# ratt-ru/tricolour

Measured on AMD Instinct MI355X. Metric: Mvis/s flagged (bl x time x chan x corr), higher is better.
Workload: dtype f32 data / f64 accumulators / u8 flags; 1 GPU; MeerKAT-64 slab: 252 of 2016 bl x 4 corr x 1024 time x 4096 chan per GPU (BASELINE configs[1] processed as HBM-resident baseline slabs), sum_threshold_flagger kwargs=stage1; params=stage1

## Files before the change

tricolour_amd/csrc/kernels_elementwise.hpp:

```cpp
#pragma once

template <int VD>
__global__ void k_prepare(const void* __restrict__ vis, const uint8_t* __restrict__ iflags,
                          float* __restrict__ data, uint8_t* __restrict__ flags,
                          int T, int F, int Fa, int factor) {
    size_t idx = (size_t)blockIdx.x * blockDim.x + threadIdx.x;
    size_t NA = (size_t)T * Fa;
    if (idx >= NA) return;
    int t = (int)(idx / Fa), fo = (int)(idx % Fa);
    size_t w = blockIdx.y;
    size_t base = w * (size_t)T * F + (size_t)t * F;
    int f0 = fo * factor;
    int f1 = min(F, f0 + factor);
    float sum = 0.0f;
    int cnt = 0;
    for (int f = f0; f < f1; f++) {
        if (VD == TRI_VIS_F64) {
            const double a = fabs(reinterpret_cast<const double*>(vis)[base + f]);
            if (!iflags[base + f] && !isnan(a)) { sum = (float)((double)sum + a); cnt++; }
            continue;
        }
        float a = load_amp<VD>(vis, base + f);
        if (!iflags[base + f] && !isnan(a)) { sum += a; cnt++; }
    }
    size_t o = w * NA + idx;
    if (cnt == 0) { data[o] = 0.0f; flags[o] = 1; }
    else { data[o] = sum / (float)cnt; flags[o] = 0; }
}

__global__ void k_abs_c64(const float2* __restrict__ z, float* __restrict__ out, size_t n) {
    size_t i = (size_t)blockIdx.x * blockDim.x + threadIdx.x;
    if (i < n) out[i] = tri_hypotf(z[i].x, z[i].y);
}

template <typename T, bool PANEL = false>
__global__ void k_transpose(const T* __restrict__ src, T* __restrict__ dst, int R, int C,
                            size_t src_ws, size_t dst_ws, float denom) {
    __shared__ T tile[64][65];
    const T* s = src + (size_t)blockIdx.z * src_ws;
    T* d = dst + (size_t)blockIdx.z * dst_ws;
    int c0 = blockIdx.x * 64, r0 = blockIdx.y * 64;
    int tx = threadIdx.x, ty = threadIdx.y;
    for (int j = ty; j < 64; j += 4) {
        int r = r0 + j, c = c0 + tx;
        if (r < R && c < C) tile[j][tx] = s[(size_t)r * C + c];
    }
    __syncthreads();
    for (int j = ty; j < 64; j += 4) {
        int c = c0 + j, r = r0 + tx;
        if (r < R && c < C) {
            T v = tile[tx][j];
            if (sizeof(T) == 4 && denom != 0.0f) v = (T)((float)v / denom);
            if (PANEL) d[((size_t)blockIdx.y * C + c) * 64 + tx] = v;
            else d[(size_t)c * R + r] = v;
        }
    }
}

template <typename T>
__global__ void k_panelize(const T* __restrict__ src, T* __restrict__ dst, int L, int C, size_t ws) {
    const size_t i = (size_t)blockIdx.x * blockDim.x + threadIdx.x;
    if (i >= (size_t)L * C) return;
    const int l = (int)(i / C), c = (int)(i % C);
    dst[blockIdx.y * ws + ((size_t)(c >> 6) * L + l) * 64 + (c & 63)] = src[blockIdx.y * ws + i];
}
template <typename T>
__global__ void k_unpanel_w(const T* __restrict__ src, T* __restrict__ dst, int L, int C, size_t ws) {
    const size_t i = (size_t)blockIdx.x * blockDim.x + threadIdx.x;
    if (i >= (size_t)L * C) return;
    const int l = (int)(i / C), c = (int)(i % C);
    dst[blockIdx.y * ws + i] = src[blockIdx.y * ws + ((size_t)(c >> 6) * L + l) * 64 + (c & 63)];
}
template <typename T>
__global__ void k_unpanel(const T* __restrict__ src, T* __restrict__ dst, int L, int C) {
    const size_t i = (size_t)blockIdx.x * blockDim.x + threadIdx.x;
    if (i >= (size_t)L * C) return;
    const int l = (int)(i / C), c = (int)(i % C);
    dst[i] = src[((size_t)(c >> 6) * L + l) * 64 + (c & 63)];
}

template <bool COPY, bool ZERO>
__global__ __launch_bounds__(256) void k_transpose_u8w(const uint8_t* __restrict__ src, uint8_t* __restrict__ dst,
                                                       uint8_t* __restrict__ copy, float* __restrict__ data, int R, int C,
                                                       size_t src_ws, size_t dst_ws, size_t copy_ws, size_t data_ws) {
    __shared__ unsigned tile[128][17];
    const uint8_t* s = src + (size_t)blockIdx.z * src_ws;
    uint8_t* d = dst + (size_t)blockIdx.z * dst_ws;
    const int c0 = blockIdx.x * 64, r0 = blockIdx.y * 128;
    const int tid = threadIdx.x;
    {
        const int tx = tid & 15, ty = tid >> 4;
        const int c = c0 + 4 * tx;
#pragma unroll
        for (int j = 0; j < 8; j++) {
            const int rr = ty + 16 * j, r = r0 + rr;
            unsigned v = 0;
            if (r < R && c < C) {
                v = *reinterpret_cast<const unsigned*>(s + (size_t)r * C + c);
                if (COPY) *reinterpret_cast<unsigned*>(copy + (size_t)blockIdx.z * copy_ws + (size_t)r * C + c) = v;
            }
            tile[rr][tx] = v;
        }
    }
    __syncthreads();
    const int bx = tid & 31, q0 = tid >> 5;
    const int r = r0 + 4 * bx;
    if (r >= R) return;
#pragma unroll
    for (int h = 0; h < 2; h++) {
        const int q = q0 + 8 * h;
        const unsigned a0 = tile[4 * bx][q], a1 = tile[4 * bx + 1][q], a2 = tile[4 * bx + 2][q], a3 = tile[4 * bx + 3][q];
        const unsigned t0 = __builtin_amdgcn_perm(a1, a0, 0x05010400u), t1 = __builtin_amdgcn_perm(a1, a0, 0x07030602u);
        const unsigned u0 = __builtin_amdgcn_perm(a3, a2, 0x05010400u), u1 = __builtin_amdgcn_perm(a3, a2, 0x07030602u);
        const unsigned o[4] = {__builtin_amdgcn_perm(u0, t0, 0x05040100u), __builtin_amdgcn_perm(u0, t0, 0x07060302u),
                               __builtin_amdgcn_perm(u1, t1, 0x05040100u), __builtin_amdgcn_perm(u1, t1, 0x07060302u)};
#pragma unroll
        for (int b = 0; b < 4; b++) {
            const int c = c0 + 4 * q + b;
            if (c >= C) break;
            *reinterpret_cast<unsigned*>(d + (size_t)c * R + r) = o[b];
            if (ZERO && o[b]) {
                const unsigned f = o[b];
                float4* pd = reinterpret_cast<float4*>(data + (size_t)blockIdx.z * data_ws + (size_t)c * R + r);
                float4 x = *pd;
                const bool dirty = ((f & 0xFFu) && __float_as_uint(x.x)) || ((f & 0xFF00u) && __float_as_uint(x.y)) ||
                                   ((f & 0xFF0000u) && __float_as_uint(x.z)) || ((f & 0xFF000000u) && __float_as_uint(x.w));
                if (dirty)
                    *pd = make_float4((f & 0xFFu) ? 0.0f : x.x, (f & 0xFF00u) ? 0.0f : x.y, (f & 0xFF0000u) ? 0.0f : x.z,
                                      (f & 0xFF000000u) ? 0.0f : x.w);
            }
        }
    }
}

__global__ void k_build_wo(const float* __restrict__ data, const uint8_t* __restrict__ flags,
                           float* __restrict__ w, float* __restrict__ o, size_t nper,
                           size_t sws, size_t dws) {
    size_t i = (size_t)blockIdx.x * blockDim.x + threadIdx.x;
    if (i >= nper) return;
    size_t win = blockIdx.y;
    bool fl = flags[win * sws + i] != 0;
    w[win * dws + i] = fl ? 0.0f : 1.0f;
    o[win * dws + i] = fl ? 0.0f : data[win * sws + i];
}

__global__ void k_build_wo4(const float* __restrict__ data, const uint8_t* __restrict__ flags,
                            float* __restrict__ w, float* __restrict__ o, size_t n4per,
                            size_t sws, size_t dws) {
    size_t i = (size_t)blockIdx.x * blockDim.x + threadIdx.x;
    if (i >= n4per) return;
    size_t win = blockIdx.y;
    uchar4 f = reinterpret_cast<const uchar4*>(flags + win * sws)[i];
    float4 d = reinterpret_cast<const float4*>(data + win * sws)[i];
    reinterpret_cast<float4*>(w + win * dws)[i] =
        make_float4(f.x ? 0.0f : 1.0f, f.y ? 0.0f : 1.0f, f.z ? 0.0f : 1.0f, f.w ? 0.0f : 1.0f);
    reinterpret_cast<float4*>(o + win * dws)[i] =
        make_float4(f.x ? 0.0f : d.x, f.y ? 0.0f : d.y, f.z ? 0.0f : d.z, f.w ? 0.0f : d.w);
}

template <int MODE>
__global__ void k_masked_div(const float* __restrict__ w, float* __restrict__ o,
                             const float* __restrict__ data, size_t nper, size_t ws_wo,
                             size_t ws_data, float denom, uint8_t* __restrict__ nanflag, int C) {
    size_t i = (size_t)blockIdx.x * blockDim.x + threadIdx.x;
    if (i >= nper) return;
    size_t win = blockIdx.y;
    float wv = w[win * ws_wo + i];
    float ov = o[win * ws_wo + i];
    if (denom != 0.0f) { wv = wv / denom; ov = ov / denom; }
    float bg = (wv == 0.0f) ? NAN : ov / wv;
    if (MODE != 1 && nanflag && isnan(bg)) nanflag[win * (size_t)C + (i % C)] = 1;
    if (MODE == 1) bg = fabsf(data[win * ws_data + i] - bg);
    o[win * ws_wo + i] = bg;
    if (MODE == 2) const_cast<float*>(w)[win * ws_wo + i] = data[win * ws_data + i] - bg;
}

template <bool TWOD>
__global__ void k_reject(const float* __restrict__ resid, uint8_t* __restrict__ flags,
                         const double* __restrict__ med, const int* __restrict__ chunk_of,
                         double scale, int L, int C, int G, size_t ws_resid, size_t ws_flags) {
    size_t i = (size_t)blockIdx.x * blockDim.x + threadIdx.x;
    if (i >= (size_t)L * C) return;
    size_t win = blockIdx.y;
    int l = (int)(i / C), c = (int)(i % C);
    int g = chunk_of[l];
    double m = TWOD ? med[win * G + g] : med[(size_t)c * G + g];
    double thr = m * scale;
    if ((double)resid[win * ws_resid + i] > thr) flags[win * ws_flags + i] = 1;
}

__global__ void k_colinterp(float* __restrict__ a, int L, int C, size_t ws,
                            const uint8_t* __restrict__ nanflag, const float* __restrict__ data,
                            size_t ws_data, float* __restrict__ resid, float* __restrict__ panel, size_t ws_panel) {
    int c = blockIdx.x * blockDim.x + threadIdx.x;
    if (c >= C) return;
    if (nanflag && !nanflag[(size_t)blockIdx.y * C + c]) return;
    float* x = a + (size_t)blockIdx.y * ws + c;
    const size_t Cs = (size_t)C;
    int last = -1;
    float lastv = 0.0f;
    int run = 0;
    constexpr int PFI = 64;
    for (int i0 = 0; i0 < L; i0 += PFI) {
        float vv[PFI];
#pragma unroll
        for (int u = 0; u < PFI; u++) vv[u] = (i0 + u < L) ? x[(size_t)(i0 + u) * Cs] : NAN;
#pragma unroll
        for (int u = 0; u < PFI; u++) {
            const int i = i0 + u;
            const float v = vv[u];
            if (i >= L || isnan(v)) continue;
            if (run < i) {
                if (last < 0) {
                    for (int j = run; j < i; j++) x[(size_t)j * Cs] = v;
                } else {
                    float diff = v - lastv;
                    double grad = (double)diff / (double)(i - last);
                    for (int j = run; j < i; j++)
                        x[(size_t)j * Cs] = (float)((double)lastv + (double)(j - last) * grad);
                }
            }
            last = i;
            lastv = v;
            run = i + 1;
        }
    }
    if (run < L) {
        float fill = last < 0 ? 0.0f : lastv;
        for (int j = run; j < L; j++) x[(size_t)j * Cs] = fill;
    }
    if (resid) {
        const float* d = data + (size_t)blockIdx.y * ws_data + c;
        float* rr = resid + (size_t)blockIdx.y * ws + c;
        int j = 0;
        for (; j + PFI <= L; j += PFI) {
            float dv[PFI], xv[PFI];
#pragma unroll
            for (int u = 0; u < PFI; u++) { dv[u] = d[(size_t)(j + u) * Cs]; xv[u] = x[(size_t)(j + u) * Cs]; }
#pragma unroll
            for (int u = 0; u < PFI; u++) rr[(size_t)(j + u) * Cs] = dv[u] - xv[u];
        }
        for (; j < L; j++) rr[(size_t)j * Cs] = d[(size_t)j * Cs] - x[(size_t)j * Cs];
        if (panel) {
            float* pp = panel + (size_t)blockIdx.y * ws_panel + (size_t)c * 64;
            for (j = 0; j < L; j++) pp[(size_t)(j >> 6) * Cs * 64 + (j & 63)] = rr[(size_t)j * Cs];
        }
    }
}

#define INTERP_SEG 512
__global__ void k_interp_scan(const float* __restrict__ a, int L, int C, size_t ws, const uint8_t* __restrict__ nanflag,
                              int* __restrict__ tab) {
    const int c = blockIdx.x * 64 + threadIdx.x;
    if (c >= C) return;
    const int seg = blockIdx.y, nseg = gridDim.y;
    const int s0 = seg * INTERP_SEG, s1 = min(L, s0 + INTERP_SEG);
    int* t = tab + (((size_t)blockIdx.z * nseg + seg) * 3) * C + c;
    if (nanflag && !nanflag[(size_t)blockIdx.z * C + c]) {
        t[0] = s0; t[C] = s1 - 1; t[2 * (size_t)C] = 0;
        return;
    }
    const float* x = a + (size_t)blockIdx.z * ws + c;
    const size_t Cs = (size_t)C;
    int first = -1, last = -1, nans = 0;
    constexpr int PFI = 64;
    for (int i0 = s0; i0 < s1; i0 += PFI) {
        float vv[PFI];
#pragma unroll
        for (int u = 0; u < PFI; u++) vv[u] = (i0 + u < s1) ? x[(size_t)(i0 + u) * Cs] : 0.0f;
#pragma unroll
        for (int u = 0; u < PFI; u++) {
            const bool nn = isnan(vv[u]);
            if (i0 + u < s1) {
                if (nn) nans = 1;
                else { if (first < 0) first = i0 + u; last = i0 + u; }
            }
        }
    }
    t[0] = first; t[C] = last; t[2 * (size_t)C] = nans;
}

__global__ void k_interp_fix(float* __restrict__ a, int L, int C, size_t ws, const int* __restrict__ tab,
                             const float* __restrict__ data, size_t ws_data, float* __restrict__ resid,
                             float* __restrict__ panel, size_t ws_panel) {
    const int c = blockIdx.x * 64 + threadIdx.x;
    if (c >= C) return;
    const int seg = blockIdx.y, nseg = gridDim.y;
    const int* tw = tab + (size_t)blockIdx.z * nseg * 3 * C + c;
    if (!tw[((size_t)seg * 3 + 2) * C]) return;
    const int s0 = seg * INTERP_SEG, s1 = min(L, s0 + INTERP_SEG);
    float* x = a + (size_t)blockIdx.z * ws + c;
    const float* d = resid ? data + (size_t)blockIdx.z * ws_data + c : nullptr;
    float* rr = resid ? resid + (size_t)blockIdx.z * ws + c : nullptr;
    float* pp = (resid && panel) ? panel + (size_t)blockIdx.z * ws_panel + (size_t)c * 64 : nullptr;
    const size_t Cs = (size_t)C;
    auto put = [&](int j, float v) {
        x[(size_t)j * Cs] = v;
        if (resid) {
            const float dr = d[(size_t)j * Cs] - v;
            rr[(size_t)j * Cs] = dr;
            if (pp) pp[(size_t)(j >> 6) * Cs * 64 + (j & 63)] = dr;
        }
    };
    auto fill = [&](int lo, int hi, int last, float lastv, int i, float v) {
        if (last < 0) {
            for (int j = lo; j < hi; j++) put(j, v);
        } else {
            float diff = v - lastv;
            double grad = (double)diff / (double)(i - last);
            for (int j = lo; j < hi; j++) put(j, (float)((double)lastv + (double)(j - last) * grad));
        }
    };
    int last = -1;
    for (int sg = seg - 1; sg >= 0 && last < 0; sg--) last = tw[((size_t)sg * 3 + 1) * C];
    float lastv = last >= 0 ? x[(size_t)last * Cs] : 0.0f;
    int run = s0;
    constexpr int PFI = 64;
    for (int i0 = s0; i0 < s1; i0 += PFI) {
        float vv[PFI];
#pragma unroll
        for (int u = 0; u < PFI; u++) vv[u] = (i0 + u < s1) ? x[(size_t)(i0 + u) * Cs] : NAN;
#pragma unroll
        for (int u = 0; u < PFI; u++) {
            const int i = i0 + u;
            const float v = vv[u];
            if (i >= s1 || isnan(v)) continue;
            if (run < i) fill(run, i, last, lastv, i, v);
            last = i;
            lastv = v;
            run = i + 1;
        }
    }
    if (run < s1) {
        int nxt = -1;
        for (int sg = seg + 1; sg < nseg && nxt < 0; sg++) nxt = tw[((size_t)sg * 3) * C];
        if (nxt >= 0) {
            fill(run, s1, last, lastv, nxt, x[(size_t)nxt * Cs]);
        } else {
            const float f = last < 0 ? 0.0f : lastv;
            for (int j = run; j < s1; j++) put(j, f);
        }
    }
}

__global__ void k_sub(const float* __restrict__ a, const float* __restrict__ b,
                      float* __restrict__ out, size_t nper, size_t ws_a, size_t ws_b,
                      size_t ws_o) {
    size_t i = (size_t)blockIdx.x * blockDim.x + threadIdx.x;
    if (i >= nper) return;
    size_t win = blockIdx.y;
    out[win * ws_o + i] = a[win * ws_a + i] - b[win * ws_b + i];
}

__global__ void k_or(uint8_t* __restrict__ a, const uint8_t* __restrict__ b, size_t nper,
                     size_t ws_a, size_t ws_b) {
    size_t i = (size_t)blockIdx.x * blockDim.x + threadIdx.x;
    if (i >= nper) return;
    size_t win = blockIdx.y;
    if (b[win * ws_b + i]) a[win * ws_a + i] = 1;
}

__global__ void k_copy_u8(const uint8_t* __restrict__ a, uint8_t* __restrict__ b, size_t n) {
    size_t i = (size_t)blockIdx.x * blockDim.x + threadIdx.x;
    if (i < n) b[i] = a[i];
}

__global__ void k_or_spec(uint8_t* __restrict__ flags, const uint8_t* __restrict__ spec, int T,
                          int Fa, int Wn) {
    size_t i = (size_t)blockIdx.x * blockDim.x + threadIdx.x;
    if (i >= (size_t)T * Fa) return;
    size_t win = blockIdx.y;
    int f = (int)(i % Fa);
    if (spec[(size_t)f * Wn + win]) flags[win * (size_t)T * Fa + i] = 1;
}

__global__ void k_combine(const uint8_t* __restrict__ spec, const uint8_t* __restrict__ tflags,
                          const uint8_t* __restrict__ fflags, uint8_t* __restrict__ comb, int T,
                          int Fa, int Wn, int lo, int hi) {
    size_t i = (size_t)blockIdx.x * blockDim.x + threadIdx.x;
    if (i >= (size_t)T * Fa) return;
    size_t win = blockIdx.y;
    int t = (int)(i / Fa), f = (int)(i % Fa);
    size_t base = win * (size_t)T * Fa;
    int t0 = max(t + lo, 0), t1 = min(t + hi, T);
    uint8_t v = 0;
    if (t1 > t0) {
        if (spec[(size_t)f * Wn + win]) v = 1;
        for (int tt = t0; tt < t1 && !v; tt++) {
            size_t a = base + (size_t)tt * Fa + f;
            v = (tflags[a] | fflags[a]) ? 1 : 0;
        }
    }
    comb[base + i] = v;
}

__global__ void k_unaverage(const uint8_t* __restrict__ comb, uint8_t* __restrict__ dil,
                            int* __restrict__ rowcnt, int* __restrict__ colcnt, int T, int Fa,
                            int F, int avg, int lo, int hi) {
    int f = blockIdx.x * blockDim.x + threadIdx.x;
    int t = blockIdx.y;
    size_t win = blockIdx.z;
    int v = 0;
    if (f < F) {
        int f0 = max(f + lo, 0), f1 = min(f + hi, F);
        const uint8_t* row = comb + win * (size_t)T * Fa + (size_t)t * Fa;
        for (int ff = f0; ff < f1 && !v; ff++) v = row[ff / avg] ? 1 : 0;
        dil[win * (size_t)T * F + (size_t)t * F + f] = (uint8_t)v;
        if (v) atomicAdd(&colcnt[win * (size_t)F + f], 1);
    }
    unsigned long long b = __ballot(v);
    if ((threadIdx.x & 63) == 0 && b) atomicAdd(&rowcnt[win * (size_t)T + t], __popcll(b));
}

template <int VD>
__global__ void k_final(const uint8_t* __restrict__ dil, const int* __restrict__ rowcnt,
                        const int* __restrict__ colcnt, const void* __restrict__ vis,
                        uint8_t* __restrict__ out, uint8_t* __restrict__ iter, int T, int F,
                        double row_limit, double col_limit, int update_iter) {
    size_t i = (size_t)blockIdx.x * blockDim.x + threadIdx.x;
    if (i >= (size_t)T * F) return;
    size_t win = blockIdx.y;
    int t = (int)(i / F), f = (int)(i % F);
    size_t a = win * (size_t)T * F + i;
    bool v = dil[a] != 0;
    v = v || ((double)rowcnt[win * (size_t)T + t] > row_limit);
    v = v || ((double)colcnt[win * (size_t)F + f] > col_limit);
    v = v || load_isnan<VD>(vis, a);
    out[a] = v ? 1 : 0;
    if (update_iter && v) iter[a] = 1;
}

__device__ __forceinline__ uint4 or4(uint4 a, uint4 b) { return make_uint4(a.x | b.x, a.y | b.y, a.z | b.z, a.w | b.w); }
__device__ __forceinline__ unsigned nz_bytes(unsigned x) {
    unsigned t = (x & 0x7F7F7F7Fu) + 0x7F7F7F7Fu;
    return ((t | x) & 0x80808080u) >> 7;
}

template <int VD>
__global__ void k_prepare4(const void* __restrict__ vis, const uint8_t* __restrict__ iflags,
                           float* __restrict__ data, uint8_t* __restrict__ flags, size_t n4) {
    size_t i = (size_t)blockIdx.x * blockDim.x + threadIdx.x;
    if (i >= n4) return;
    uchar4 f = reinterpret_cast<const uchar4*>(iflags)[i];
    float a[4];
    if (VD == TRI_VIS_C64) {
        float4 z0 = reinterpret_cast<const float4*>(vis)[2 * i];
        float4 z1 = reinterpret_cast<const float4*>(vis)[2 * i + 1];
        a[0] = tri_hypotf(z0.x, z0.y); a[1] = tri_hypotf(z0.z, z0.w);
        a[2] = tri_hypotf(z1.x, z1.y); a[3] = tri_hypotf(z1.z, z1.w);
    } else {
        float4 z = reinterpret_cast<const float4*>(vis)[i];
        a[0] = fabsf(z.x); a[1] = fabsf(z.y); a[2] = fabsf(z.z); a[3] = fabsf(z.w);
    }
    unsigned char fl[4] = {f.x, f.y, f.z, f.w};
    float o[4];
    unsigned char of[4];
#pragma unroll
    for (int k = 0; k < 4; k++) {
        bool bad = fl[k] != 0 || isnan(a[k]);
        o[k] = bad ? 0.0f : (0.0f + a[k]) / 1.0f;
        of[k] = bad ? 1 : 0;
    }
    reinterpret_cast<float4*>(data)[i] = make_float4(o[0], o[1], o[2], o[3]);
    reinterpret_cast<uchar4*>(flags)[i] = make_uchar4(of[0], of[1], of[2], of[3]);
}

template <int VD>
__global__ void k_amplitude4(const void* __restrict__ vis, float* __restrict__ ampl,
                             uint8_t* __restrict__ iter, uint16_t* __restrict__ nanmask, size_t n4) {
    size_t i = (size_t)blockIdx.x * blockDim.x + threadIdx.x;
    if (i >= n4) return;
    float a[4];
    bool vn[4];
    if (VD == TRI_VIS_C64) {
        float4 z0 = reinterpret_cast<const float4*>(vis)[2 * i];
        float4 z1 = reinterpret_cast<const float4*>(vis)[2 * i + 1];
        a[0] = tri_hypotf(z0.x, z0.y); a[1] = tri_hypotf(z0.z, z0.w);
        a[2] = tri_hypotf(z1.x, z1.y); a[3] = tri_hypotf(z1.z, z1.w);
        vn[0] = isnan(z0.x) || isnan(z0.y); vn[1] = isnan(z0.z) || isnan(z0.w);
        vn[2] = isnan(z1.x) || isnan(z1.y); vn[3] = isnan(z1.z) || isnan(z1.w);
    } else {
        float4 z = reinterpret_cast<const float4*>(vis)[i];
        a[0] = fabsf(z.x); a[1] = fabsf(z.y); a[2] = fabsf(z.z); a[3] = fabsf(z.w);
        vn[0] = isnan(z.x); vn[1] = isnan(z.y); vn[2] = isnan(z.z); vn[3] = isnan(z.w);
    }
#pragma unroll
    for (int k = 0; k < 4; k++) a[k] = (0.0f + a[k]) / 1.0f;
    reinterpret_cast<float4*>(ampl)[i] = make_float4(a[0], a[1], a[2], a[3]);
    const unsigned nanb = (isnan(a[0]) ? 1u : 0u) | (isnan(a[1]) ? 0x100u : 0u) | (isnan(a[2]) ? 0x10000u : 0u) |
                          (isnan(a[3]) ? 0x1000000u : 0u);
    if (nanb) reinterpret_cast<unsigned*>(iter)[i] |= nanb;
    unsigned m = ((vn[0] ? 1u : 0u) | (vn[1] ? 2u : 0u) | (vn[2] ? 4u : 0u) | (vn[3] ? 8u : 0u)) << (4 * (threadIdx.x & 3));
    m |= __shfl_xor(m, 1, 64);
    m |= __shfl_xor(m, 2, 64);
    if ((threadIdx.x & 3) == 0) nanmask[i >> 2] = (uint16_t)m;
}

__global__ void k_zero_flagged4(const uint8_t* __restrict__ flags, float* __restrict__ data, size_t n4per,
                                size_t ws_flags, size_t ws_data) {
    size_t i = (size_t)blockIdx.x * blockDim.x + threadIdx.x;
    if (i >= n4per) return;
    size_t win = blockIdx.y;
    const unsigned f = reinterpret_cast<const unsigned*>(flags + win * ws_flags)[i];
    if (f == 0) return;
    float4* pd = reinterpret_cast<float4*>(data + win * ws_data) + i;
    float4 d = *pd;
    *pd = make_float4((f & 0xFFu) ? 0.0f : d.x, (f & 0xFF00u) ? 0.0f : d.y, (f & 0xFF0000u) ? 0.0f : d.z,
                      (f & 0xFF000000u) ? 0.0f : d.w);
}

template <int OP>
__global__ void k_u8_op16(const uint8_t* __restrict__ a, uint8_t* __restrict__ b, size_t n16per,
                          size_t ws_a, size_t ws_b) {
    size_t i = (size_t)blockIdx.x * blockDim.x + threadIdx.x;
    if (i >= n16per) return;
    size_t win = blockIdx.y;
    uint4 va = reinterpret_cast<const uint4*>(a + win * ws_a)[i];
    uint4* pb = reinterpret_cast<uint4*>(b + win * ws_b) + i;
    if (OP == 0) *pb = va;
    else if (OP == 1) *pb = or4(*pb, va);
    else *pb = make_uint4(nz_bytes(va.x), nz_bytes(va.y), nz_bytes(va.z), nz_bytes(va.w));
}

__global__ void k_spec_rows(const uint8_t* __restrict__ spec, uint8_t* __restrict__ rows, int Fa, int Wn) {
    size_t i = (size_t)blockIdx.x * blockDim.x + threadIdx.x;
    if (i >= (size_t)Fa * Wn) return;
    int w = (int)(i / Fa), f = (int)(i % Fa);
    rows[i] = spec[(size_t)f * Wn + w];
}

__global__ void k_or_spec16(uint8_t* __restrict__ flags, const uint8_t* __restrict__ spec_rows, int T, int Fa16) {
    size_t i = (size_t)blockIdx.x * blockDim.x + threadIdx.x;
    if (i >= (size_t)T * Fa16) return;
    size_t win = blockIdx.y;
    int f16 = (int)(i % Fa16);
    uint4 sp = reinterpret_cast<const uint4*>(spec_rows + win * (size_t)Fa16 * 16)[f16];
    uint4* pf = reinterpret_cast<uint4*>(flags + win * (size_t)T * Fa16 * 16) + i;
    *pf = or4(*pf, sp);
}

__global__ void k_or_spec_more16(uint8_t* __restrict__ flags, const uint8_t* __restrict__ spec_rows,
                                 const uint8_t* __restrict__ more, int T, int Fa16) {
    size_t i = (size_t)blockIdx.x * blockDim.x + threadIdx.x;
    if (i >= (size_t)T * Fa16) return;
    size_t win = blockIdx.y;
    int f16 = (int)(i % Fa16);
    uint4 sp = reinterpret_cast<const uint4*>(spec_rows + win * (size_t)Fa16 * 16)[f16];
    size_t a = win * (size_t)T * Fa16 + i;
    uint4* pf = reinterpret_cast<uint4*>(flags) + a;
    *pf = or4(or4(*pf, sp), reinterpret_cast<const uint4*>(more)[a]);
}

__global__ void k_or_spec_ft16(uint8_t* __restrict__ flagsFT, const uint8_t* __restrict__ spec_rows, int T16, int Fa) {
    size_t i = (size_t)blockIdx.x * blockDim.x + threadIdx.x;
    if (i >= (size_t)T16 * Fa) return;
    size_t win = blockIdx.y;
    int f = (int)(i / T16);
    if (!spec_rows[win * (size_t)Fa + f]) return;
    reinterpret_cast<uint4*>(flagsFT + win * (size_t)T16 * 16 * Fa)[i] = make_uint4(0x01010101u, 0x01010101u, 0x01010101u, 0x01010101u);
}

__global__ void k_combine16(const uint8_t* __restrict__ spec_rows, const uint8_t* __restrict__ tflags,
                            const uint8_t* __restrict__ fflags, uint8_t* __restrict__ comb, int T,
                            int Fa16, int lo, int hi) {
    size_t i = (size_t)blockIdx.x * blockDim.x + threadIdx.x;
    if (i >= (size_t)T * Fa16) return;
    size_t win = blockIdx.y;
    int t = (int)(i / Fa16), f16 = (int)(i % Fa16);
    size_t base = win * (size_t)T * Fa16;
    int t0 = max(t + lo, 0), t1 = min(t + hi, T);
    uint4 v = make_uint4(0, 0, 0, 0);
    if (t1 > t0) {
        v = reinterpret_cast<const uint4*>(spec_rows + win * (size_t)Fa16 * 16)[f16];
        const uint4* tp = reinterpret_cast<const uint4*>(tflags) + base;
        const uint4* fp = reinterpret_cast<const uint4*>(fflags) + base;
        for (int tt = t0; tt < t1; tt++) {
            size_t a = (size_t)tt * Fa16 + f16;
            v = or4(v, or4(tp[a], fp[a]));
        }
    }
    reinterpret_cast<uint4*>(comb)[base + i] = v;
}

template <bool TPANEL>
__global__ __launch_bounds__(64) void k_combine_dilate16(const uint8_t* __restrict__ spec_rows, const uint8_t* __restrict__ tflags,
                                                        const uint8_t* __restrict__ fflags, uint8_t* __restrict__ dil,
                                                        int* __restrict__ rowcnt, int T, int F16, int lo, int hi) {
    const int lane = threadIdx.x;
    const int f16 = blockIdx.x * 64 + lane;
    const int t = blockIdx.y;
    const size_t win = blockIdx.z;
    const size_t base = win * (size_t)T * F16;
    const int t0 = max(t + lo, 0), t1 = min(t + hi, T);
    const bool in = f16 < F16;
    uint4 c = make_uint4(0, 0, 0, 0);
    if (in && t1 > t0) {
        c = reinterpret_cast<const uint4*>(spec_rows + win * (size_t)F16 * 16)[f16];
        const uint4* tp = reinterpret_cast<const uint4*>(tflags) + base;
        const uint4* fp = reinterpret_cast<const uint4*>(fflags) + base;
        for (int tt = t0; tt < t1; tt++) {
            size_t a = (size_t)tt * F16 + f16;
            size_t at = TPANEL ? ((size_t)(f16 >> 2) * T + tt) * 4 + (f16 & 3) : a;
            c = or4(c, or4(tp[at], fp[a]));
        }
    }
    auto edge = [&](int g, int b) -> unsigned {
        if (g < 0 || g >= F16 || t1 <= t0) return 0u;
        unsigned v = spec_rows[(win * (size_t)F16 + g) * 16 + b];
        for (int tt = t0; tt < t1; tt++) {
            size_t a = (base + (size_t)tt * F16 + g) * 16 + b;
            size_t at = TPANEL ? (base + ((size_t)(g >> 2) * T + tt) * 4 + (g & 3)) * 16 + b : a;
            v |= (unsigned)tflags[at] | (unsigned)fflags[a];
        }
        return v;
    };
    unsigned prev = __shfl_up(c.w >> 24, 1, 64), next = __shfl_down(c.x & 0xFFu, 1, 64);
    if (lane == 0) prev = edge(f16 - 1, 15);
    if (lane == 63) next = edge(f16 + 1, 0);
    int cnt = 0;
    if (in) {
        const unsigned w[4] = {c.x, c.y, c.z, c.w};
        unsigned o[4];
#pragma unroll
        for (int j = 0; j < 4; j++) {
            const unsigned left = (w[j] << 8) | (j > 0 ? w[j - 1] >> 24 : prev & 0xFFu);
            const unsigned right = (w[j] >> 8) | ((j < 3 ? w[j + 1] & 0xFFu : next & 0xFFu) << 24);
            o[j] = (w[j] | left | right) & 0x01010101u;
            cnt += __popc(o[j]);
        }
        reinterpret_cast<uint4*>(dil)[base + (size_t)t * F16 + f16] = make_uint4(o[0], o[1], o[2], o[3]);
    }
    for (int off = 32; off > 0; off >>= 1) cnt += __shfl_down(cnt, off, 64);
    if (lane == 0 && cnt) atomicAdd(&rowcnt[win * (size_t)T + t], cnt);
}

template <int LO, int E>
__global__ void k_unaverage16(const uint8_t* __restrict__ comb, uint8_t* __restrict__ dil,
                              int* __restrict__ rowcnt, int T, int F16) {
    int f16 = blockIdx.x * blockDim.x + threadIdx.x;
    int t = blockIdx.y;
    size_t win = blockIdx.z;
    int cnt = 0;
    if (f16 < F16) {
        const uint4* row = reinterpret_cast<const uint4*>(comb) + (win * (size_t)T + t) * F16;
        uint4 z = make_uint4(0, 0, 0, 0);
        uint4 p = f16 > 0 ? row[f16 - 1] : z;
        uint4 c = row[f16];
        uint4 n = f16 + 1 < F16 ? row[f16 + 1] : z;
        unsigned w[12] = {p.x, p.y, p.z, p.w, c.x, c.y, c.z, c.w, n.x, n.y, n.z, n.w};
        unsigned o[4] = {0, 0, 0, 0};
#pragma unroll
        for (int k = 0; k < 16; k++) {
            unsigned v = 0;
#pragma unroll
            for (int sft = LO; sft < LO + E; sft++) {
                const int idx = 16 + k + sft;
                v |= (w[idx >> 2] >> (8 * (idx & 3))) & 0xFFu;
            }
            o[k >> 2] |= (v & 1u) << (8 * (k & 3));
        }
        reinterpret_cast<uint4*>(dil)[(win * (size_t)T + t) * F16 + f16] = make_uint4(o[0], o[1], o[2], o[3]);
        cnt = __popc(o[0]) + __popc(o[1]) + __popc(o[2]) + __popc(o[3]);
    }
    for (int off = 32; off > 0; off >>= 1) cnt += __shfl_down(cnt, off, 64);
    if ((threadIdx.x & 63) == 0 && cnt) atomicAdd(&rowcnt[win * (size_t)T + t], cnt);
}

__global__ void k_colcount(const uint8_t* __restrict__ dil, int* __restrict__ colcnt, int T, int F4) {
    int f4 = blockIdx.x * blockDim.x + threadIdx.x;
    if (f4 >= F4) return;
    size_t win = blockIdx.y;
    const unsigned* p = reinterpret_cast<const unsigned*>(dil) + win * (size_t)T * F4 + f4;
    unsigned c0 = 0, c1 = 0, c2 = 0, c3 = 0;
    int t = 0;
    for (; t + 8 <= T; t += 8) {
        unsigned v[8];
#pragma unroll
        for (int u = 0; u < 8; u++) v[u] = p[(size_t)(t + u) * F4];
#pragma unroll
        for (int u = 0; u < 8; u++) {
            c0 += v[u] & 0xFFu; c1 += (v[u] >> 8) & 0xFFu; c2 += (v[u] >> 16) & 0xFFu; c3 += v[u] >> 24;
        }
    }
    for (; t < T; t++) {
        unsigned v = p[(size_t)t * F4];
        c0 += v & 0xFFu; c1 += (v >> 8) & 0xFFu; c2 += (v >> 16) & 0xFFu; c3 += v >> 24;
    }
    reinterpret_cast<int4*>(colcnt)[win * (size_t)F4 + f4] = make_int4((int)c0, (int)c1, (int)c2, (int)c3);
}

#define TRI_VIS_NANMASK (-1000)
template <int VD>
__global__ void k_final16(const uint8_t* __restrict__ dil, const int* __restrict__ rowcnt,
                          const int* __restrict__ colcnt, const void* __restrict__ vis,
                          uint8_t* __restrict__ out, uint8_t* __restrict__ iter, int T, int F16,
                          double row_limit, double col_limit, int update_iter) {
    size_t i = (size_t)blockIdx.x * blockDim.x + threadIdx.x;
    if (i >= (size_t)T * F16) return;
    size_t win = blockIdx.y;
    int t = (int)(i / F16), f16 = (int)(i % F16);
    size_t a16 = win * (size_t)T * F16 + i;
    uint4 d = reinterpret_cast<const uint4*>(dil)[a16];
    unsigned dw[4] = {d.x, d.y, d.z, d.w};
    bool rowall = (double)rowcnt[win * (size_t)T + t] > row_limit;
    const int4* cc = reinterpret_cast<const int4*>(colcnt + win * (size_t)F16 * 16) + (size_t)f16 * 4;
    unsigned o[4];
    unsigned nm = 0;
    if (VD == TRI_VIS_NANMASK) nm = reinterpret_cast<const uint16_t*>(vis)[a16];
#pragma unroll
    for (int q = 0; q < 4; q++) {
        int4 c4 = cc[q];
        int cv[4] = {c4.x, c4.y, c4.z, c4.w};
        unsigned nanb = 0;
        if (VD == TRI_VIS_NANMASK) {
            const unsigned b = nm >> (4 * q);
            nanb = (b & 1u) | ((b & 2u) << 7) | ((b & 4u) << 14) | ((b & 8u) << 21);
        } else if (VD == TRI_VIS_C64) {
            const float4* vp = reinterpret_cast<const float4*>(vis) + (a16 * 16 + q * 4) / 2;
            float4 z0 = vp[0], z1 = vp[1];
            nanb = ((isnan(z0.x) || isnan(z0.y)) ? 1u : 0u) | ((isnan(z0.z) || isnan(z0.w)) ? 0x100u : 0u) |
                   ((isnan(z1.x) || isnan(z1.y)) ? 0x10000u : 0u) | ((isnan(z1.z) || isnan(z1.w)) ? 0x1000000u : 0u);
        } else {
            float4 z = reinterpret_cast<const float4*>(vis)[(a16 * 16 + q * 4) / 4];
            nanb = (isnan(z.x) ? 1u : 0u) | (isnan(z.y) ? 0x100u : 0u) | (isnan(z.z) ? 0x10000u : 0u) |
                   (isnan(z.w) ? 0x1000000u : 0u);
        }
        unsigned colb = 0;
#pragma unroll
        for (int k = 0; k < 4; k++) colb |= ((double)cv[k] > col_limit ? 1u : 0u) << (8 * k);
        o[q] = rowall ? 0x01010101u : (dw[q] | colb | nanb);
    }
    uint4 ov = make_uint4(o[0], o[1], o[2], o[3]);
    reinterpret_cast<uint4*>(out)[a16] = ov;
    if (update_iter) {
        uint4* ip = reinterpret_cast<uint4*>(iter) + a16;
        *ip = or4(*ip, ov);
    }
}

template <int MODE>
__global__ void k_masked_div4(const float* __restrict__ w, float* __restrict__ o,
                              const float* __restrict__ data, size_t n4per, size_t ws_wo, size_t ws_data,
                              float denom, uint8_t* __restrict__ nanflag, int C) {
    size_t i = (size_t)blockIdx.x * blockDim.x + threadIdx.x;
    if (i >= n4per) return;
    size_t win = blockIdx.y;
    float4 wv = reinterpret_cast<const float4*>(w + win * ws_wo)[i];
    float4* po = reinterpret_cast<float4*>(o + win * ws_wo) + i;
    float4 ov = *po;
    if (denom != 0.0f) {
        wv = make_float4(wv.x / denom, wv.y / denom, wv.z / denom, wv.w / denom);
        ov = make_float4(ov.x / denom, ov.y / denom, ov.z / denom, ov.w / denom);
    }
    float bg[4] = {(wv.x == 0.0f) ? NAN : ov.x / wv.x, (wv.y == 0.0f) ? NAN : ov.y / wv.y,
                   (wv.z == 0.0f) ? NAN : ov.z / wv.z, (wv.w == 0.0f) ? NAN : ov.w / wv.w};
    if (MODE != 1 && nanflag) {
        int cb = (int)((i * 4) % C);
#pragma unroll
        for (int k = 0; k < 4; k++)
            if (isnan(bg[k])) nanflag[win * (size_t)C + cb + k] = 1;
    }
    if (MODE == 1) {
        float4 dv = reinterpret_cast<const float4*>(data + win * ws_data)[i];
        bg[0] = fabsf(dv.x - bg[0]); bg[1] = fabsf(dv.y - bg[1]);
        bg[2] = fabsf(dv.z - bg[2]); bg[3] = fabsf(dv.w - bg[3]);
    }
    *po = make_float4(bg[0], bg[1], bg[2], bg[3]);
    if (MODE == 2) {
        float4 dv = reinterpret_cast<const float4*>(data + win * ws_data)[i];
        reinterpret_cast<float4*>(const_cast<float*>(w) + win * ws_wo)[i] =
            make_float4(dv.x - bg[0], dv.y - bg[1], dv.z - bg[2], dv.w - bg[3]);
    }
}

__global__ void k_sub4(const float* __restrict__ a, const float* __restrict__ b, float* __restrict__ out,
                       size_t n4per, size_t ws_a, size_t ws_b, size_t ws_o) {
    size_t i = (size_t)blockIdx.x * blockDim.x + threadIdx.x;
    if (i >= n4per) return;
    size_t win = blockIdx.y;
    float4 x = reinterpret_cast<const float4*>(a + win * ws_a)[i];
    float4 y = reinterpret_cast<const float4*>(b + win * ws_b)[i];
    reinterpret_cast<float4*>(out + win * ws_o)[i] = make_float4(x.x - y.x, x.y - y.y, x.z - y.z, x.w - y.w);
}

__global__ void __launch_bounds__(256)
k_reject4_t(const float* __restrict__ resid, uint8_t* __restrict__ flags, uint8_t* __restrict__ flags_t4,
            const double* __restrict__ med, const int* __restrict__ chunk_of, double scale, int L, int C4, int G,
            size_t ws_resid, size_t ws_flags) {
    __shared__ unsigned tile[64][65];
    const size_t win = blockIdx.z;
    const int w0 = blockIdx.x * 64, l0 = blockIdx.y * 64;
    const int tx = threadIdx.x, ty = threadIdx.y;
    const float4* r4 = reinterpret_cast<const float4*>(resid + win * ws_resid);
    unsigned* fw = reinterpret_cast<unsigned*>(flags + win * ws_flags);
    unsigned* ft = reinterpret_cast<unsigned*>(flags_t4 + win * ws_flags);
    for (int j = ty; j < 64; j += 4) {
        const int l = l0 + j, w = w0 + tx;
        if (l < L && w < C4) {
            const double thr = med[win * G + chunk_of[l]] * scale;
            const size_t i = (size_t)l * C4 + w;
            const float4 rv = r4[i];
            unsigned f = fw[i];
            if ((double)rv.x > thr) f = (f & 0xFFFFFF00u) | 0x00000001u;
            if ((double)rv.y > thr) f = (f & 0xFFFF00FFu) | 0x00000100u;
            if ((double)rv.z > thr) f = (f & 0xFF00FFFFu) | 0x00010000u;
            if ((double)rv.w > thr) f = (f & 0x00FFFFFFu) | 0x01000000u;
            fw[i] = f;
            tile[j][tx] = f;
        }
    }
    __syncthreads();
    for (int j = ty; j < 64; j += 4) {
        const int w = w0 + j, l = l0 + tx;
        if (l < L && w < C4) ft[(size_t)w * L + l] = tile[tx][j];
    }
}

__global__ void __launch_bounds__(256)
k_reject_tf(const float* __restrict__ resid, unsigned* __restrict__ flags_t4, const double* __restrict__ med,
            const int* __restrict__ chunk_of, double scale, int T4, int C, int ld, int G, size_t ws_resid, size_t ws_words) {
    const int c = blockIdx.x * 256 + threadIdx.x;
    if (c >= C) return;
    const int q = blockIdx.y;
    const size_t win = blockIdx.z;
    const double thr = med[win * G + chunk_of[c]] * scale;
    const float* rr = resid + win * ws_resid + (size_t)(4 * q) * ld + c;
    unsigned* pw = flags_t4 + win * ws_words + (size_t)q * C + c;
    unsigned f = *pw;
    if ((double)rr[0] > thr) f = (f & 0xFFFFFF00u) | 0x00000001u;
    if ((double)rr[(size_t)ld] > thr) f = (f & 0xFFFF00FFu) | 0x00000100u;
    if ((double)rr[(size_t)2 * ld] > thr) f = (f & 0xFF00FFFFu) | 0x00010000u;
    if ((double)rr[(size_t)3 * ld] > thr) f = (f & 0x00FFFFFFu) | 0x01000000u;
    *pw = f;
}

__global__ void k_reject4(const float* __restrict__ resid, uint8_t* __restrict__ flags,
                          const double* __restrict__ med, const int* __restrict__ chunk_of,
                          double scale, int C4, int G, size_t n4per, size_t ws_resid, size_t ws_flags) {
    size_t i = (size_t)blockIdx.x * blockDim.x + threadIdx.x;
    if (i >= n4per) return;
    size_t win = blockIdx.y;
    int l = (int)(i / C4);
    double thr = med[win * G + chunk_of[l]] * scale;
    float4 rv = reinterpret_cast<const float4*>(resid + win * ws_resid)[i];
    uchar4* pf = reinterpret_cast<uchar4*>(flags + win * ws_flags) + i;
    uchar4 f = *pf;
    if ((double)rv.x > thr) f.x = 1;
    if ((double)rv.y > thr) f.y = 1;
    if ((double)rv.z > thr) f.z = 1;
    if ((double)rv.w > thr) f.w = 1;
    *pf = f;
}

__global__ void k_fill_windows(float2* __restrict__ vis, uint8_t* __restrict__ flags, size_t n) {
    size_t i = (size_t)blockIdx.x * blockDim.x + threadIdx.x;
    if (i >= n) return;
    vis[i] = make_float2(NAN, NAN);
    flags[i] = 1;
}

__global__ void k_pack(const float2* __restrict__ data, const uint8_t* __restrict__ flag,
                       const int32_t* __restrict__ row_bl, const int32_t* __restrict__ row_time,
                       int nchan, int ncorr, int nbl, int ntime, float2* __restrict__ vw,
                       uint8_t* __restrict__ fw) {
    int f = blockIdx.x * blockDim.x + threadIdx.x;
    size_t r = blockIdx.y;
    if (f >= nchan) return;
    int bl = row_bl[r], t = row_time[r];
    if (bl < 0 || bl >= nbl || t < 0 || t >= ntime) return;
    for (int c = 0; c < ncorr; c++) {
        size_t i = (r * nchan + f) * (size_t)ncorr + c;
        size_t o = (((size_t)bl * ncorr + c) * ntime + t) * (size_t)nchan + f;
        vw[o] = data[i];
        fw[o] = flag[i];
    }
}

template <int NC>
__global__ void k_pack_v(const float2* __restrict__ data, const uint8_t* __restrict__ flag,
                         const int32_t* __restrict__ row_bl, const int32_t* __restrict__ row_time,
                         int nchan, int nbl, int ntime, float2* __restrict__ vw, uint8_t* __restrict__ fw) {
    const int f = blockIdx.x * blockDim.x + threadIdx.x;
    const size_t r = blockIdx.y;
    if (f >= nchan) return;
    const int bl = row_bl[r], t = row_time[r];
    if (bl < 0 || bl >= nbl || t < 0 || t >= ntime) return;
    const size_t i = (r * nchan + f) * (size_t)NC;
    float2 v[NC];
    uint8_t fl[NC];
    if (NC == 4) {
        const float4 a = reinterpret_cast<const float4*>(data + i)[0], b = reinterpret_cast<const float4*>(data + i)[1];
        v[0] = make_float2(a.x, a.y); v[1 % NC] = make_float2(a.z, a.w);
        v[2 % NC] = make_float2(b.x, b.y); v[3 % NC] = make_float2(b.z, b.w);
        const uchar4 q = *reinterpret_cast<const uchar4*>(flag + i);
        fl[0] = q.x; fl[1 % NC] = q.y; fl[2 % NC] = q.z; fl[3 % NC] = q.w;
    } else if (NC == 2) {
        const float4 a = *reinterpret_cast<const float4*>(data + i);
        v[0] = make_float2(a.x, a.y); v[1 % NC] = make_float2(a.z, a.w);
        const uchar2 q = *reinterpret_cast<const uchar2*>(flag + i);
        fl[0] = q.x; fl[1 % NC] = q.y;
    } else {
        v[0] = data[i];
        fl[0] = flag[i];
    }
#pragma unroll
    for (int c = 0; c < NC; c++) {
        const size_t o = (((size_t)bl * NC + c) * ntime + t) * (size_t)nchan + f;
        vw[o] = v[c];
        fw[o] = fl[c];
    }
}

template <int NC>
__global__ void k_unpack_v(const uint8_t* __restrict__ fw, const int32_t* __restrict__ row_bl,
                           const int32_t* __restrict__ row_time, int nchan, int nbl, int ntime,
                           uint8_t* __restrict__ out, int any_corr) {
    const int f = blockIdx.x * blockDim.x + threadIdx.x;
    const size_t r = blockIdx.y;
    if (f >= nchan) return;
    const int bl = row_bl[r], t = row_time[r];
    const bool ok = !(bl < 0 || bl >= nbl || t < 0 || t >= ntime);
    uint8_t v[NC];
    uint8_t any = 0;
#pragma unroll
    for (int c = 0; c < NC; c++) {
        v[c] = ok ? fw[(((size_t)bl * NC + c) * ntime + t) * (size_t)nchan + f] : 0;
        any |= v[c] ? 1 : 0;
    }
    const size_t i = (r * nchan + f) * (size_t)NC;
    if (NC == 4) *reinterpret_cast<uchar4*>(out + i) = any_corr ? make_uchar4(any, any, any, any) : make_uchar4(v[0], v[1 % NC], v[2 % NC], v[3 % NC]);
    else if (NC == 2) *reinterpret_cast<uchar2*>(out + i) = any_corr ? make_uchar2(any, any) : make_uchar2(v[0], v[1 % NC]);
    else out[i] = any_corr ? any : v[0];
}

__global__ void k_unpack(const uint8_t* __restrict__ fw, const int32_t* __restrict__ row_bl,
                         const int32_t* __restrict__ row_time, int nchan, int ncorr, int nbl,
                         int ntime, uint8_t* __restrict__ out, int any_corr) {
    int f = blockIdx.x * blockDim.x + threadIdx.x;
    size_t r = blockIdx.y;
    if (f >= nchan) return;
    int bl = row_bl[r], t = row_time[r];
    bool ok = !(bl < 0 || bl >= nbl || t < 0 || t >= ntime);
    uint8_t any = 0;
    if (any_corr && ok)
        for (int c = 0; c < ncorr; c++)
            any |= fw[(((size_t)bl * ncorr + c) * ntime + t) * (size_t)nchan + f] ? 1 : 0;
    for (int c = 0; c < ncorr; c++) {
        size_t i = (r * nchan + f) * (size_t)ncorr + c;
        uint8_t v = ok ? fw[(((size_t)bl * ncorr + c) * ntime + t) * (size_t)nchan + f] : 0;
        out[i] = any_corr ? any : v;
    }
}

template <int VD>
__global__ void k_flag_nans_zeros(const void* __restrict__ vis, const uint8_t* __restrict__ flags,
                                  uint8_t* __restrict__ out, size_t n) {
    size_t i = (size_t)blockIdx.x * blockDim.x + threadIdx.x;
    if (i >= n) return;
    bool f;
    if (VD == TRI_VIS_C64) {
        float2 z = reinterpret_cast<const float2*>(vis)[i];
        f = (z.x == 0.0f && z.y == 0.0f) || isnan(z.x) || isnan(z.y);
    } else {
        float x = reinterpret_cast<const float*>(vis)[i];
        f = x == 0.0f || isnan(x);
    }
    out[i] = (f || flags[i] != 0) ? 1 : 0;
}

__global__ void k_apply_bl_chan_mask(const uint8_t* __restrict__ flags, uint8_t* __restrict__ out,
                                     const uint8_t* __restrict__ bl_sel,
                                     const uint8_t* __restrict__ chan_mask, int mode, int nchan,
                                     size_t rows_per_bl, size_t row0, size_t bl0) {
    int f = blockIdx.x * blockDim.x + threadIdx.x;
    if (f >= nchan) return;
    size_t bl = bl0 + blockIdx.z;
    size_t a = (bl * rows_per_bl + row0 + blockIdx.y) * (size_t)nchan + f;
    uint8_t v = flags[a];
    if (bl_sel[bl]) v = mode == 0 ? (uint8_t)((v | chan_mask[f]) ? 1 : 0) : (uint8_t)(chan_mask[f] ? 1 : 0);
    out[a] = v;
}


__global__ void k_uv_count(const uint8_t* __restrict__ rflags, unsigned* __restrict__ cnt, size_t N) {
    size_t cp = blockIdx.y;
    size_t i0 = (size_t)blockIdx.x * 4096;
    unsigned c = 0;
    for (size_t i = i0 + threadIdx.x; i < min(N, i0 + 4096); i += 256) c += rflags[cp * N + i] ? 1u : 0u;
    for (int o = 32; o > 0; o >>= 1) c += __shfl_down(c, o, 64);
    if ((threadIdx.x & 63) == 0 && c) atomicAdd(&cnt[cp], c);
}

__global__ void k_uv_mean(const float2* __restrict__ vis, const uint8_t* __restrict__ rflags,
                          float2* __restrict__ avg, int T, int F) {
    int f = blockIdx.x * blockDim.x + threadIdx.x;
    if (f >= F) return;
    size_t cp = blockIdx.y;
    size_t base = cp * (size_t)T * F + f;
    float sr = 0.0f, si = 0.0f;
    long long n = 0;
    for (int t = 0; t < T; t++) {
        size_t a = base + (size_t)t * F;
        float2 z = vis[a];
        if (!rflags[a] && !isnan(z.x) && !isnan(z.y)) { sr += z.x; si += z.y; n++; }
    }
    float2 m = make_float2(0.0f, 0.0f);
    if (n > 0 && isfinite(sr) && isfinite(si)) m = make_float2((float)((double)sr / (double)n), (float)((double)si / (double)n));
    avg[cp * (size_t)F + f] = m;
}

__global__ void __launch_bounds__(256)
k_uv_lowpass(const float2* __restrict__ avg, float2* __restrict__ smooth, int F, int K) {
    __shared__ double xr[64], xi[64];
    __shared__ double red[2][4];
    size_t cp = blockIdx.x;
    const float2* a = avg + cp * (size_t)F;
    const int tid = threadIdx.x, lane = tid & 63, wave = tid >> 6;
    for (int k = 0; k < K; k++) {
        double pr = 0.0, pi_ = 0.0;
        for (int f = tid; f < F; f += 256) {
            double s, c;
            long long kf = ((long long)k * f) % F;
            sincospi(2.0 * (double)kf / (double)F, &s, &c);
            double re = a[f].x, im = a[f].y;
            pr += re * c + im * s;
            pi_ += im * c - re * s;
        }
        for (int o = 32; o > 0; o >>= 1) { pr += __shfl_down(pr, o, 64); pi_ += __shfl_down(pi_, o, 64); }
        if (lane == 0) { red[0][wave] = pr; red[1][wave] = pi_; }
        __syncthreads();
        if (tid == 0) {
            xr[k] = red[0][0] + red[0][1] + red[0][2] + red[0][3];
            xi[k] = red[1][0] + red[1][1] + red[1][2] + red[1][3];
        }
        __syncthreads();
    }
// ... 221 lines not shown
```

tricolour_amd/csrc/tricolour_amd.hip:

```cpp
#include <unordered_set>
#include "tri_common.hpp"
#include "kernels_elementwise.hpp"
#include "kernels_median.hpp"
#include "kernels_reject.hpp"
#include "kernels_reject_tile.hpp"
#include "kernels_boxfilter.hpp"
#include "kernels_boxline.hpp"
#include "kernels_boxpipe.hpp"
#include "kernels_boxweight.hpp"
#include "kernels_boxexact.hpp"
#include "kernels_sumthreshold.hpp"
#include "kernels_scan.hpp"
#include "kernels_sir.hpp"
#include "kernels_linerms.hpp"
#include "steps/kernels_blint.hpp"
#include "steps/ldev/kernels_ldev.hpp"

namespace {

static hipError_t lds_optin(const void* fn, hipFuncAttribute attr, int value) {
    thread_local std::unordered_set<uint64_t> done;
    int dev = 0;
    hipError_t e = hipGetDevice(&dev);
    if (e != hipSuccess) return e;
// ... 530 lines not shown
    LAUNCHCHK();
    return TRI_OK;
}

template <int KS>
int launch_boxt_spec_ks(const Run& r, const float* srcData, const uint8_t* srcFlags, float* dstW, float* dstO,
                        int n, int C, int rad, float denom) {
    const int d = 2 * rad - KS;
    const size_t lds = (size_t)4 * d * 64 * sizeof(float);
    dim3 grid((unsigned)cdiv(C, 64), 2);
    HIPCHK(lds_optin_all(160 * 1024, &k_boxt_spec<KS, true>));
    if (d > 0) hipLaunchKernelGGL((k_boxt_spec<KS, true>), grid, dim3(64), lds, r.st, srcData, srcFlags, dstW, dstO, n, C, rad, denom);
    else hipLaunchKernelGGL((k_boxt_spec<KS, false>), grid, dim3(64), 0, r.st, srcData, srcFlags, dstW, dstO, n, C, rad, denom);
    LAUNCHCHK();
    return TRI_OK;
}

int launch_boxt_spec(const Run& r, int ks, const float* srcData, const uint8_t* srcFlags, float* dstW, float* dstO,
                     int n, int C, int rad, float denom) {
    switch (ks) {
        case 8: return launch_boxt_spec_ks<8>(r, srcData, srcFlags, dstW, dstO, n, C, rad, denom);
        case 16: return launch_boxt_spec_ks<16>(r, srcData, srcFlags, dstW, dstO, n, C, rad, denom);
        case 32: return launch_boxt_spec_ks<32>(r, srcData, srcFlags, dstW, dstO, n, C, rad, denom);
        case 64: return launch_boxt_spec_ks<64>(r, srcData, srcFlags, dstW, dstO, n, C, rad, denom);
        case 80: return launch_boxt_spec_ks<80>(r, srcData, srcFlags, dstW, dstO, n, C, rad, denom);
    }
    return set_err(TRI_EINVAL, "no register-ring kernel for %d slots", ks);
}

static thread_local int g_boxp_override = -1;
static int boxp_pick_block(int rad, int C) {
    static const bool off = is1(getenv("TRI_SPEC_NO_PIPE"));
    if (g_boxp_override == 0 || (off && g_boxp_override < 0)) return 0;
    if (g_boxp_override != 8 && 2 * rad >= 16 && C % 4 == 0 && boxp_lds_bytes(rad, 16) <= 160 * 1024) return 16;
    if (g_boxp_override == 16) return 0;
    if (2 * rad >= 8 && C % 2 == 0 && boxp_lds_bytes(rad, 8) <= 160 * 1024) return 8;
    return 0;
}

template <int B, int P>
int launch_boxp_spec_b(const Run& r, const float* srcData, const uint8_t* srcFlags, float* dstW, float* dstO,
                       int n, int C, int rad, float denom) {
    HIPCHK(lds_optin_all(160 * 1024, &k_boxp_spec<B, P>));
    dim3 grid((unsigned)cdiv(C, 64), 2);
    hipLaunchKernelGGL((k_boxp_spec<B, P>), grid, dim3(256), boxp_lds_bytes(rad, B), r.st, srcData, srcFlags, dstW, dstO, n, C, rad, denom);
    LAUNCHCHK();
    return TRI_OK;
}

#ifndef BOXQ_MIN_2R
#define BOXQ_MIN_2R 56
#endif
thread_local int g_boxq_override = -1;
static int boxq_pick_ks(int rad) {
    static const bool off = is1(getenv("TRI_FILTER_NO_PIPE_T"));
    if (g_boxq_override == 0 || (off && g_boxq_override < 0)) return 0;
    const int ks = 2 * rad / 16 * 16;
    return (ks >= 16 && ks <= 96) ? ks : 0;
}

template <int KS, int B = 16>
int launch_boxq_ks(const Run& r, const float* srcData, const uint8_t* srcFlags, float* dstW, float* dstO,
                   int n, int C, int rad, float denom, size_t sws, size_t dws, int64_t W) {
    HIPCHK(lds_optin_all(160 * 1024, &k_boxq<KS, 0, B>, &k_boxq<KS, 1, B>));
    dim3 grid((unsigned)cdiv(C, 64), (unsigned)W);
    const BoxDenom dn = box_reciprocal(denom);
    if (boxw_usable(rad, n, C)) { const int rc = launch_boxw(r, srcFlags, dstW, n, C, rad, denom, sws, dws, W); if (rc) return rc; }
    else hipLaunchKernelGGL((k_boxq<KS, 0, B>), grid, dim3(256), boxq_lds_bytes(B), r.st, srcData, srcFlags, dstW, n, C, rad, dn, sws, dws);
    hipLaunchKernelGGL((k_boxq<KS, 1, B>), grid, dim3(256), boxq_lds_bytes(B), r.st, srcData, srcFlags, dstO, n, C, rad, dn, sws, dws);
    LAUNCHCHK();
    return TRI_OK;
}

#ifndef BOXQ_B8_MIN_2R
#define BOXQ_B8_MIN_2R 32
#endif
#ifndef BOXQ_B8_MAX2R
#define BOXQ_B8_MAX2R 88
#endif
thread_local int g_boxq_b8_override = -1;
static int boxq_pick_ks8(int rad) {
    static const int b8 = [] { const char* e = getenv("TRI_FILTER_PIPE_T_B8"); return e ? atoi(e) : 1; }();
    if (!b8 || g_boxq_b8_override == 0 || 2 * rad < BOXQ_B8_MIN_2R || 2 * rad >= BOXQ_B8_MAX2R) return 0;
    return 2 * rad / 8 * 8;
}

template <int KS>
int launch_boxq_deep(const Run& r, const float* srcData, const uint8_t* srcFlags, float* dstW, float* dstO,
                     int n, int C, int rad, float denom, size_t sws, size_t dws, int64_t W) {
    HIPCHK(lds_optin_all(160 * 1024, &k_boxq_deep<KS, 0>, &k_boxq_deep<KS, 1>));
    dim3 grid((unsigned)cdiv(C, 64), (unsigned)W);
    const BoxDenom dn = box_reciprocal(denom);
    if (boxw_usable(rad, n, C)) { const int rc = launch_boxw(r, srcFlags, dstW, n, C, rad, denom, sws, dws, W); if (rc) return rc; }
    else hipLaunchKernelGGL((k_boxq_deep<KS, 0>), grid, dim3(256), boxq_lds_bytes(8, 4), r.st, srcData, srcFlags, dstW, n, C, rad, dn, sws, dws);
    hipLaunchKernelGGL((k_boxq_deep<KS, 1>), grid, dim3(256), boxq_lds_bytes(8, 4), r.st, srcData, srcFlags, dstO, n, C, rad, dn, sws, dws);
    LAUNCHCHK();
    return TRI_OK;
}
#ifndef BOXQ_DEEP
#define BOXQ_DEEP 1
#endif

int launch_boxq(const Run& r, int ks, const float* srcData, const uint8_t* srcFlags, float* dstW, float* dstO,
                int n, int C, int rad, float denom, size_t sws, size_t dws, int64_t W) {
    if (BOXQ_DEEP && boxq_pick_ks8(40) > 0) {
        if (2 * rad >= 88 && 2 * rad < 96) return launch_boxq_deep<80>(r, srcData, srcFlags, dstW, dstO, n, C, rad, denom, sws, dws, W);
        if (2 * rad >= 104 && 2 * rad < 112) return launch_boxq_deep<96>(r, srcData, srcFlags, dstW, dstO, n, C, rad, denom, sws, dws, W);
    }
    switch (boxq_pick_ks8(rad)) {
        case 32: return launch_boxq_ks<32, 8>(r, srcData, srcFlags, dstW, dstO, n, C, rad, denom, sws, dws, W);
        case 40: return launch_boxq_ks<40, 8>(r, srcData, srcFlags, dstW, dstO, n, C, rad, denom, sws, dws, W);
        case 48: return launch_boxq_ks<48, 8>(r, srcData, srcFlags, dstW, dstO, n, C, rad, denom, sws, dws, W);
        case 56: return launch_boxq_ks<56, 8>(r, srcData, srcFlags, dstW, dstO, n, C, rad, denom, sws, dws, W);
        case 64: return launch_boxq_ks<64, 8>(r, srcData, srcFlags, dstW, dstO, n, C, rad, denom, sws, dws, W);
        case 80: return launch_boxq_ks<80, 8>(r, srcData, srcFlags, dstW, dstO, n, C, rad, denom, sws, dws, W);
    }
    switch (ks) {
        case 16: return launch_boxq_ks<16>(r, srcData, srcFlags, dstW, dstO, n, C, rad, denom, sws, dws, W);
        case 32: return launch_boxq_ks<32>(r, srcData, srcFlags, dstW, dstO, n, C, rad, denom, sws, dws, W);
        case 48: return launch_boxq_ks<48>(r, srcData, srcFlags, dstW, dstO, n, C, rad, denom, sws, dws, W);
        case 64: return launch_boxq_ks<64>(r, srcData, srcFlags, dstW, dstO, n, C, rad, denom, sws, dws, W);
        case 80: return launch_boxq_ks<80>(r, srcData, srcFlags, dstW, dstO, n, C, rad, denom, sws, dws, W);
        case 96: return launch_boxq_ks<96>(r, srcData, srcFlags, dstW, dstO, n, C, rad, denom, sws, dws, W);
    }
    return set_err(TRI_EINVAL, "no stage-pipeline kernel for %d slots", ks);
}

int launch_boxt(const Run& r, int ks, const float* srcData, const uint8_t* srcFlags, float* dstW, float* dstO,
                int n, int C, int rad, float denom, size_t sws, size_t dws, int64_t W) {
    switch (ks) {
        case 16: return launch_boxt_ks<16>(r, srcData, srcFlags, dstW, dstO, n, C, rad, denom, sws, dws, W);
        case 20: return launch_boxt_ks<20>(r, srcData, srcFlags, dstW, dstO, n, C, rad, denom, sws, dws, W);
        case 32: return launch_boxt_ks<32>(r, srcData, srcFlags, dstW, dstO, n, C, rad, denom, sws, dws, W);
        case 64: return launch_boxt_ks<64>(r, srcData, srcFlags, dstW, dstO, n, C, rad, denom, sws, dws, W);
        case 80: return launch_boxt_ks<80>(r, srcData, srcFlags, dstW, dstO, n, C, rad, denom, sws, dws, W);
    }
    return set_err(TRI_EINVAL, "no register-ring kernel for %d slots", ks);
}

enum class ColSrc {
    ByteFlags,
    Images,
    PackedFlags
};
enum ColFlag : unsigned {
    COL_TRANSPOSED_OUT = 1,
    COL_WEIGHTS_01 = 2
};
enum class ColFamily { SpecPipe, SpecRing, StagePipe, RegRing, Lane4, LdsRing, MultiPass };
thread_local bool g_colfilter_unpadded = false;

int launch_colfilter(const Run& r, ColSrc src, float* bufW, float* bufO, const float* srcData,
                     const uint8_t* srcFlags, float* dstW, float* dstO, int n, int C, int rad,
                     size_t bws, size_t sws, size_t dws, int64_t W, unsigned flags = 0, float* deferred_denom = nullptr) {
    const bool transposed_out = flags & COL_TRANSPOSED_OUT, weights_are_01 = flags & COL_WEIGHTS_01;
    const float denom = box_denominator(rad);
    const int intw = (weights_are_01 && rad <= 31) ? 1 : 0;
    int bt = colfilter_lds_block(rad, C);
    if (deferred_denom) *deferred_denom = 0.0f;
    const bool regs_ok = !deferred_denom && !transposed_out && weights_are_01 && (uint64_t)n * (uint64_t)C * 4u < (1ull << 31);
    const bool spectrum = regs_ok && src == ColSrc::ByteFlags && W == 1;
    const bool packed = regs_ok && src == ColSrc::PackedFlags && n % 4 == 0;
    ColFamily fam;
    if (spectrum && boxp_pick_block(rad, C) > 0 && rad <= 107 && ((uintptr_t)srcData % 16 == 0) && ((uintptr_t)srcFlags % 4 == 0) &&
        ((uintptr_t)dstW % 16 == 0) && ((uintptr_t)dstO % 16 == 0))
        fam = ColFamily::SpecPipe;
    else if (spectrum && boxr_pick_ks(rad) > 0) fam = ColFamily::SpecRing;
    else if (packed && boxq_pick_ks(rad) > 0 && rad <= 107 && (g_boxq_override == 1 || 2 * rad >= BOXQ_MIN_2R)) fam = ColFamily::StagePipe;
    else if (packed && boxr_pick_ks_t(rad) > 0) fam = ColFamily::RegRing;
    else if (bt > 0 && colfilter_use_lane4(rad) && !transposed_out && src != ColSrc::ByteFlags) fam = ColFamily::Lane4;
    else {
        if (bt > 0 && colfilter_use_lane4(rad) && src == ColSrc::ByteFlags) {
            bt = rad <= 20 ? 128 : (rad <= 40 ? 64 : 0);
            while (bt > 64 && bt / 2 >= C) bt /= 2;
        }
        fam = bt > 0 ? ColFamily::LdsRing : ColFamily::MultiPass;
    }
    if (fam == ColFamily::MultiPass && g_colfilter_unpadded)
        return set_err(TRI_EUNSUPPORTED, "radius %d takes the in-place multi-pass filter, which needs images padded to n + 4r rows", rad);
    const bool built = src != ColSrc::Images, divide = !deferred_denom;
    const float *const inW = built ? nullptr : bufW, *const inO = built ? nullptr : bufO;
    const size_t in_ws = built ? 0 : bws;
    switch (fam) {
        case ColFamily::SpecPipe:
            if (boxp_pick_block(rad, C) == 16) return launch_boxp_spec_b<16, 16>(r, srcData, srcFlags, dstW, dstO, n, C, rad, denom);
            return launch_boxp_spec_b<8, 16>(r, srcData, srcFlags, dstW, dstO, n, C, rad, denom);
        case ColFamily::SpecRing:
            return launch_boxt_spec(r, boxr_pick_ks(rad), srcData, srcFlags, dstW, dstO, n, C, rad, denom);
        case ColFamily::StagePipe:
            return launch_boxq(r, boxq_pick_ks(rad), srcData, srcFlags, dstW, dstO, n, C, rad, denom, sws, dws, W);
        case ColFamily::RegRing:
            return launch_boxt(r, boxr_pick_ks_t(rad), srcData, srcFlags, dstW, dstO, n, C, rad, denom, sws, dws, W);
        case ColFamily::Lane4: {
            HIPCHK(lds_optin_all(160 * 1024, &k_colfilter_lane4<0, true>, &k_colfilter_lane4<1, true>, &k_colfilter_lane4<1, false>,
                                 &k_colfilter_lane4<2, false>, &k_colfilter_lane4<2, true>));
            const auto k = src == ColSrc::PackedFlags ? (divide ? &k_colfilter_lane4<2, true> : &k_colfilter_lane4<2, false>)
                                                      : (divide ? &k_colfilter_lane4<1, true> : &k_colfilter_lane4<1, false>);
            if (!divide) *deferred_denom = denom;
            hipLaunchKernelGGL(k, dim3((unsigned)cdiv(C, 16), (unsigned)W, 2), dim3(64), (size_t)lane4_ring_capacity(rad) * 64 * sizeof(float), r.st,
                               inW, inO, srcData, srcFlags, dstW, dstO, n, C, rad, denom, in_ws, sws, dws);
            break;
        }
        case ColFamily::LdsRing: {
            HIPCHK(lds_optin_all(160 * 1024, &k_colfilter_lds<0, true, false>, &k_colfilter_lds<1, true, false>, &k_colfilter_lds<1, false, false>,
                                 &k_colfilter_lds<1, true, true>, &k_colfilter_lds<2, false, false>, &k_colfilter_lds<2, true, false>));
            auto k = &k_colfilter_lds<0, true, false>;
            bool div = true;
            if (src == ColSrc::PackedFlags) { div = divide; k = div ? &k_colfilter_lds<2, true, false> : &k_colfilter_lds<2, false, false>; }
            else if (transposed_out) k = &k_colfilter_lds<1, true, true>;
            else if (src == ColSrc::Images) { div = divide; k = div ? &k_colfilter_lds<1, true, false> : &k_colfilter_lds<1, false, false>; }
            if (!div) *deferred_denom = denom;
            hipLaunchKernelGGL(k, dim3((unsigned)cdiv(C, bt), (unsigned)W, 2), dim3(bt), (size_t)4 * 2 * rad * bt * sizeof(float), r.st,
                               inW, inO, srcData, srcFlags, dstW, dstO, n, C, rad, denom, in_ws, sws, dws, intw);
            break;
        }
        case ColFamily::MultiPass: {
            const int blk = C >= 256 ? 256 : (C >= 128 ? 128 : 64);
            const auto k = src == ColSrc::ByteFlags ? &k_colfilter<0> : &k_colfilter<1>;
            hipLaunchKernelGGL(k, dim3((unsigned)cdiv(C, blk), (unsigned)W, 2), dim3(blk), 0, r.st, bufW, bufO, srcData, srcFlags,
                               dstW, dstO, n, C, rad, denom, bws, sws, dws);
            break;
        }
    }
    LAUNCHCHK();
    return TRI_OK;
}

bool st_use_pipe(const StWin& sw) {
    static const bool off = is1(getenv("TRI_ST_NO_PIPE"));
    return !off && sw.nw >= 1 && sw.nw <= 8 && stp_lds_bytes(sw) <= 160 * 1024;
}

enum class StKernel { Dyn, Fused, Mask, MaskPanel, Pipe };

int st_launch(hipStream_t st, StKernel k, const StWin& sw, const float* data, const double* med, uint8_t* out,
              const int64_t* d_chunk_ends, double thr_scale, int L, int C, int G, size_t ws_data, size_t ws_out, int64_t W,
              double* ring, uint8_t* acc) {
    int blk = C >= 256 ? 256 : (C >= 128 ? 128 : 64);
    if (const char* e = getenv("TRI_ST_BLK")) { int b = atoi(e); if (b >= 64 && b <= ST_MAXBLK && C >= b) blk = b; }
    const dim3 grid((unsigned)cdiv(C, blk), (unsigned)G, (unsigned)W);
    StFusedArgs fa;
    for (int j = 0; j < 4; j++) fa.tf[j] = sw.tf[j < sw.nw ? j : 0];
    if (k == StKernel::MaskPanel)
        hipLaunchKernelGGL((k_colst_mask<1, 2, 4, 8, true>), grid, dim3(blk), 0, st, data, med, out, d_chunk_ends, fa, thr_scale, L, C, G, ws_data, ws_out);
    else if (k == StKernel::Mask)
        hipLaunchKernelGGL((k_colst_mask<1, 2, 4, 8>), grid, dim3(blk), 0, st, data, med, out, d_chunk_ends, fa, thr_scale, L, C, G, ws_data, ws_out);
    else if (k == StKernel::Fused)
        hipLaunchKernelGGL((k_colst_fused<1, 2, 4, 8>), grid, dim3(blk), 0, st, data, med, out, d_chunk_ends, fa, thr_scale, L, C, G, ws_data, ws_out);
    else if (k == StKernel::Pipe) {
        HIPCHK(lds_optin_all(160 * 1024, &k_colst_pipe));
        hipLaunchKernelGGL(k_colst_pipe, dim3((unsigned)cdiv(C, 64), (unsigned)G, (unsigned)W), dim3(64 * sw.nw), stp_lds_bytes(sw), st,
                           data, med, out, d_chunk_ends, sw, stp_plan(sw), thr_scale, L, C, G, ws_data, ws_out);
    } else
        hipLaunchKernelGGL(k_colst_dyn, grid, dim3(blk), 0, st, data, med, out, ring, acc, d_chunk_ends, sw, thr_scale, L, C, G, ws_data, ws_out);
    LAUNCHCHK();
    return TRI_OK;
}

int launch_colst(const Run& r, const StWin& sw, const float* data, const double* med,
                 uint8_t* out, const int64_t* d_chunk_ends, int L, int C, int G, size_t ws_data,
                 size_t ws_out, int64_t W, bool panel = false) {
    StKernel k;
    if (st_use_fused(sw)) {
        if (panel && !(st_use_mask(L, C) && C % 64 == 0)) return set_err(TRI_EUNSUPPORTED, "panel images: lane-mask SumThreshold kernel on 64-column panels only");
        k = panel ? StKernel::MaskPanel : (st_use_mask(L, C) ? StKernel::Mask : StKernel::Fused);
    } else if (panel) {
        return set_err(TRI_EUNSUPPORTED, "panel images: windows (1, 2, 4, 8) only");
    } else {
        k = st_use_pipe(sw) ? StKernel::Pipe : StKernel::Dyn;
    }
    const double thr_scale = r.p->outlier_nsigma * TRI_MAD_NORMAL;
    return st_launch(r.st, k, sw, data, med, out, d_chunk_ends, thr_scale, L, C, G, ws_data, ws_out, W, r.ws.ring, r.ws.acc);
}

int launch_interp(const Run& r, float* a, int L, int C, size_t ws, int64_t W, const uint8_t* nanflag,
                  const float* data, size_t ws_data, float* resid, float* panel = nullptr, size_t ws_panel = 0) {
    static const bool one_pass = is1(getenv("TRI_INTERP_ONE_PASS"));
    const int nseg = (int)cdiv(L, INTERP_SEG);
    if (one_pass || nseg < 2 || nseg > 65535) {
        hipLaunchKernelGGL(k_colinterp, dim3((unsigned)cdiv(C, 256), (unsigned)W), dim3(256), 0, r.st, a, L, C, ws, nanflag, data, ws_data, resid, panel, ws_panel);
    } else {
        dim3 grid((unsigned)cdiv(C, 64), (unsigned)nseg, (unsigned)W);
        hipLaunchKernelGGL(k_interp_scan, grid, dim3(64), 0, r.st, (const float*)a, L, C, ws, nanflag, r.ws.itab);
        hipLaunchKernelGGL(k_interp_fix, grid, dim3(64), 0, r.st, a, L, C, ws, (const int*)r.ws.itab, data, ws_data, resid, panel, ws_panel);
    }
    LAUNCHCHK();
    return TRI_OK;
}

template <typename T>
int launch_transpose(const Run& r, const T* src, T* dst, int R, int C, size_t sws, size_t dws,
                     int64_t W, float denom = 0.0f, bool panel = false) {
    dim3 grid((unsigned)cdiv(C, 64), (unsigned)cdiv(R, 64), (unsigned)W);
    if (panel) {
        if (R % 64 != 0) return set_err(TRI_EUNSUPPORTED, "panel output needs a multiple of 64 columns");
        hipLaunchKernelGGL((k_transpose<T, true>), grid, dim3(64, 4), 0, r.st, src, dst, R, C, sws, dws, denom);
        LAUNCHCHK();
        return TRI_OK;
    }
    if (sizeof(T) == 1 && R % 4 == 0 && C % 4 == 0 && sws % 4 == 0 && dws % 4 == 0 &&
        ((uintptr_t)src % 4 == 0) && ((uintptr_t)dst % 4 == 0)) {
        dim3 gridw((unsigned)cdiv(C, 64), (unsigned)cdiv(R, 128), (unsigned)W);
        hipLaunchKernelGGL((k_transpose_u8w<false, false>), gridw, dim3(256), 0, r.st, (const uint8_t*)src, (uint8_t*)dst,
                           (uint8_t*)nullptr, (float*)nullptr, R, C, sws, dws, (size_t)0, (size_t)0);
        LAUNCHCHK();
        return TRI_OK;
    }
    hipLaunchKernelGGL(k_transpose<T>, grid, dim3(64, 4), 0, r.st, src, dst, R, C, sws, dws, denom);
    LAUNCHCHK();
    return TRI_OK;
}


template <int OP>
int launch_u8(const Run& r, const uint8_t* a, uint8_t* b, size_t nper, size_t ws_a, size_t ws_b, int64_t W) {
    if (r.pl.vec && nper % 16 == 0 && ws_a % 16 == 0 && ws_b % 16 == 0) {
        hipLaunchKernelGGL(k_u8_op16<OP>, grid1(nper / 16, W), dim3(256), 0, r.st, a, b, nper / 16, ws_a, ws_b);
    } else if (OP == 0) {
        for (int64_t w = 0; w < W; w++)
            hipLaunchKernelGGL(k_copy_u8, dim3((unsigned)cdiv(nper, 256)), dim3(256), 0, r.st, a + w * ws_a, b + w * ws_b, nper);
    } else if (OP == 1) {
        hipLaunchKernelGGL(k_or, grid1(nper, W), dim3(256), 0, r.st, b, a, nper, ws_b, ws_a);
    } else {
        for (int64_t w = 0; w < W; w++)
            hipLaunchKernelGGL(k_normalise_flags, dim3((unsigned)cdiv(nper, 256)), dim3(256), 0, r.st, a + w * ws_a, b + w * ws_b, nper);
    }
    LAUNCHCHK();
    return TRI_OK;
}

template <int MODE>
int launch_masked_div(const Run& r, const float* w, float* o, const float* data, size_t nper, size_t ws_wo, size_t ws_data, int64_t W, float denom = 0.0f,
                      uint8_t* nanflag = nullptr, int C = 1) {
    if (nper % 4 == 0 && ws_wo % 4 == 0 && ws_data % 4 == 0 && (nanflag == nullptr || C % 4 == 0) && ((uintptr_t)w % 16 == 0) && ((uintptr_t)o % 16 == 0))
        hipLaunchKernelGGL(k_masked_div4<MODE>, grid1(nper / 4, W), dim3(256), 0, r.st, w, o, data, nper / 4, ws_wo, ws_data, denom, nanflag, C);
    else
        hipLaunchKernelGGL(k_masked_div<MODE>, grid1(nper, W), dim3(256), 0, r.st, w, o, data, nper, ws_wo, ws_data, denom, nanflag, C);
    LAUNCHCHK();
    return TRI_OK;
}

int launch_sub(const Run& r, const float* a, const float* b, float* out, size_t nper, size_t ws_a, size_t ws_b, size_t ws_o, int64_t W) {
    if (nper % 4 == 0 && ws_a % 4 == 0 && ws_b % 4 == 0 && ws_o % 4 == 0 && ((uintptr_t)a % 16 == 0) && ((uintptr_t)b % 16 == 0) && ((uintptr_t)out % 16 == 0))
        hipLaunchKernelGGL(k_sub4, grid1(nper / 4, W), dim3(256), 0, r.st, a, b, out, nper / 4, ws_a, ws_b, ws_o);
    else
        hipLaunchKernelGGL(k_sub, grid1(nper, W), dim3(256), 0, r.st, a, b, out, nper, ws_a, ws_b, ws_o);
    LAUNCHCHK();
    return TRI_OK;
}

static bool filter_no_tin() { static const bool v = is1(getenv("TRI_FILTER_NO_TIN")); return v; }
bool colfilter_t_usable(int rad) { return !filter_no_tin() && rad > 0 && rad <= 16; }

int launch_colfilter_t(const Run& r, const float* srcW, const float* srcO, float* dstW, float* dstO,
                       int n, int C, int ld, int rad, size_t sws_img, size_t dws, int64_t W, float* deferred_denom) {
    float denom = box_denominator(rad);
    size_t lds = ((size_t)4 * 2 * rad * CFT_BT + (size_t)CFT_PF * (CFT_BT + 1)) * sizeof(float);
    HIPCHK(lds_optin_all(160 * 1024, &k_colfilter_lds_t<false>, &k_colfilter_lds_t<true>));
    dim3 grid((unsigned)cdiv(C, CFT_BT), (unsigned)W, 2);
    if (deferred_denom) *deferred_denom = denom;
    const auto k = deferred_denom ? &k_colfilter_lds_t<false> : &k_colfilter_lds_t<true>;
    hipLaunchKernelGGL(k, grid, dim3(CFT_BT), lds, r.st, srcW, srcO, dstW, dstO, n, C, ld, rad, denom, sws_img, dws);
    LAUNCHCHK();
    return TRI_OK;
}

bool colfilter_tf_usable(int rad) {
    static const bool off = is1(getenv("TRI_FILTER_NO_FUSED_DIV"));
    return !off && colfilter_t_usable(rad);
}

template <int MODE>
int launch_colfilter_tf(const Run& r, const float* srcW, const float* srcO, float* dstW, float* dstO, const float* data,
                        int n, int C, int ld, int rad, size_t sws_img, size_t dws, size_t ws_data, int64_t W, uint8_t* nanflag) {
    float denom = box_denominator(rad);
    size_t lds = (size_t)2 * ((size_t)4 * 2 * rad * CFF_BT + (size_t)CFT_PF * (CFF_BT + 1)) * sizeof(float);
    HIPCHK(lds_optin_all(160 * 1024, &k_colfilter_lds_tf<MODE>));
    dim3 grid((unsigned)cdiv(C, CFF_BT), (unsigned)W);
    hipLaunchKernelGGL(k_colfilter_lds_tf<MODE>, grid, dim3(2 * CFF_BT), lds, r.st, srcW, srcO, dstW, dstO, data, n, C, ld, rad,
                       denom, sws_img, dws, ws_data, nanflag);
    LAUNCHCHK();
    return TRI_OK;
}

template <int KS, int MODE>
int launch_boxf_ks(const Run& r, const float* srcW, const float* srcO, float* dstW, float* dstO, const float* data,
                   int n, int C, int ld, int rad, size_t sws_img, size_t dws, size_t ws_data, int64_t W, uint8_t* nanflag,
                   float* dstP, size_t pws, bool* wroteP) {
    const BoxDenom denom = box_reciprocal(box_denominator(rad));
    const int d = 2 * rad - KS;
    if (!(MODE == 2 && boxf_panel_ok(KS, d > 0))) dstP = nullptr;
    if (dstP && wroteP) *wroteP = true;
    const size_t lds = ((size_t)4 * d * 64 + (size_t)2 * boxr_pf_f(KS) * boxf_nsub(KS) * boxf_ts(boxr_pf_f(KS) * boxf_nsub(KS))) * sizeof(float);
    if (srcO <= srcW || ((uint64_t)(srcO - srcW) + (uint64_t)C * ld) * 4u >= (1ull << 31))
        return set_err(TRI_EUNSUPPORTED, "fused frequency stage: the data image must follow the weight image within 2^31 bytes");
    const unsigned gap = (unsigned)(srcO - srcW);
    HIPCHK(lds_optin_all(160 * 1024, &k_boxf<KS, true, MODE>));
    dim3 grid((unsigned)cdiv(C, 32), (unsigned)W);
    auto k = d > 0 ? &k_boxf<KS, true, MODE> : &k_boxf<KS, false, MODE>;
    if constexpr (KS == 32) {
        if (d > 14) { k = &k_boxf<KS, true, MODE, 1>; HIPCHK(lds_optin_all(160 * 1024, k)); }
    }
    hipLaunchKernelGGL(k, grid, dim3(64), lds, r.st, srcW, gap, dstW, dstO, data, n, C, ld, rad, denom, sws_img, dws, ws_data, nanflag, dstP, pws);
    LAUNCHCHK();
    return TRI_OK;
}

#ifndef BOXQF_MIN_2R
#define BOXQF_MIN_2R 34
#endif
#ifndef BOXQF_FEW_WAVES
#define BOXQF_FEW_WAVES 2048
#endif
#ifndef BOXQF_B8_DEFAULT
#define BOXQF_B8_DEFAULT 1
#endif
#ifndef BOXQF_B8_MAX2R
#define BOXQF_B8_MAX2R 88
#endif
template <int KS, int MODE, int B = 16>
int launch_boxqf_ks(const Run& r, const float* srcW, unsigned gap, float* dstW, float* dstO, const float* data,
                    int n, int C, int ld, int rad, size_t sws_img, size_t dws, size_t ws_data, int64_t W, uint8_t* nanflag) {
    HIPCHK(lds_optin_all(160 * 1024, &k_boxqf<KS, MODE, B>));
    const BoxDenom denom = box_reciprocal(box_denominator(rad));
    dim3 grid((unsigned)cdiv(C, 64), (unsigned)W);
    hipLaunchKernelGGL((k_boxqf<KS, MODE, B>), grid, dim3(512), boxqf_lds_bytes(B, boxqf_dbl(KS, B)), r.st, srcW, gap, dstW, dstO, data, n, C, ld, rad,
                       denom, sws_img, dws, ws_data, nanflag);
    LAUNCHCHK();
    return TRI_OK;
}

template <int MODE>
int launch_boxf(const Run& r, int ks, const float* srcW, const float* srcO, float* dstW, float* dstO, const float* data,
                int n, int C, int ld, int rad, size_t sws_img, size_t dws, size_t ws_data, int64_t W, uint8_t* nanflag,
                float* dstP = nullptr, size_t pws = 0, bool* wroteP = nullptr) {
    if (MODE != 2 || n % 64 != 0) dstP = nullptr;
    {
        static const bool off = is1(getenv("TRI_FILTER_NO_PIPE_F"));
        const int kq = boxq_pick_ks(rad);
        const bool few = (int64_t)W * cdiv(C, 32) < BOXQF_FEW_WAVES;
        const bool want = g_boxq_override == 1 || (g_boxq_override < 0 && !off && (2 * rad >= BOXQF_MIN_2R || (few && 2 * rad >= 16)));
        if (want && kq > 0 && srcO > srcW && n % 4 == 0 && ld % 4 == 0 && sws_img % 4 == 0 && (uint64_t)(srcO - srcW) % 4 == 0 &&
            ((uintptr_t)srcW % 16 == 0) && ((uint64_t)(srcO - srcW) + (uint64_t)C * ld) * 4u < (1ull << 31) &&
            (uint64_t)n * (uint64_t)C * 4u < (1ull << 31)) {
            const unsigned gap = (unsigned)(srcO - srcW);
            static const int b8 = [] { const char* e = getenv("TRI_FILTER_PIPE_F_B8"); return e ? atoi(e) : BOXQF_B8_DEFAULT; }();
            if (b8 && g_boxq_b8_override != 0 && 2 * rad >= 16 && 2 * rad < BOXQF_B8_MAX2R) {
                switch (2 * rad / 8 * 8) {
                    case 16: return launch_boxqf_ks<16, MODE, 8>(r, srcW, gap, dstW, dstO, data, n, C, ld, rad, sws_img, dws, ws_data, W, nanflag);
                    case 24: return launch_boxqf_ks<24, MODE, 8>(r, srcW, gap, dstW, dstO, data, n, C, ld, rad, sws_img, dws, ws_data, W, nanflag);
                    case 32: return launch_boxqf_ks<32, MODE, 8>(r, srcW, gap, dstW, dstO, data, n, C, ld, rad, sws_img, dws, ws_data, W, nanflag);
                    case 40: return launch_boxqf_ks<40, MODE, 8>(r, srcW, gap, dstW, dstO, data, n, C, ld, rad, sws_img, dws, ws_data, W, nanflag);
                    case 48: return launch_boxqf_ks<48, MODE, 8>(r, srcW, gap, dstW, dstO, data, n, C, ld, rad, sws_img, dws, ws_data, W, nanflag);
#if BOXQF_B8_MAX2R > 56
                    case 56: return launch_boxqf_ks<56, MODE, 8>(r, srcW, gap, dstW, dstO, data, n, C, ld, rad, sws_img, dws, ws_data, W, nanflag);
                    case 64: return launch_boxqf_ks<64, MODE, 8>(r, srcW, gap, dstW, dstO, data, n, C, ld, rad, sws_img, dws, ws_data, W, nanflag);
#endif
#if BOXQF_B8_MAX2R > 72
                    case 72: return launch_boxqf_ks<72, MODE, 8>(r, srcW, gap, dstW, dstO, data, n, C, ld, rad, sws_img, dws, ws_data, W, nanflag);
                    case 80:
                        if (MODE == 1) return launch_boxqf_ks<80, 1, 8>(r, srcW, gap, dstW, dstO, data, n, C, ld, rad, sws_img, dws, ws_data, W, nanflag);
                        break;
#endif
#if BOXQF_B8_MAX2R > 88
                    case 96: return launch_boxqf_ks<96, MODE, 8>(r, srcW, gap, dstW, dstO, data, n, C, ld, rad, sws_img, dws, ws_data, W, nanflag);
#endif
                }
            }
            switch (kq) {
                case 16: return launch_boxqf_ks<16, MODE>(r, srcW, gap, dstW, dstO, data, n, C, ld, rad, sws_img, dws, ws_data, W, nanflag);
                case 32: return launch_boxqf_ks<32, MODE>(r, srcW, gap, dstW, dstO, data, n, C, ld, rad, sws_img, dws, ws_data, W, nanflag);
                case 48: return launch_boxqf_ks<48, MODE>(r, srcW, gap, dstW, dstO, data, n, C, ld, rad, sws_img, dws, ws_data, W, nanflag);
                case 64: return launch_boxqf_ks<64, MODE>(r, srcW, gap, dstW, dstO, data, n, C, ld, rad, sws_img, dws, ws_data, W, nanflag);
                case 80: return launch_boxqf_ks<80, MODE>(r, srcW, gap, dstW, dstO, data, n, C, ld, rad, sws_img, dws, ws_data, W, nanflag);
                case 96: return launch_boxqf_ks<96, MODE>(r, srcW, gap, dstW, dstO, data, n, C, ld, rad, sws_img, dws, ws_data, W, nanflag);
            }
        }
    }
    switch (ks) {
        case 8: return launch_boxf_ks<8, MODE>(r, srcW, srcO, dstW, dstO, data, n, C, ld, rad, sws_img, dws, ws_data, W, nanflag, dstP, pws, wroteP);
        case 16: return launch_boxf_ks<16, MODE>(r, srcW, srcO, dstW, dstO, data, n, C, ld, rad, sws_img, dws, ws_data, W, nanflag, dstP, pws, wroteP);
        case 32: return launch_boxf_ks<32, MODE>(r, srcW, srcO, dstW, dstO, data, n, C, ld, rad, sws_img, dws, ws_data, W, nanflag, dstP, pws, wroteP);
        case 64: return launch_boxf_ks<64, MODE>(r, srcW, srcO, dstW, dstO, data, n, C, ld, rad, sws_img, dws, ws_data, W, nanflag, dstP, pws, wroteP);
        case 80: return launch_boxf_ks<80, MODE>(r, srcW, srcO, dstW, dstO, data, n, C, ld, rad, sws_img, dws, ws_data, W, nanflag, dstP, pws, wroteP);
    }
    return set_err(TRI_EINVAL, "no register-ring kernel for %d slots", ks);
}

thread_local int g_boxx_override = -1;
thread_local unsigned long long g_boxx_last_stats[2] = {0, 0};
#ifndef BOXX_MIN_R
#define BOXX_MIN_R 56
#endif
int boxx_pick_l(int rad, int n) {
    static const bool env_off = is1(getenv("TRI_FILTER_NO_EXACT"));
    static const int force_nti = [] { const char* e = getenv("TRI_BOXX_NTI"); return e ? atoi(e) : 0; }();
    if (g_boxx_override == 0 || (g_boxx_override < 0 && (env_off || rad < BOXX_MIN_R))) return 0;
    if (rad < 1 || n % 4 != 0) return 0;
    const int64_t P = (int64_t)n + 4 * (int64_t)rad;
    struct Cand { int nti, l; };
    static const Cand cands[] = {{128, 37}, {128, 41}, {256, 17}, {256, 19}, {256, 21}, {256, 25}};
    for (const Cand& c : cands) {
        if (force_nti && c.nti != force_nti) continue;
        if (c.nti == 128 && (P <= 128 * 17 || rad < 64)) continue;
        if ((int64_t)c.nti * c.l < P || c.l > 2 * rad + 1 || (2 * rad + 1) / c.l > BOXX_AMAX) continue;
        if (boxx_lds_bytes(c.nti, c.l, rad) > 159 * 1024) continue;
        return c.l | (c.nti << 8);
    }
    return 0;
}
static bool boxx_recip_ok(int rad) { return rad <= 128 || rad == 166 || rad == 221 || rad == 277 || rad == 397 || rad == 795; }

template <int NTI, int L, int MODE>
int launch_boxx_l(const Run& r, const float* srcW, unsigned gap, const float* data, const uint8_t* mask, float* outA, float* outB,
                  int n, int C, int ld, int rad, size_t sws_img, size_t ws_data, size_t ws_mask, size_t ws_outA, size_t ws_outB,
                  int64_t W, uint8_t* nanflag, unsigned long long* stats) {
    const BoxDenom denom = box_reciprocal(box_denominator(rad));
    const size_t lds = boxx_lds_bytes(NTI, L, rad);
    dim3 grid((unsigned)C, (unsigned)W);
    const auto k = boxx_recip_ok(rad) ? &k_boxx<NTI, L, MODE, true> : &k_boxx<NTI, L, MODE, false>;
    HIPCHK(lds_optin_all(159 * 1024, k));
    hipLaunchKernelGGL(k, grid, dim3(2 * NTI), lds, r.st, srcW, gap, data, mask, outA, outB, n, ld, rad, denom, sws_img,
                       ws_data, ws_mask, ws_outA, ws_outB, nanflag, stats);
    LAUNCHCHK();
    return TRI_OK;
}
template <int MODE>
int launch_boxx(const Run& r, int L, const float* srcW, const float* srcO, const float* data, const uint8_t* mask, float* outA, float* outB,
                int n, int C, int ld, int rad, size_t sws_img, size_t ws_data, size_t ws_mask, size_t ws_outA, size_t ws_outB,
                int64_t W, uint8_t* nanflag, unsigned long long* stats = nullptr) {
    if (srcO <= srcW || ld % 4 != 0 || sws_img % 4 != 0 || (uint64_t)(srcO - srcW) % 4 != 0 || ((uintptr_t)srcW % 16 != 0) ||
        ((uintptr_t)data % 16 != 0) || ws_data % 4 != 0 || ((uintptr_t)outA % 16 != 0) || ws_outA % 4 != 0 ||
        (mask && (((uintptr_t)mask % 4 != 0) || ws_mask % 4 != 0)) || (uint64_t)(srcO - srcW) > 0xffffffffull ||
        (MODE == 2 && (((uintptr_t)outB % 16 != 0) || ws_outB % 4 != 0)) || C > 65535 * 1024)
        return set_err(TRI_EUNSUPPORTED, "exact row filter: unaligned images");
    const unsigned gap = (unsigned)(srcO - srcW);
#define BOXX_CASE(NTI, LL) case ((NTI) << 8 | (LL)): return launch_boxx_l<NTI, LL, MODE>(r, srcW, gap, data, mask, outA, outB, n, C, ld, rad, sws_img, ws_data, ws_mask, ws_outA, ws_outB, W, nanflag, stats);
    switch (L) {
        BOXX_CASE(128, 37) BOXX_CASE(128, 41)
        BOXX_CASE(256, 17) BOXX_CASE(256, 19) BOXX_CASE(256, 21) BOXX_CASE(256, 25)
    }
#undef BOXX_CASE
    return set_err(TRI_EINVAL, "no exact row filter for code %d", L);
}

bool colfilter_t4_usable(int rad) { return !filter_no_tin() && colfilter_use_lane4(rad); }

int launch_colfilter_t4(const Run& r, const float* srcW, const float* srcO, float* dstW, float* dstO,
                        int n, int C, int ld, int rad, size_t sws_img, size_t dws, int64_t W, float* deferred_denom) {
    float denom = box_denominator(rad);
    size_t lds = ((size_t)lane4_ring_capacity(rad) * 64 + 32 * 17) * sizeof(float);
    HIPCHK(lds_optin_all(160 * 1024, &k_colfilter_lane4<3, false>, &k_colfilter_lane4<3, true>));
    dim3 grid((unsigned)cdiv(C, 16), (unsigned)W, 2);
    if (deferred_denom) *deferred_denom = denom;
    const auto k = deferred_denom ? &k_colfilter_lane4<3, false> : &k_colfilter_lane4<3, true>;
    hipLaunchKernelGGL(k, grid, dim3(64), lds, r.st, srcW, srcO, (const float*)nullptr, (const uint8_t*)nullptr,
                       dstW, dstO, n, C, rad, denom, sws_img, (size_t)ld, dws);
    LAUNCHCHK();
    return TRI_OK;
}

int spectrum_medians(const Run& r, const float* img, const uint8_t* flg) {
    const Plan& pl = r.pl;
    const Ws& ws = r.ws;
    const int Fa = (int)pl.Fa, Wn = (int)r.Wb, G = (int)pl.G;
    int rc = launch_transpose<float>(r, img, ws.srowsf, Fa, Wn, 0, 0, 1);
    if (rc) return rc;
    rc = launch_transpose<uint8_t>(r, flg, ws.srowsu, Fa, Wn, 0, 0, 1);
    if (rc) return rc;
    bool seg4 = Fa % 4 == 0;
    for (int64_t g = 0; g < pl.G + 1 && seg4; g++) seg4 = r.p->chunk_ends[g] % 4 == 0;
    MedianJob j;
    j.data = ws.srowsf; j.flags = ws.srowsu; j.med = ws.smed; j.RS = (size_t)Fa;
    j.seg_start = ws.segC_start; j.seg_len = ws.segC_len; j.R = Wn; j.G = G; j.W = 1; j.max_len = pl.maxchunk;
    j.vec_ok = j.segs_aligned = seg4; j.rows_aligned = Fa % 4 == 0;
    return launch_median(r, j);
}

int spectrum_background(const Run& r) {
    const Plan& pl = r.pl;
    const Ws& ws = r.ws;
    int Fa = (int)pl.Fa, Wn = (int)r.Wb, G = (int)pl.G;
    size_t nS = (size_t)Fa * Wn;
    hipLaunchKernelGGL(k_copy_u8, dim3((unsigned)cdiv(nS, 256)), dim3(256), 0, r.st, ws.sflags, ws.sbgf, nS);
    LAUNCHCHK();
    double rej = TRI_MAD_NORMAL * r.p->background_reject;
    bool rowD_valid = false;
    for (int ext = pl.nit; ext >= 0; ext--) {
        bool final_pass = ext == 0;
        double sigma = (double)(final_pass ? 1 : ext) * r.p->spike_width_freq;
        int rad = (int)box_radius(sigma);
        const int xl = (rad > 0 && 2 * (size_t)pl.PT >= 4) ? boxx_pick_l(rad, Fa) : 0;
        if (xl > 0) {
            float* rowW = ws.Aw;
            float* rowO = ws.Aw + nS;
            float* rowD = ws.Aw + 2 * nS;
            float* rowR = ws.Aw + 3 * nS;
            hipLaunchKernelGGL(k_build_wo, grid1(nS, 1), dim3(256), 0, r.st, ws.sdata, ws.sbgf, ws.sw, ws.so, nS, (size_t)0, (size_t)0);
            LAUNCHCHK();
            int rc = launch_transpose<float>(r, ws.sw, rowW, Fa, Wn, 0, 0, 1);
            if (!rc) rc = launch_transpose<float>(r, ws.so, rowO, Fa, Wn, 0, 0, 1);
            if (!rc && !rowD_valid) rc = launch_transpose<float>(r, ws.sdata, rowD, Fa, Wn, 0, 0, 1);
            if (rc) return rc;
            rowD_valid = true;
            if (final_pass)
                rc = launch_boxx<2>(r, xl, rowW, rowO, rowD, nullptr, rowR, rowW, Fa, Wn, Fa, rad, 0, 0, 0, 0, 0, 1, reinterpret_cast<uint8_t*>(ws.rowcnt));
            else
                rc = launch_boxx<1>(r, xl, rowW, rowO, rowD, nullptr, rowR, nullptr, Fa, Wn, Fa, rad, 0, 0, 0, 0, 0, 1, nullptr);
            if (!rc) rc = launch_transpose<float>(r, rowR, ws.so, Wn, Fa, 0, 0, 1);
            if (rc) return rc;
            if (!final_pass) {
                rc = spectrum_medians(r, ws.so, ws.sbgf);
                if (rc) return rc;
                hipLaunchKernelGGL(k_reject<false>, grid1(nS, 1), dim3(256), 0, r.st, ws.so, ws.sbgf, ws.smed, ws.d_chunk_of, rej, Fa, Wn, G, (size_t)0, (size_t)0);
                LAUNCHCHK();
            }
            continue;
        }
        if (rad > 0) {
            int rc = launch_colfilter(r, ColSrc::ByteFlags, ws.sw, ws.so, ws.sdata, ws.sbgf, ws.sw, ws.so, Fa, Wn, rad, 0, 0, 0, 1, COL_WEIGHTS_01);
            if (rc) return rc;
        } else {
            hipLaunchKernelGGL(k_build_wo, grid1(nS, 1), dim3(256), 0, r.st, ws.sdata, ws.sbgf, ws.sw, ws.so, nS, (size_t)0, (size_t)0);
            LAUNCHCHK();
        }
        if (final_pass) {
            { int rc2 = launch_masked_div<0>(r, ws.sw, ws.so, ws.sdata, nS, 0, 0, 1); if (rc2) return rc2; }
        } else {
            { int rc2 = launch_masked_div<1>(r, ws.sw, ws.so, ws.sdata, nS, 0, 0, 1); if (rc2) return rc2; }
            int rc = spectrum_medians(r, ws.so, ws.sbgf);
            if (rc) return rc;
            hipLaunchKernelGGL(k_reject<false>, grid1(nS, 1), dim3(256), 0, r.st, ws.so, ws.sbgf, ws.smed, ws.d_chunk_of, rej, Fa, Wn, G, (size_t)0, (size_t)0);
            LAUNCHCHK();
        }
    }
    return launch_interp(r, ws.so, Fa, Wn, (size_t)0, 1, (const uint8_t*)nullptr, (const float*)nullptr, (size_t)0, (float*)nullptr);
}

static bool bg_flags_packed(int T, size_t N) {
    static const bool no_pack = is1(getenv("TRI_NO_PACKED_FLAGS"));
    return !no_pack && (T % 4 == 0) && (N % 4 == 0);
}


enum class TimeStage {
    BuildOnly,
    PackedSweep,
    Prebuilt,
    PrebuiltDirectFT,
    ByteFlags
};
enum class FreqStage {
    ExactRows,
    FusedRing,
    FusedLds,
    LdsDiv,
    Lane4Div,
    Transposed
};
enum class Reject {
    None,
    InRows,
    Tile,
    OnePass,
    MedianReject4T,
    MedianReject4,
    MedianReject
};

struct FreqPick {
    FreqStage route;
    int ks;
    int xl;
    size_t off;
};
static FreqPick pick_freq_unfused(int rad, int C) {
    return {FreqStage::Transposed, 0, 0, colfilter_lds_block(rad, C) > 0 ? 0 : (size_t)4 * rad * C};
}
static FreqPick pick_freq_stage(int rad, int n, int C, size_t gap, bool exact_rows) {
    const int ks = ((uint64_t)gap + (uint64_t)n * C) * 4u < (1ull << 31) ? boxr_pick_ks_f(rad) : 0;
    const int xl = (rad > 0 && (!ks || rad >= BOXX_MIN_R) && exact_rows) ? boxx_pick_l(rad, n) : 0;
    if (xl > 0) return {FreqStage::ExactRows, 0, xl, 0};
    if (ks > 0) return {FreqStage::FusedRing, ks, 0, 0};
    if (colfilter_tf_usable(rad)) return {FreqStage::FusedLds, 0, 0, 0};
    if (colfilter_t_usable(rad)) return {FreqStage::LdsDiv, 0, 0, 0};
    if (colfilter_t4_usable(rad)) return {FreqStage::Lane4Div, 0, 0, 0};
    return pick_freq_unfused(rad, C);
}

struct TileRoute { bool use; size_t ccap, ucap; int ytiles; };
static int medrej_force_fallback() { static const int v = [] { const char* e = getenv("TRI_MEDREJ_FORCE_FALLBACK"); return e ? atoi(e) : 0; }(); return v; }
static bool no_fused_reject() { static const bool v = is1(getenv("TRI_NO_FUSED_REJECT")); return v; }
static bool fused_medrej() { static const bool v = is1(getenv("TRI_FUSED_MEDREJ")); return v; }
static TileRoute pick_tile_route(const Run& r, bool packed) {
    const Plan& pl = r.pl;
    static const bool no_tile = is1(getenv("TRI_NO_TILE_MEDREJ"));
    const int T = (int)pl.T, G = (int)pl.G;
    const size_t wsA = 2 * (size_t)pl.PT * pl.Fa, wsB = (size_t)pl.PF * T;
    const size_t mr_nb = (size_t)pl.maxchunk * T;
    TileRoute t = {false, (mr_nb / 4) & ~(size_t)3, (mr_nb / 8) & ~(size_t)3, 0};
    for (int g = 0; g < G; g++) t.ytiles += (int)cdiv(r.p->chunk_ends[g + 1] - r.p->chunk_ends[g], 64);
    t.use = pl.vec && wsB % 4 == 0 && wsA % 4 == 0 && packed && !no_fused_reject() && !no_tile && !fused_medrej() && G <= 65535 &&
            mrt_scratch_words(G, t.ccap, t.ucap) <= wsA && (medrej_force_fallback() || (pl.maxchunk - 1) * (int64_t)T >= 65536) &&
            t.ytiles > 0 && t.ytiles <= 65535;
    return t;
}
static unsigned medrej_capq(size_t wsA, int G) {
    const size_t per_block = (wsA / (size_t)G) & ~(size_t)7;
    return (unsigned)std::min<size_t>(per_block / 2, 0x3ffffffcu);
}

struct BgStep {
    int r0, r1;
    bool final_pass;
    TimeStage time;
    bool time_needs_bytes;
    bool time_defers;
    FreqPick freq;
    bool freq_transposes;
    Reject reject;
    bool reads_ft_flags;
};

static BgStep pick_bg_step(const Run& r, bool packed, bool tile_route, int ext) {
    const Plan& pl = r.pl;
    const int T = (int)pl.T, Fa = (int)pl.Fa, G = (int)pl.G;
    const size_t wsA = 2 * (size_t)pl.PT * Fa, wsB = (size_t)pl.PF * T;
    BgStep s;
    s.final_pass = ext == 0;
    const double e = (double)(s.final_pass ? 1 : ext);
    s.r0 = (int)box_radius(e * r.p->spike_width_time);
    s.r1 = (int)box_radius(e * r.p->spike_width_freq);

    static const bool prebuild = [] { const char* e = getenv("TRI_TIME_PREBUILD"); return !(e && e[0] == '0'); }();
    const bool sweep = s.r0 > 0 && colfilter_lds_block(s.r0, Fa) > 0;
    if (s.r0 == 0) s.time = TimeStage::BuildOnly;
    else if (sweep && packed) s.time = TimeStage::PackedSweep;
    else if (sweep && prebuild) {
        static const bool want_direct = is1(getenv("TRI_FILTER_DIRECT_FT"));
        s.time = (want_direct && T % 4 == 0 && wsB % 4 == 0) ? TimeStage::PrebuiltDirectFT : TimeStage::Prebuilt;
    } else s.time = TimeStage::ByteFlags;
    s.time_needs_bytes = packed && (s.time == TimeStage::BuildOnly || s.time == TimeStage::ByteFlags);

    s.freq = s.time == TimeStage::PrebuiltDirectFT ? pick_freq_unfused(s.r1, T)
                                                   : pick_freq_stage(s.r1, Fa, T, (size_t)(r.ws.Ao - r.ws.Aw), !r.ampl_cached || r.data_mask);
    s.freq_transposes = s.time != TimeStage::PrebuiltDirectFT;
    s.time_defers = s.freq.route == FreqStage::Transposed;

    static const bool no_tfr = is1(getenv("TRI_FILTER_NO_TF_REJECT"));
    const bool vec4 = pl.vec && wsB % 4 == 0;
    if (s.final_pass) s.reject = Reject::None;
    else if (s.freq.route == FreqStage::ExactRows && packed && !no_tfr && G <= 65535 && (uint64_t)T * Fa * 4u < (1ull << 31))
        s.reject = Reject::InRows;
    else if (tile_route) s.reject = Reject::Tile;
    else if (vec4 && wsA % 4 == 0 && packed && !no_fused_reject() && fused_medrej() && medrej_capq(wsA, G) >= 1024 && G <= 65535 &&
             (uint64_t)T * Fa * 4u < (1ull << 32))
        s.reject = Reject::OnePass;
    else if (vec4 && packed && !no_fused_reject()) s.reject = Reject::MedianReject4T;
    else s.reject = vec4 ? Reject::MedianReject4 : Reject::MedianReject;
    s.reads_ft_flags = s.time_needs_bytes || (!s.final_pass && s.reject != Reject::InRows);
    return s;
}

struct BgImages {
    int T, Fa;
    int64_t W;
    const float *dataTF, *dataFT;
    const uint8_t* flagsTF;
    uint8_t* comb;
    float *Aw, *Ao; size_t wsA;
    float *Bw, *Bo; size_t wsB;
    float* rows; size_t ws_rows;
    const uint8_t* mask; size_t ws_mask;
    uint8_t* nanflag;
    float* residP;
    unsigned long long* xstats;
};

struct BgState {
    uint8_t *cur_ft, *alt_ft;
    bool bgf_ft_stale;
    bool wrote_panel;
};

static int bg_time_stage(const Run& r, const BgStep& s, const BgImages& im, const BgState& st, float* den_t) {
    const int T = im.T, Fa = im.Fa;
    const size_t N = (size_t)T * Fa;
    const int64_t W = im.W;
    int rc = TRI_OK;
    *den_t = 0.0f;
    float* const defer = s.time_defers ? den_t : nullptr;
    const uint8_t* fl = im.flagsTF;
    if (s.time_needs_bytes) {
        rc = launch_transpose<uint8_t>(r, st.cur_ft, im.comb, Fa, T, N, N, W);
        if (rc) return rc;
        fl = im.comb;
    }
    switch (s.time) {
        case TimeStage::BuildOnly:
            hipLaunchKernelGGL(k_build_wo, grid1(N, W), dim3(256), 0, r.st, im.dataTF, fl, im.Aw, im.Ao, N, N, im.wsA);
            LAUNCHCHK();
            return TRI_OK;
        case TimeStage::PackedSweep:
            return launch_colfilter(r, ColSrc::PackedFlags, im.Aw, im.Ao, im.dataTF, fl, im.Aw, im.Ao, T, Fa, s.r0, im.wsA, N, im.wsA, W, COL_WEIGHTS_01, defer);
        case TimeStage::Prebuilt:
        case TimeStage::PrebuiltDirectFT:
            if (N % 4 == 0 && im.wsA % 4 == 0)
                hipLaunchKernelGGL(k_build_wo4, grid1(N / 4, W), dim3(256), 0, r.st, im.dataTF, fl, im.Aw, im.Ao, N / 4, N, im.wsA);
            else
                hipLaunchKernelGGL(k_build_wo, grid1(N, W), dim3(256), 0, r.st, im.dataTF, fl, im.Aw, im.Ao, N, N, im.wsA);
            LAUNCHCHK();
            if (s.time == TimeStage::Prebuilt)
                return launch_colfilter(r, ColSrc::Images, im.Aw, im.Ao, nullptr, nullptr, im.Aw, im.Ao, T, Fa, s.r0, im.wsA, 0, im.wsA, W, COL_WEIGHTS_01, defer);
            return launch_colfilter(r, ColSrc::Images, im.Aw, im.Ao, nullptr, nullptr, im.Bw + s.freq.off, im.Bo + s.freq.off, T, Fa, s.r0, im.wsA, 0, im.wsB, W, COL_TRANSPOSED_OUT);
        case TimeStage::ByteFlags:
            return launch_colfilter(r, ColSrc::ByteFlags, im.Aw, im.Ao, im.dataTF, fl, im.Aw, im.Ao, T, Fa, s.r0, im.wsA, N, im.wsA, W);
    }
    return set_err(TRI_EINVAL, "internal: no such time stage");
}

template <int MODE>
static int bg_freq_stage_mode(const Run& r, const BgStep& s, const BgImages& im, BgState& st, float den_t) {
    const int T = im.T, Fa = im.Fa, r1 = s.r1;
    const size_t N = (size_t)T * Fa, wsA = im.wsA, wsB = im.wsB;
    const int64_t W = im.W;
    uint8_t* const nan = MODE == 2 ? im.nanflag : nullptr;
    float den_f = 0.0f;
    int rc = TRI_OK;
    if (MODE == 2) HIPCHK(hipMemsetAsync(im.nanflag, 0, (size_t)W * T, r.st));
    switch (s.freq.route) {
        case FreqStage::ExactRows:
            rc = launch_boxx<MODE>(r, s.freq.xl, im.Aw, im.Ao, im.dataTF, im.mask, im.rows, MODE == 2 ? im.Aw : nullptr, Fa, T, Fa, r1, wsA, N,
                                   im.ws_mask, im.ws_rows, MODE == 2 ? wsA : 0, W, nan, im.xstats);
            if (!rc && MODE == 2) rc = launch_transpose<float>(r, im.Aw, im.Bw, T, Fa, wsA, wsB, W);
            if (rc || s.reject == Reject::InRows) return rc;
            return launch_transpose<float>(r, im.rows, im.Bo, T, Fa, im.ws_rows, wsB, W);
        case FreqStage::FusedRing:
            return launch_boxf<MODE>(r, s.freq.ks, im.Aw, im.Ao, im.Bw, im.Bo, im.dataFT, Fa, T, Fa, r1, wsA, wsB, N, W, nan,
                                     MODE == 2 ? im.residP : nullptr, MODE == 2 ? N : 0, &st.wrote_panel);
        case FreqStage::FusedLds:
            return launch_colfilter_tf<MODE>(r, im.Aw, im.Ao, im.Bw, im.Bo, im.dataFT, Fa, T, Fa, r1, wsA, wsB, N, W, nan);
        case FreqStage::LdsDiv:
            rc = launch_colfilter_t(r, im.Aw, im.Ao, im.Bw, im.Bo, Fa, T, Fa, r1, wsA, wsB, W, &den_f);
            break;
        case FreqStage::Lane4Div:
            rc = launch_colfilter_t4(r, im.Aw, im.Ao, im.Bw, im.Bo, Fa, T, Fa, r1, wsA, wsB, W, &den_f);
            break;
        case FreqStage::Transposed:
            if (s.freq_transposes) {
                rc = launch_transpose<float>(r, im.Aw, im.Bw + s.freq.off, T, Fa, wsA, wsB, W, den_t);
                if (!rc) rc = launch_transpose<float>(r, im.Ao, im.Bo + s.freq.off, T, Fa, wsA, wsB, W, den_t);
            }
            if (!rc && r1 > 0) rc = launch_colfilter(r, ColSrc::Images, im.Bw, im.Bo, nullptr, nullptr, im.Bw, im.Bo, Fa, T, r1, wsB, 0, wsB, W, 0, &den_f);
            break;
    }
    if (rc) return rc;
    return launch_masked_div<MODE>(r, im.Bw, im.Bo, im.dataFT, N, wsB, N, W, den_f, nan, MODE == 2 ? T : 1);
}
static int bg_freq_stage(const Run& r, const BgStep& s, const BgImages& im, BgState& st, float den_t) {
    return s.final_pass ? bg_freq_stage_mode<2>(r, s, im, st, den_t) : bg_freq_stage_mode<1>(r, s, im, st, den_t);
}

static int bg_reject_stage(const Run& r, const BgStep& s, const TileRoute& tile, bool packed, BgState& st) {
    const Plan& pl = r.pl;
    const Ws& ws = r.ws;
    const int T = (int)pl.T, Fa = (int)pl.Fa, G = (int)pl.G;
    const int64_t W = r.Wb;
    const size_t N = (size_t)T * Fa, wsA = 2 * (size_t)pl.PT * Fa, wsB = (size_t)pl.PF * T;
    const double rej = TRI_MAD_NORMAL * r.p->background_reject;
    if (s.reject == Reject::None) return TRI_OK;
    if (s.reject != Reject::Tile && st.cur_ft == ws.flagsFT)
        return set_err(TRI_EUNSUPPORTED, "internal: background flags read in place on a route that rewrites them");
    switch (s.reject) {
        case Reject::InRows: {
            unsigned* gc = reinterpret_cast<unsigned*>(ws.Aw);
            unsigned cap = (unsigned)(std::min<size_t>((wsA / 2) / (size_t)G, 0x7fffffffu) & ~(size_t)3);
            if (median_no_predict() || (int64_t)cap < pl.maxchunk * pl.T || wsA % 4 != 0) { gc = nullptr; cap = 0; }
            hipLaunchKernelGGL((k_median2<false, true>), dim3((unsigned)G, (unsigned)W), dim3(256), 0, r.st, (const float*)ws.Ao,
                               (const uint8_t*)ws.bgfTF, ws.med, wsA, N, (size_t)0, (size_t)1, ws.segC_start, ws.segC_len, 1, G,
                               gc, gc ? wsA : (size_t)0, cap, T / 4, Fa);
            hipLaunchKernelGGL(k_reject_tf, dim3((unsigned)cdiv(Fa, 256), (unsigned)(T / 4), (unsigned)W), dim3(256), 0, r.st,
                               (const float*)ws.Ao, reinterpret_cast<unsigned*>(ws.bgfTF), ws.med, ws.d_chunk_of, rej, T / 4, Fa, Fa, G,
                               wsA, N / 4);
            LAUNCHCHK();
            st.bgf_ft_stale = true;
            return TRI_OK;
        }
        case Reject::Tile: {
            unsigned* sc = reinterpret_cast<unsigned*>(ws.Aw);
            hipLaunchKernelGGL(k_mr_predict, dim3((unsigned)G, (unsigned)W), dim3(256), 0, r.st, (const float*)ws.Bo, (const uint8_t*)st.cur_ft,
                               ws.d_chunk_ends, rej, T / 4, G, wsB, N, sc, wsA, tile.ccap, tile.ucap, medrej_force_fallback());
            for (unsigned round = 1; round <= 2; round++) {
                hipLaunchKernelGGL(k_mr_pass, dim3((unsigned)cdiv(T / 4, 64), (unsigned)tile.ytiles, (unsigned)W), dim3(256), 0, r.st, (const float*)ws.Bo,
                                   (const uint8_t*)st.cur_ft, st.alt_ft, ws.bgfTF, ws.d_chunk_ends, Fa, T / 4, G, wsB, N, sc, wsA, tile.ccap, tile.ucap, round);
                hipLaunchKernelGGL(k_mr_finish, dim3((unsigned)G, (unsigned)W), dim3(256), 0, r.st, (const float*)ws.Bo, (const uint8_t*)st.cur_ft, st.alt_ft,
                                   ws.bgfTF, ws.med, ws.d_chunk_ends, rej, Fa, T / 4, G, wsB, N, sc, wsA, tile.ccap, tile.ucap, round);
            }
            hipLaunchKernelGGL(k_median_reject, dim3((unsigned)G, (unsigned)W), dim3(256), 0, r.st, (const float*)ws.Bo, (const uint8_t*)st.cur_ft,
                               st.alt_ft, ws.bgfTF, ws.med, ws.d_chunk_ends, rej, Fa, T / 4, G, wsB, N, sc, wsA, 0u, 0u, 1,
                               (const unsigned*)sc, wsA, (int)MRT_PARW, 11);
            LAUNCHCHK();
            std::swap(st.cur_ft, st.alt_ft);
            if (st.alt_ft == ws.flagsFT) st.alt_ft = ws.fflFT;
            return TRI_OK;
        }
        case Reject::OnePass: {
            const unsigned capq = medrej_capq(wsA, G);
            hipLaunchKernelGGL(k_median_reject, dim3((unsigned)G, (unsigned)W), dim3(256), 0, r.st, (const float*)ws.Bo, (const uint8_t*)st.cur_ft,
                               st.alt_ft, ws.bgfTF, ws.med, ws.d_chunk_ends, rej, Fa, T / 4, G, wsB, N,
                               reinterpret_cast<unsigned*>(ws.Aw), wsA, capq, capq, medrej_force_fallback());
            LAUNCHCHK();
            std::swap(st.cur_ft, st.alt_ft);
            return TRI_OK;
        }
        default:
            break;
    }
    MedianJob j;
    j.data = ws.Bo; j.flags = st.cur_ft; j.med = ws.med; j.WSd = wsB; j.WSf = N;
    j.seg_start = ws.segB_start; j.seg_len = ws.segB_len; j.R = 1; j.G = G; j.W = W; j.max_len = pl.maxchunk * pl.T;
    j.vec_ok = T % 4 == 0 && wsB % 4 == 0 && N % 4 == 0;
    j.gcand = reinterpret_cast<unsigned*>(ws.Aw); j.cand_ws = wsA;
    j.cand_cap = (unsigned)(std::min<size_t>(wsA / (size_t)G, 0x7fffffffu) & ~(size_t)3);
    const int rc = launch_median(r, j);
    if (rc) return rc;
    if (s.reject == Reject::MedianReject4T) {
        hipLaunchKernelGGL(k_reject4_t, dim3((unsigned)cdiv(T / 4, 64), (unsigned)cdiv(Fa, 64), (unsigned)W), dim3(64, 4), 0, r.st,
                           ws.Bo, st.cur_ft, ws.bgfTF, ws.med, ws.d_chunk_of, rej, Fa, T / 4, G, wsB, N);
        LAUNCHCHK();
        return TRI_OK;
    }
    if (s.reject == Reject::MedianReject4)
        hipLaunchKernelGGL(k_reject4, grid1(N / 4, W), dim3(256), 0, r.st, ws.Bo, st.cur_ft, ws.med, ws.d_chunk_of, rej, T / 4, G, N / 4, wsB, N);
    else
        hipLaunchKernelGGL(k_reject<true>, grid1(N, W), dim3(256), 0, r.st, ws.Bo, st.cur_ft, ws.med, ws.d_chunk_of, rej, Fa, T, G, wsB, N);
    LAUNCHCHK();
    if (packed) return launch_transpose<float>(r, reinterpret_cast<const float*>(st.cur_ft), reinterpret_cast<float*>(ws.bgfTF), Fa, T / 4, N / 4, N / 4, W);
    return launch_transpose<uint8_t>(r, st.cur_ft, ws.bgfTF, Fa, T, N, N, W);
}

int background2d(const Run& r, bool flagsFT_current, float* residP = nullptr, bool* wroteP = nullptr) {
    const Plan& pl = r.pl;
    const Ws& ws = r.ws;
    const int T = (int)pl.T, Fa = (int)pl.Fa;
    const int64_t W = r.Wb;
    const size_t N = (size_t)T * Fa;
    const bool packed = bg_flags_packed(T, N);
    const TileRoute tile = pick_tile_route(r, packed);
    static const bool copy_flags = is1(getenv("TRI_BG_COPY_FLAGS"));
    bool flags_in_place = flagsFT_current && !copy_flags && packed && tile.use;
    for (int ext = pl.nit; ext >= 1 && flags_in_place; ext--)
        if (pick_bg_step(r, packed, tile.use, ext).freq.route == FreqStage::ExactRows) flags_in_place = false;
    int rc = TRI_OK;
    if (!flags_in_place)
        rc = flagsFT_current ? launch_u8<0>(r, ws.flagsFT, ws.bgfFT, N, N, N, W)
                             : launch_transpose<uint8_t>(r, ws.flagsTF, ws.bgfFT, T, Fa, N, N, W);
    if (rc) return rc;
    if (packed)
        rc = launch_transpose<float>(r, reinterpret_cast<const float*>(flags_in_place ? ws.flagsFT : ws.bgfFT), reinterpret_cast<float*>(ws.bgfTF), Fa, T / 4, N / 4, N / 4, W);
    else
        rc = launch_u8<0>(r, ws.flagsTF, ws.bgfTF, N, N, N, W);
    if (rc) return rc;

    BgImages im;
    im.T = T; im.Fa = Fa; im.W = W;
    im.dataTF = ws.dataTF; im.dataFT = ws.dataFT;
    im.flagsTF = ws.bgfTF; im.comb = ws.comb;
    im.Aw = ws.Aw; im.Ao = ws.Ao; im.wsA = 2 * (size_t)pl.PT * Fa;
    im.Bw = ws.Bw; im.Bo = ws.Bo; im.wsB = (size_t)pl.PF * T;
    im.rows = ws.Ao; im.ws_rows = im.wsA;
    im.mask = r.ampl_cached ? r.data_mask : nullptr; im.ws_mask = r.data_mask_ws;
    im.nanflag = reinterpret_cast<uint8_t*>(ws.rowcnt);
    im.residP = residP; im.xstats = nullptr;
    BgState st = {flags_in_place ? ws.flagsFT : ws.bgfFT, flags_in_place ? ws.bgfFT : ws.fflFT, false, false};
    for (int ext = pl.nit; ext >= 0; ext--) {
        const BgStep s = pick_bg_step(r, packed, tile.use, ext);
        if (st.bgf_ft_stale && s.reads_ft_flags) {
            rc = launch_transpose<float>(r, reinterpret_cast<const float*>(ws.bgfTF), reinterpret_cast<float*>(st.cur_ft), T / 4, Fa, N / 4, N / 4, W);
            if (rc) return rc;
            st.bgf_ft_stale = false;
        }
        float den_t = 0.0f;
        rc = bg_time_stage(r, s, im, st, &den_t);
        if (!rc) rc = bg_freq_stage(r, s, im, st, den_t);
        if (!rc) rc = bg_reject_stage(r, s, tile, packed, st);
        if (rc) return rc;
    }
    if (wroteP) *wroteP = st.wrote_panel;
    return launch_interp(r, ws.Bo, Fa, T, im.wsB, W, reinterpret_cast<const uint8_t*>(ws.rowcnt), (const float*)ws.dataFT, N, ws.Bw,
                         st.wrote_panel ? residP : nullptr, N);
}


enum class Begin {
    FusedCached,
    Cached,
    Prepare4,
    Prepare
};
enum class SpecOr {
    Scalar,
    Rows16,
    FtInPlace,
    FtInPlaceDeferTf
};
enum class ChunkFlags {
    ExtraSources,
    OrMore16,
    OrBytes
};
enum class Finish {
    FusedDilate,
    Combine16Dilate,
    Combine16,
    Combine
};
enum class FinalKernel {
    NanMask16,
    Vis16,
    Scalar
};
struct IterStep {
    Begin begin; SpecOr spec_or; ChunkFlags chunk_flags; Finish finish; FinalKernel final_kernel;
    bool panel;
    bool fused_resid;
    int lo, hi, flo, fhi;
    bool ft_current() const { return spec_or == SpecOr::FtInPlace || spec_or == SpecOr::FtInPlaceDeferTf; }
};

static void smear_extents(int64_t e, int* lo, int* hi) {
    const int64_t half = e >= 0 ? e / 2 : -((-e + 1) / 2);
    *lo = (int)-half; *hi = (int)(-half + e);
}
static bool st_no_panel() { static const bool off = is1(getenv("TRI_ST_NO_PANEL")); return off; }

static IterStep pick_iteration(const Run& r) {
    const Plan& pl = r.pl;
    const int T = (int)pl.T, F = (int)pl.F, Fa = (int)pl.Fa;
    const size_t N = (size_t)T * Fa;
    static const bool no_fused_begin = is1(getenv("TRI_NO_FUSED_BEGIN"));
    static const bool no_ft_or = is1(getenv("TRI_NO_FT_SPEC_OR"));
    static const bool no_fused_or = is1(getenv("TRI_NO_FUSED_OR"));
    static const bool no_fused_dilate = is1(getenv("TRI_NO_FUSED_DILATE"));
    static const bool no_fused_resid = [] { const char* e = getenv("TRI_NO_FUSED_RESID_TF"); return !(e && e[0] == '0'); }();
    IterStep s;
    smear_extents(r.p->time_extend, &s.lo, &s.hi);
    smear_extents(r.p->freq_extend, &s.flo, &s.fhi);
    if (!r.ampl_cached) s.begin = pl.vec ? Begin::Prepare4 : Begin::Prepare;
    else s.begin = (!no_fused_begin && T % 4 == 0 && Fa % 4 == 0 && N % 4 == 0 && (uintptr_t)r.ws.iter % 4 == 0) ? Begin::FusedCached : Begin::Cached;
    if (!pl.vec) s.spec_or = SpecOr::Scalar;
    else if (no_ft_or || T % 16 != 0) s.spec_or = SpecOr::Rows16;
    else s.spec_or = bg_flags_packed(T, N) ? SpecOr::FtInPlaceDeferTf : SpecOr::FtInPlace;
    const bool defer_tf = s.spec_or == SpecOr::FtInPlaceDeferTf;
    if (defer_tf && !no_fused_or && median_takes_extra_flags(pl.maxchunk) && Fa % 4 == 0) s.chunk_flags = ChunkFlags::ExtraSources;
    else s.chunk_flags = defer_tf ? ChunkFlags::OrMore16 : ChunkFlags::OrBytes;
    if (!pl.vec) s.finish = Finish::Combine;
    else if (s.flo != -1 || s.fhi != 2) s.finish = Finish::Combine16;
    else s.finish = no_fused_dilate ? Finish::Combine16Dilate : Finish::FusedDilate;
    s.final_kernel = !pl.vec ? FinalKernel::Scalar : r.ampl_cached ? FinalKernel::NanMask16 : FinalKernel::Vis16;
    s.panel = !st_no_panel() && s.chunk_flags == ChunkFlags::ExtraSources && s.finish == Finish::FusedDilate && Fa % 64 == 0 && Fa == F &&
              median_takes_extra_flags(pl.maxchunk + 3) && st_use_fused(pl.swT) && st_use_mask(T, Fa);
    s.fused_resid = s.panel && !no_fused_resid;
    return s;
}

template <int VD>
static int launch_prepare(const Run& r, const IterStep& s, const void* vis) {
    const Plan& pl = r.pl;
    const Ws& ws = r.ws;
    const size_t N = (size_t)pl.T * pl.Fa, W = (size_t)r.Wb;
    if (s.begin == Begin::Prepare4)
        hipLaunchKernelGGL(k_prepare4<VD>, dim3((unsigned)cdiv(N * W / 4, 256)), dim3(256), 0, r.st, vis, ws.iter, ws.dataTF, ws.flagsTF, N * W / 4);
    else
        hipLaunchKernelGGL(k_prepare<VD>, grid1(N, W), dim3(256), 0, r.st, vis, ws.iter, ws.dataTF, ws.flagsTF, (int)pl.T, (int)pl.F, (int)pl.Fa, (int)pl.avg);
    LAUNCHCHK();
    return TRI_OK;
}
template <int VD>
static int launch_final(const Run& r, const IterStep& s, const void* vis, uint8_t* out_flags, bool update_iter) {
    const Ws& ws = r.ws;
    const int T = (int)r.pl.T, F = (int)r.pl.F, upd = update_iter ? 1 : 0;
    const size_t NF = (size_t)T * F, W = (size_t)r.Wb;
    const double row_limit = r.p->flag_all_freq_frac * (double)F, col_limit = (double)T * r.p->flag_all_time_frac;
    if (s.final_kernel == FinalKernel::NanMask16)
        hipLaunchKernelGGL(k_final16<TRI_VIS_NANMASK>, grid1(NF / 16, W), dim3(256), 0, r.st, ws.dil, ws.rowcnt, ws.colcnt, (const void*)ws.nanmask, out_flags, ws.iter, T, F / 16, row_limit, col_limit, upd);
    else if (s.final_kernel == FinalKernel::Vis16)
        hipLaunchKernelGGL(k_final16<VD>, grid1(NF / 16, W), dim3(256), 0, r.st, ws.dil, ws.rowcnt, ws.colcnt, vis, out_flags, ws.iter, T, F / 16, row_limit, col_limit, upd);
    else
        hipLaunchKernelGGL(k_final<VD>, grid1(NF, W), dim3(256), 0, r.st, ws.dil, ws.rowcnt, ws.colcnt, vis, out_flags, ws.iter, T, F, row_limit, col_limit, upd);
    LAUNCHCHK();
    return TRI_OK;
}
#define BY_VIS_DTYPE(FN, ...) \
    (vis_dtype == TRI_VIS_C64 ? FN<TRI_VIS_C64>(__VA_ARGS__) : vis_dtype == TRI_VIS_F64 ? FN<TRI_VIS_F64>(__VA_ARGS__) : FN<TRI_VIS_F32>(__VA_ARGS__))

static int iter_begin(const Run& r, const IterStep& s, const void* vis, int vis_dtype) {
    const Ws& ws = r.ws;
    const int T = (int)r.pl.T, Fa = (int)r.pl.Fa;
    const size_t N = (size_t)T * Fa;
    const int64_t W = r.Wb;
    int rc = TRI_OK;
    switch (s.begin) {
        case Begin::FusedCached:
            hipLaunchKernelGGL((k_transpose_u8w<true, true>), dim3((unsigned)cdiv(Fa, 64), (unsigned)cdiv(T, 128), (unsigned)W), dim3(256), 0, r.st,
                               ws.iter, ws.flagsFT, ws.flagsTF, ws.dataFT, T, Fa, N, N, N, N);
            break;
        case Begin::Cached:
            rc = launch_u8<0>(r, ws.iter, ws.flagsTF, N, N, N, W);
            if (!rc) rc = launch_transpose<uint8_t>(r, ws.flagsTF, ws.flagsFT, T, Fa, N, N, W);
            if (rc) return rc;
            hipLaunchKernelGGL(k_zero_flagged4, grid1(N / 4, W), dim3(256), 0, r.st, ws.flagsFT, ws.dataFT, N / 4, N, N);
            break;
        case Begin::Prepare4:
        case Begin::Prepare:
            rc = BY_VIS_DTYPE(launch_prepare, r, s, vis);
            if (!rc) rc = launch_transpose<float>(r, ws.dataTF, ws.dataFT, T, Fa, N, N, W);
            if (!rc) rc = launch_transpose<uint8_t>(r, ws.flagsTF, ws.flagsFT, T, Fa, N, N, W);
            return rc;
    }
    LAUNCHCHK();
    return TRI_OK;
}

static int time_medians(const Run& r, const float* dataFT, size_t ws_data) {
    const Ws& ws = r.ws;
    const int T = (int)r.pl.T, Fa = (int)r.pl.Fa;
    MedianJob j;
    j.data = dataFT; j.flags = ws.flagsFT; j.med = ws.med; j.WSd = ws_data; j.WSf = (size_t)T * Fa; j.RS = (size_t)T;
    j.seg_start = ws.segT_start; j.seg_len = ws.segT_len; j.R = Fa; j.G = 1; j.W = r.Wb; j.max_len = r.pl.T;
    j.rows_aligned = T % 4 == 0; j.segs_aligned = true;
    return launch_median(r, j);
}

static int iter_spectrum(const Run& r, const IterStep& s) {
    const Ws& ws = r.ws;
    const int T = (int)r.pl.T, Fa = (int)r.pl.Fa, Wn = (int)r.Wb;
    const size_t N = (size_t)T * Fa, nS = (size_t)Fa * Wn;
    const int64_t W = r.Wb;
    int rc = time_medians(r, ws.dataFT, N);
    if (rc) return rc;
    hipLaunchKernelGGL(k_spec_from_med, dim3((unsigned)cdiv(nS, 256)), dim3(256), 0, r.st, ws.med, ws.sdata, ws.sflags, Fa, Wn);
    LAUNCHCHK();
    rc = spectrum_background(r);
    if (!rc) rc = launch_sub(r, ws.sdata, ws.so, ws.sres, nS, 0, 0, 0, 1);
    if (!rc) rc = spectrum_medians(r, ws.sres, ws.sflags);
    if (!rc) rc = launch_colst(r, r.pl.swF, ws.sres, ws.smed, ws.sout, ws.d_chunk_ends, Fa, Wn, (int)r.pl.G, 0, 0, 1);
    if (rc) return rc;
    if (s.spec_or != SpecOr::Scalar)
        hipLaunchKernelGGL(k_spec_rows, dim3((unsigned)cdiv(nS, 256)), dim3(256), 0, r.st, ws.sout, ws.srows, Fa, Wn);
    switch (s.spec_or) {
        case SpecOr::Scalar:
            hipLaunchKernelGGL(k_or_spec, grid1(N, W), dim3(256), 0, r.st, ws.flagsTF, ws.sout, T, Fa, Wn);
            break;
        case SpecOr::Rows16:
            hipLaunchKernelGGL(k_or_spec16, grid1(N / 16, W), dim3(256), 0, r.st, ws.flagsTF, ws.srows, T, Fa / 16);
            break;
        case SpecOr::FtInPlace:
            hipLaunchKernelGGL(k_or_spec16, grid1(N / 16, W), dim3(256), 0, r.st, ws.flagsTF, ws.srows, T, Fa / 16);
            hipLaunchKernelGGL(k_or_spec_ft16, grid1(N / 16, W), dim3(256), 0, r.st, ws.flagsFT, ws.srows, T / 16, Fa);
            break;
        case SpecOr::FtInPlaceDeferTf:
            hipLaunchKernelGGL(k_or_spec_ft16, grid1(N / 16, W), dim3(256), 0, r.st, ws.flagsFT, ws.srows, T / 16, Fa);
            break;
    }
    LAUNCHCHK();
    return TRI_OK;
}

static int iter_residual(const Run& r, const IterStep& s, const float** residTF) {
    const Ws& ws = r.ws;
    const int T = (int)r.pl.T, Fa = (int)r.pl.Fa;
    bool wrote_panel = false;
    const int rc = background2d(r, s.ft_current(), s.fused_resid ? ws.residP : nullptr, &wrote_panel);
    *residTF = wrote_panel ? ws.residP : ws.Aw;
    if (rc || wrote_panel) return rc;
    return launch_transpose<float>(r, ws.Bw, ws.Aw, Fa, T, (size_t)r.pl.PF * T, (size_t)T * Fa, r.Wb, 0.0f, s.panel);
}

static int iter_sumthreshold(const Run& r, const IterStep& s, const float* residTF) {
    const Plan& pl = r.pl;
    const Ws& ws = r.ws;
    const int T = (int)pl.T, Fa = (int)pl.Fa, G = (int)pl.G;
    const size_t N = (size_t)T * Fa, wsB = (size_t)pl.PF * T;
    const int64_t W = r.Wb;
    int rc = s.ft_current() ? TRI_OK : launch_transpose<uint8_t>(r, ws.flagsTF, ws.flagsFT, T, Fa, N, N, W);
    if (!rc) rc = time_medians(r, ws.Bw, wsB);
    if (!rc) rc = launch_colst(r, pl.swT, residTF, ws.med, ws.tflTF, ws.d_tends, T, Fa, 1, N, N, W, s.panel);
    if (rc) return rc;
    MedianJob cj;
    cj.data = residTF; cj.flags = ws.flagsTF; cj.med = ws.med; cj.WSd = cj.WSf = N; cj.RS = (size_t)Fa;
    cj.seg_start = ws.segC_start; cj.seg_len = ws.segC_len; cj.R = T; cj.G = G; cj.W = W; cj.max_len = pl.maxchunk;
    cj.rows_aligned = Fa % 4 == 0;
    switch (s.chunk_flags) {
        case ChunkFlags::ExtraSources:
            cj.flags2 = ws.tflTF; cj.colflags = ws.srows; cj.WScol = (size_t)Fa; cj.panel_rows = s.panel ? T : 0;
            break;
        case ChunkFlags::OrMore16:
            hipLaunchKernelGGL(k_or_spec_more16, grid1(N / 16, W), dim3(256), 0, r.st, ws.flagsTF, ws.srows, ws.tflTF, T, Fa / 16);
            LAUNCHCHK();
            break;
        case ChunkFlags::OrBytes:
            rc = launch_u8<1>(r, ws.tflTF, ws.flagsTF, N, N, N, W);
            break;
    }
    if (!rc) rc = launch_median(r, cj);
    if (!rc) rc = launch_colst(r, pl.swF, ws.Bw, ws.med, ws.fflFT, ws.d_chunk_ends, Fa, T, G, wsB, N, W);
    if (!rc) rc = launch_transpose<uint8_t>(r, ws.fflFT, ws.fflTF, Fa, T, N, N, W);
    return rc;
}

static int iter_taps(const Run& r, const IterStep& s, const float* residTF) {
    const Ws& ws = r.ws;
    const int T = (int)r.pl.T, Fa = (int)r.pl.Fa, Wn = (int)r.Wb;
    const size_t N = (size_t)T * Fa;
    const Debug& d = *r.dbg;
    hipLaunchKernelGGL(k_gather_col_f32, dim3((unsigned)cdiv(Fa, 256)), dim3(256), 0, r.st, ws.sres, d.f32, Fa, Wn, 0);
    hipLaunchKernelGGL(k_gather_col_u8, dim3((unsigned)cdiv(Fa, 256)), dim3(256), 0, r.st, ws.sout, d.u8, Fa, Wn, 0);
    if (s.panel) {
        hipLaunchKernelGGL(k_unpanel<float>, dim3((unsigned)cdiv(N, 256)), dim3(256), 0, r.st, residTF, d.f32 + Fa + N, T, Fa);
        hipLaunchKernelGGL(k_unpanel<uint8_t>, dim3((unsigned)cdiv(N, 256)), dim3(256), 0, r.st, (const uint8_t*)ws.tflTF, d.u8 + Fa, T, Fa);
    } else {
        HIPCHK(hipMemcpyAsync(d.f32 + Fa + N, residTF, N * sizeof(float), hipMemcpyDeviceToDevice, r.st));
        HIPCHK(hipMemcpyAsync(d.u8 + Fa, ws.tflTF, N, hipMemcpyDeviceToDevice, r.st));
    }
    LAUNCHCHK();
    HIPCHK(hipMemcpyAsync(d.f32 + Fa, ws.Bo, N * sizeof(float), hipMemcpyDeviceToDevice, r.st));
    HIPCHK(hipMemcpyAsync(d.u8 + Fa + N, ws.fflTF, N, hipMemcpyDeviceToDevice, r.st));
    return TRI_OK;
}

static int iter_finish(const Run& r, const IterStep& s, const void* vis, int vis_dtype, uint8_t* out_flags, bool update_iter) {
    const Ws& ws = r.ws;
    const int T = (int)r.pl.T, F = (int)r.pl.F, Fa = (int)r.pl.Fa, Wn = (int)r.Wb;
    const size_t N = (size_t)T * Fa;
    const int64_t W = r.Wb;
    const dim3 grid16((unsigned)cdiv(F / 16, 64), (unsigned)T, (unsigned)W);
    HIPCHK(hipMemsetAsync(ws.rowcnt, 0, (size_t)W * T * sizeof(int), r.st));
    switch (s.finish) {
        case Finish::FusedDilate:
            if (s.panel) hipLaunchKernelGGL(k_combine_dilate16<true>, grid16, dim3(64), 0, r.st, ws.srows, ws.tflTF, ws.fflTF, ws.dil, ws.rowcnt, T, F / 16, s.lo, s.hi);
            else hipLaunchKernelGGL(k_combine_dilate16<false>, grid16, dim3(64), 0, r.st, ws.srows, ws.tflTF, ws.fflTF, ws.dil, ws.rowcnt, T, F / 16, s.lo, s.hi);
            hipLaunchKernelGGL(k_colcount, grid1(F / 4, W), dim3(256), 0, r.st, ws.dil, ws.colcnt, T, F / 4);
            break;
        case Finish::Combine16Dilate:
            hipLaunchKernelGGL(k_combine16, grid1(N / 16, W), dim3(256), 0, r.st, ws.srows, ws.tflTF, ws.fflTF, ws.comb, T, Fa / 16, s.lo, s.hi);
            hipLaunchKernelGGL((k_unaverage16<-1, 3>), grid16, dim3(64), 0, r.st, ws.comb, ws.dil, ws.rowcnt, T, F / 16);
            hipLaunchKernelGGL(k_colcount, grid1(F / 4, W), dim3(256), 0, r.st, ws.dil, ws.colcnt, T, F / 4);
            break;
        case Finish::Combine16:
        case Finish::Combine:
            if (s.finish == Finish::Combine16)
                hipLaunchKernelGGL(k_combine16, grid1(N / 16, W), dim3(256), 0, r.st, ws.srows, ws.tflTF, ws.fflTF, ws.comb, T, Fa / 16, s.lo, s.hi);
            else
                hipLaunchKernelGGL(k_combine, grid1(N, W), dim3(256), 0, r.st, ws.sout, ws.tflTF, ws.fflTF, ws.comb, T, Fa, Wn, s.lo, s.hi);
            LAUNCHCHK();
            HIPCHK(hipMemsetAsync(ws.colcnt, 0, (size_t)W * F * sizeof(int), r.st));
            hipLaunchKernelGGL(k_unaverage, dim3((unsigned)cdiv(F, 256), (unsigned)T, (unsigned)W), dim3(256), 0, r.st, ws.comb, ws.dil, ws.rowcnt, ws.colcnt,
                               T, Fa, F, (int)r.pl.avg, s.flo, s.fhi);
            break;
    }
    LAUNCHCHK();
    return BY_VIS_DTYPE(launch_final, r, s, vis, out_flags, update_iter);
}
#undef BY_VIS_DTYPE

int run_iteration(const Run& r, const IterStep& s, const void* vis, int vis_dtype, uint8_t* out_flags, bool update_iter, bool tap) {
    const float* residTF = nullptr;
    int rc = iter_begin(r, s, vis, vis_dtype);
    if (!rc) rc = iter_spectrum(r, s);
    if (!rc) rc = iter_residual(r, s, &residTF);
    if (!rc) rc = iter_sumthreshold(r, s, residTF);
    if (!rc && tap && r.dbg) rc = iter_taps(r, s, residTF);
    if (!rc) rc = iter_finish(r, s, vis, vis_dtype, out_flags, update_iter);
    return rc;
}

int process_windows(Run& r, const void* vis, int vis_dtype, const uint8_t* flags, uint8_t* out_flags,
                    int64_t w_begin, int64_t w_end, int64_t T, int64_t F, void* wsp, size_t ws_bytes, bool tap_first) {
    const tri_params* p = r.p;
    Ws probe;
    carve(r.pl, 1, nullptr, 0, true, &probe);
    if (probe.total > ws_bytes)
        return set_err(TRI_EWORKSPACE, "workspace of %zu bytes is smaller than the %zu needed for one window", ws_bytes, probe.total);
    int64_t lo = 1, hi = std::min<int64_t>(w_end - w_begin, 16384);
    while (lo < hi) {
        int64_t mid = (lo + hi + 1) / 2;
        carve(r.pl, mid, nullptr, 0, true, &probe);
        if (probe.total <= ws_bytes) lo = mid; else hi = mid - 1;
    }
    const int64_t Wb = lo;
    carve(r.pl, Wb, wsp, ws_bytes, false, &r.ws);

    ChunkTab ct;
    ct.n = (int)p->n_chunk_ends;
    for (int i = 0; i < ct.n; i++) ct.ends[i] = p->chunk_ends[i];
    {
        int nthr = (int)std::max<int64_t>(r.pl.Fa, ct.n);
        hipLaunchKernelGGL(k_tables, dim3((unsigned)cdiv(nthr, 256)), dim3(256), 0, r.st, ct, (int)T, (int)r.pl.Fa,
                           r.ws.d_chunk_ends, r.ws.d_tends, r.ws.segC_start, r.ws.segC_len, r.ws.segB_start,
                           r.ws.segB_len, r.ws.segT_start, r.ws.segT_len, r.ws.d_chunk_of);
        LAUNCHCHK();
    }
    const size_t NF = (size_t)T * F;
    const size_t esz = (vis_dtype == TRI_VIS_C64 || vis_dtype == TRI_VIS_F64) ? 8 : 4;
    static const bool no_cache = is1(getenv("TRI_NO_AMPL_CACHE"));
    r.ampl_cached = r.pl.vec && !no_cache && p->num_major_iterations > 0;
    r.data_mask = (r.ampl_cached && r.pl.Fa == F) ? r.ws.iter : nullptr;
    r.data_mask_ws = (size_t)T * r.pl.Fa;
    const IterStep step = pick_iteration(r);
    int rc = TRI_OK;
    for (int64_t w0 = w_begin; w0 < w_end; w0 += Wb) {
        r.Wb = std::min(Wb, w_end - w0);
        const char* vis_b = (const char*)vis + (size_t)w0 * NF * esz;
        uint8_t* out_b = out_flags + (size_t)w0 * NF;
        rc = launch_u8<2>(r, flags + (size_t)w0 * NF, r.ws.iter, NF, NF, NF, r.Wb);
        if (rc) return rc;
        if (r.ampl_cached) {
            const size_t n4 = (size_t)r.Wb * NF / 4;
            if (vis_dtype == TRI_VIS_C64)
                hipLaunchKernelGGL(k_amplitude4<TRI_VIS_C64>, dim3((unsigned)cdiv(n4, 256)), dim3(256), 0, r.st, (const void*)vis_b, r.ws.dataTF, r.ws.iter, r.ws.nanmask, n4);
            else
                hipLaunchKernelGGL(k_amplitude4<TRI_VIS_F32>, dim3((unsigned)cdiv(n4, 256)), dim3(256), 0, r.st, (const void*)vis_b, r.ws.dataTF, r.ws.iter, r.ws.nanmask, n4);
            LAUNCHCHK();
            rc = launch_transpose<float>(r, r.ws.dataTF, r.ws.dataFT, (int)T, (int)r.pl.Fa, NF, NF, r.Wb);
            if (rc) return rc;
        }
        for (int64_t it = 0; it < p->num_major_iterations; it++) {
            bool last = it == p->num_major_iterations - 1;
            bool tap = last && tap_first && w0 == w_begin;
            rc = run_iteration(r, step, vis_b, vis_dtype, out_b, !last, tap);
            if (rc) return rc;
        }
    }
    return TRI_OK;
}

struct SubStreams {
    hipStream_t st[2] = {nullptr, nullptr};
    hipEvent_t fork = nullptr, join[2] = {nullptr, nullptr};
    int device = -1;
};
thread_local SubStreams g_sub;

int get_substreams(SubStreams** out) {
    int dev = 0;
    HIPCHK(hipGetDevice(&dev));
    if (g_sub.device != dev) {
        if (g_sub.device >= 0) return set_err(TRI_EUNSUPPORTED, "a calling thread must stay on one device");
        int lo = 0, hi = 0;
        HIPCHK(hipDeviceGetStreamPriorityRange(&lo, &hi));
        HipStream st0, st1;
        HipEvent fork, join0, join1;
        HIPCHK(hipStreamCreateWithPriority(st0.out(), hipStreamNonBlocking, hi));
        HIPCHK(hipStreamCreateWithPriority(st1.out(), hipStreamNonBlocking, lo));
        HIPCHK(hipEventCreateWithFlags(fork.out(), hipEventDisableTiming));
        HIPCHK(hipEventCreateWithFlags(join0.out(), hipEventDisableTiming));
        HIPCHK(hipEventCreateWithFlags(join1.out(), hipEventDisableTiming));
        g_sub.st[0] = st0.release();
        g_sub.st[1] = st1.release();
        g_sub.fork = fork.release();
        g_sub.join[0] = join0.release();
        g_sub.join[1] = join1.release();
        g_sub.device = dev;
    }
    *out = &g_sub;
    return TRI_OK;
}

int flagger_impl(const void* vis, int vis_dtype, const uint8_t* flags, uint8_t* out_flags,
                 int64_t n_cp, int64_t T, int64_t F, const tri_params* p, void* workspace,
                 size_t workspace_bytes, void* stream, Debug* dbg) {
    if (!vis || !flags || !out_flags || !p) return set_err(TRI_EINVAL, "NULL pointer argument");
    if (n_cp < 0) return set_err(TRI_EINVAL, "negative window count");
    if (vis_dtype != TRI_VIS_C64 && vis_dtype != TRI_VIS_F32 && vis_dtype != TRI_VIS_F64)
        return set_err(TRI_EUNSUPPORTED, "vis dtype must be complex64, float32 or float64 amplitudes");
    Run r;
    r.st = (hipStream_t)stream;
    r.p = p;
    r.dbg = dbg;
    int rc = make_plan(T, F, p, &r.pl);
    if (rc) return rc;
    if (r.pl.G > TRI_MAX_CHUNKS) return set_err(TRI_EUNSUPPORTED, "at most %d frequency chunks", TRI_MAX_CHUNKS);
    if ((((uintptr_t)vis) | ((uintptr_t)flags) | ((uintptr_t)out_flags)) & 15) r.pl.vec = false;
    if (vis_dtype == TRI_VIS_F64) r.pl.vec = false;
    if (n_cp == 0) return TRI_OK;
    if (!workspace) return set_err(TRI_EWORKSPACE, "NULL workspace");
    if (((uintptr_t)workspace & 255) != 0) return set_err(TRI_EINVAL, "workspace must be 256-byte aligned");
    if (p->num_major_iterations == 0)
        HIPCHK(hipMemsetAsync(out_flags, 0, (size_t)n_cp * (size_t)T * F, r.st));

    const char* fe = getenv("TRI_SUBSTREAMS");
    const int force = fe ? atoi(fe) : -1;
    Ws probe;
    carve(r.pl, 1, nullptr, 0, true, &probe);
    const size_t half = (workspace_bytes / 2) & ~(size_t)255;
    const bool can_split = n_cp >= 2 && half >= probe.total && dbg == nullptr;
    const bool want_split = force == 1;
    if (!(can_split && want_split))
        return process_windows(r, vis, vis_dtype, flags, out_flags, 0, n_cp, T, F, workspace, workspace_bytes, true);

    SubStreams* ss = nullptr;
    rc = get_substreams(&ss);
    if (rc) return rc;
    HIPCHK(hipEventRecord(ss->fork, r.st));
    const int64_t mid = (n_cp + 1) / 2;
    for (int k = 0; k < 2 && rc == TRI_OK; k++) {
        Run rk;
        rk.st = ss->st[k];
        rk.p = p;
        rk.dbg = nullptr;
        rk.pl = r.pl;
        HIPCHK(hipStreamWaitEvent(rk.st, ss->fork, 0));
        rc = process_windows(rk, vis, vis_dtype, flags, out_flags, k == 0 ? 0 : mid, k == 0 ? mid : n_cp, T, F,
                             (char*)workspace + (size_t)k * half, half, false);
        (void)hipEventRecord(ss->join[k], rk.st);
        (void)hipStreamWaitEvent(r.st, ss->join[k], 0);
    }
    return rc;
}

}

extern "C" int tri_sum_threshold_flagger(const void* vis, int vis_dtype, const uint8_t* flags,
                                         uint8_t* out_flags, int64_t n_cp, int64_t ntime,
                                         int64_t nchan, const tri_params* p, void* workspace,
                                         size_t workspace_bytes, void* stream) {
    return flagger_impl(vis, vis_dtype, flags, out_flags, n_cp, ntime, nchan, p, workspace,
                        workspace_bytes, stream, nullptr);
}

extern "C" int tri_sum_threshold_flagger_debug(const void* vis, int vis_dtype, const uint8_t* flags,
                                               uint8_t* out_flags, int64_t n_cp, int64_t ntime,
                                               int64_t nchan, const tri_params* p, void* workspace,
                                               size_t workspace_bytes, void* stream,
                                               float* dbg_f32, uint8_t* dbg_u8) {
    Debug d{dbg_f32, dbg_u8};
    return flagger_impl(vis, vis_dtype, flags, out_flags, n_cp, ntime, nchan, p, workspace,
                        workspace_bytes, stream, (dbg_f32 && dbg_u8) ? &d : nullptr);
}

extern "C" int tri_abs_c64(const void* z, float* out, int64_t n, void* stream) {
    if (!z || !out || n < 0) return set_err(TRI_EINVAL, "bad argument");
    if (n == 0) return TRI_OK;
    hipLaunchKernelGGL(k_abs_c64, dim3((unsigned)cdiv(n, 256)), dim3(256), 0, (hipStream_t)stream, (const float2*)z, out, (size_t)n);
    LAUNCHCHK();
    return TRI_OK;
}

extern "C" int tri_fill_windows(void* vis_windows_c64, uint8_t* flag_windows, int64_t n, void* stream) {
    if (!vis_windows_c64 || !flag_windows || n < 0) return set_err(TRI_EINVAL, "bad argument");
    if (n == 0) return TRI_OK;
    hipLaunchKernelGGL(k_fill_windows, dim3((unsigned)cdiv(n, 256)), dim3(256), 0, (hipStream_t)stream, (float2*)vis_windows_c64, flag_windows, (size_t)n);
    LAUNCHCHK();
    return TRI_OK;
}

template <class Launch>
static int for_row_slabs(int64_t rows, int64_t nchan, int64_t ncorr, int64_t nbl, int64_t ntime, Launch&& launch) {
    if (rows == 0) return TRI_OK;
    if (rows > 0x7FFFFFFF || nchan > 0x7FFFFFFF || ncorr > 0x7FFFFFFF || nbl > 0x7FFFFFFF || ntime > 0x7FFFFFFF)
        return set_err(TRI_EUNSUPPORTED, "dimension too large for one call");
    for (int64_t r0 = 0; r0 < rows; r0 += 65535) {
        launch(r0, (unsigned)std::min<int64_t>(65535, rows - r0));
        LAUNCHCHK();
    }
    return TRI_OK;
}

extern "C" int tri_pack_data(const void* data_c64, const uint8_t* flag, const int32_t* row_bl,
                             const int32_t* row_time, int64_t rows, int64_t nchan, int64_t ncorr,
                             int64_t nbl, int64_t ntime, void* vis_windows_c64,
                             uint8_t* flag_windows, void* stream) {
    if (!data_c64 || !flag || !row_bl || !row_time || !vis_windows_c64 || !flag_windows)
        return set_err(TRI_EINVAL, "NULL pointer argument");
    if (rows < 0 || nchan <= 0 || ncorr <= 0 || nbl < 0 || ntime < 0) return set_err(TRI_EINVAL, "bad shape");
    const bool al = ((uintptr_t)data_c64 % 16 == 0) && ((uintptr_t)flag % 4 == 0);
    hipStream_t st = (hipStream_t)stream;
    return for_row_slabs(rows, nchan, ncorr, nbl, ntime, [&](int64_t r0, unsigned nr) {
        const dim3 grid((unsigned)cdiv(nchan, 256), nr, 1);
        const float2* dsl = (const float2*)data_c64 + (size_t)r0 * nchan * ncorr;
        const uint8_t* fsl = flag + (size_t)r0 * nchan * ncorr;
        if (ncorr == 4 && al)
            hipLaunchKernelGGL(k_pack_v<4>, grid, dim3(256), 0, st, dsl, fsl, row_bl + r0, row_time + r0,
                               (int)nchan, (int)nbl, (int)ntime, (float2*)vis_windows_c64, flag_windows);
        else if (ncorr == 2 && al)
            hipLaunchKernelGGL(k_pack_v<2>, grid, dim3(256), 0, st, dsl, fsl, row_bl + r0, row_time + r0,
                               (int)nchan, (int)nbl, (int)ntime, (float2*)vis_windows_c64, flag_windows);
        else if (ncorr == 1)
            hipLaunchKernelGGL(k_pack_v<1>, grid, dim3(256), 0, st, dsl, fsl, row_bl + r0, row_time + r0,
                               (int)nchan, (int)nbl, (int)ntime, (float2*)vis_windows_c64, flag_windows);
        else
            hipLaunchKernelGGL(k_pack, grid, dim3(256), 0, st, dsl, fsl,
                               row_bl + r0, row_time + r0, (int)nchan, (int)ncorr, (int)nbl, (int)ntime,
                               (float2*)vis_windows_c64, flag_windows);
    });
}

extern "C" int tri_unpack_data(const uint8_t* flag_windows, const int32_t* row_bl,
                               const int32_t* row_time, int64_t rows, int64_t nchan, int64_t ncorr,
                               int64_t nbl, int64_t ntime, uint8_t* out_flags, int any_corr,
                               void* stream) {
    if (!flag_windows || !row_bl || !row_time || !out_flags) return set_err(TRI_EINVAL, "NULL pointer argument");
    if (rows < 0 || nchan <= 0 || ncorr <= 0 || nbl < 0 || ntime < 0) return set_err(TRI_EINVAL, "bad shape");
    const bool al = (uintptr_t)out_flags % 4 == 0;
    hipStream_t st = (hipStream_t)stream;
    return for_row_slabs(rows, nchan, ncorr, nbl, ntime, [&](int64_t r0, unsigned nr) {
        const dim3 grid((unsigned)cdiv(nchan, 256), nr, 1);
        uint8_t* osl = out_flags + (size_t)r0 * nchan * ncorr;
        if (ncorr == 4 && al)
            hipLaunchKernelGGL(k_unpack_v<4>, grid, dim3(256), 0, st, flag_windows, row_bl + r0, row_time + r0,
                               (int)nchan, (int)nbl, (int)ntime, osl, any_corr);
        else if (ncorr == 2 && al)
            hipLaunchKernelGGL(k_unpack_v<2>, grid, dim3(256), 0, st, flag_windows, row_bl + r0, row_time + r0,
                               (int)nchan, (int)nbl, (int)ntime, osl, any_corr);
        else if (ncorr == 1)
            hipLaunchKernelGGL(k_unpack_v<1>, grid, dim3(256), 0, st, flag_windows, row_bl + r0, row_time + r0,
                               (int)nchan, (int)nbl, (int)ntime, osl, any_corr);
        else
            hipLaunchKernelGGL(k_unpack, grid, dim3(256), 0, st, flag_windows, row_bl + r0, row_time + r0,
                               (int)nchan, (int)ncorr, (int)nbl, (int)ntime, osl, any_corr);
    });
}

static bool fill_stokes_terms(StokesTerm* dst, const int32_t* idx, const double* alpha, int64_t cnt, int64_t ncorr) {
    for (int64_t k = 0; k < cnt; k++) {
        dst[k].c1 = idx[4 * k];
        dst[k].c2 = idx[4 * k + 1];
        dst[k].s1 = idx[4 * k + 2];
        dst[k].s2 = idx[4 * k + 3];
        dst[k].ar = alpha[2 * k];
        dst[k].ai = alpha[2 * k + 1];
        if (dst[k].c1 < 0 || dst[k].c1 >= ncorr || dst[k].c2 < 0 || dst[k].c2 >= ncorr) return false;
    }
    return true;
}

static int scan_stokes_terms(int mode, const int32_t* pol_idx, const double* pol_alpha, int64_t n_pol, int64_t ncorr,
                             StokesTerms& terms) {
    if (mode < 0 || mode > 2) return set_err(TRI_EINVAL, "mode must be 0 (standard), 1 (polarisation) or 2 (total_power)");
    terms.n_pol = 0;
    terms.n_unpol = 0;
    if (mode != 0) {
        if (n_pol <= 0) return set_err(TRI_EINVAL, "modes 1 and 2 need at least one stokes term");
        if (n_pol > TRI_MAX_STOKES_TERMS) return set_err(TRI_EUNSUPPORTED, "at most 4 stokes terms");
        if (!pol_idx || !pol_alpha) return set_err(TRI_EINVAL, "NULL pointer argument");
        terms.n_pol = (int)n_pol;
        if (!fill_stokes_terms(terms.pol, pol_idx, pol_alpha, n_pol, ncorr))
            return set_err(TRI_EINVAL, "correlation index out of range");
    }
    return TRI_OK;
}

extern "C" int tri_pack_scan(const void* data_c64, const void* model_c64, const uint8_t* flag,
                             const int32_t* row_bl, const int32_t* row_time, int64_t rows, int64_t nchan,
                             int64_t ncorr, int64_t nbl, int64_t ntime, int mode, const int32_t* pol_idx,
                             const double* pol_alpha, int64_t n_pol, void* vis_windows_c64,
                             uint8_t* flag_windows, void* stream) {
    if (!data_c64 || !row_bl || !row_time || !vis_windows_c64 || !flag_windows)
        return set_err(TRI_EINVAL, "NULL pointer argument");
    if (rows < 0 || nchan <= 0 || ncorr <= 0 || nbl < 0 || ntime < 0) return set_err(TRI_EINVAL, "bad shape");
    StokesTerms terms;
    if (const int rc = scan_stokes_terms(mode, pol_idx, pol_alpha, n_pol, ncorr, terms)) return rc;
    const bool stokes = mode != 0;
    const bool al = (uintptr_t)data_c64 % 16 == 0 && (uintptr_t)model_c64 % 16 == 0 && (uintptr_t)flag % 4 == 0;
    const bool vec = al && (ncorr == 4 || ncorr == 2 || ncorr == 1);
    hipStream_t st = (hipStream_t)stream;
    float2* vw = (float2*)vis_windows_c64;
    return for_row_slabs(rows, nchan, ncorr, nbl, ntime, [&](int64_t r0, unsigned nr) {
        const dim3 grid((unsigned)cdiv(nchan, 256), nr, 1);
        const size_t off = (size_t)r0 * nchan * ncorr;
        const float2* d = (const float2*)data_c64 + off;
        const float2* m = model_c64 ? (const float2*)model_c64 + off : nullptr;
        const uint8_t* fl = flag ? flag + off : nullptr;
        const int32_t* rb = row_bl + r0;
        const int32_t* rt = row_time + r0;
#define TRI_PACK_SCAN_V(NC, S)                                                                                      \
        do {                                                                                                         \
            if (m && fl)  hipLaunchKernelGGL((k_pack_scan_v<NC, S, true, true>), grid, dim3(256), 0, st, d, m, fl,   \
                                             rb, rt, (int)nchan, (int)nbl, (int)ntime, terms, vw, flag_windows);     \
            else if (m)   hipLaunchKernelGGL((k_pack_scan_v<NC, S, true, false>), grid, dim3(256), 0, st, d, m, fl,  \
                                             rb, rt, (int)nchan, (int)nbl, (int)ntime, terms, vw, flag_windows);     \
            else if (fl)  hipLaunchKernelGGL((k_pack_scan_v<NC, S, false, true>), grid, dim3(256), 0, st, d, m, fl,  \
                                             rb, rt, (int)nchan, (int)nbl, (int)ntime, terms, vw, flag_windows);     \
            else          hipLaunchKernelGGL((k_pack_scan_v<NC, S, false, false>), grid, dim3(256), 0, st, d, m, fl, \
                                             rb, rt, (int)nchan, (int)nbl, (int)ntime, terms, vw, flag_windows);     \
        } while (0)
        if (vec && ncorr == 4 && stokes) TRI_PACK_SCAN_V(4, true);
        else if (vec && ncorr == 4) TRI_PACK_SCAN_V(4, false);
        else if (vec && ncorr == 2 && stokes) TRI_PACK_SCAN_V(2, true);
        else if (vec && ncorr == 2) TRI_PACK_SCAN_V(2, false);
        else if (vec && ncorr == 1 && stokes) TRI_PACK_SCAN_V(1, true);
        else if (vec && ncorr == 1) TRI_PACK_SCAN_V(1, false);
        else
            hipLaunchKernelGGL(k_pack_scan, grid, dim3(256), 0, st, d, m, fl, rb, rt, (int)nchan, (int)ncorr,
                               (int)nbl, (int)ntime, stokes ? 1 : 0, terms, vw, flag_windows);
#undef TRI_PACK_SCAN_V
    });
}

extern "C" int tri_unpack_scan(const uint8_t* flag_windows, const int32_t* row_bl, const int32_t* row_time,
                               int64_t rows, int64_t nchan, int64_t wcorr, int64_t out_ncorr, int64_t nbl,
                               int64_t ntime, uint8_t* out_flags, void* stream) {
    if (!flag_windows || !row_bl || !row_time || !out_flags) return set_err(TRI_EINVAL, "NULL pointer argument");
    if (rows < 0 || nchan <= 0 || out_ncorr <= 0 || nbl < 0 || ntime < 0) return set_err(TRI_EINVAL, "bad shape");
    if (wcorr != 1 && wcorr != out_ncorr) return set_err(TRI_EINVAL, "wcorr must be 1 or out_ncorr");
    hipStream_t st = (hipStream_t)stream;
    return for_row_slabs(rows, nchan, out_ncorr, nbl, ntime, [&](int64_t r0, unsigned nr) {
        const dim3 grid((unsigned)cdiv(nchan, 256), nr, 1);
        uint8_t* osl = out_flags + (size_t)r0 * nchan * out_ncorr;
        if (out_ncorr == 4 && (uintptr_t)out_flags % 4 == 0)
            hipLaunchKernelGGL(k_unpack_scan<4>, grid, dim3(256), 0, st, flag_windows, row_bl + r0,
                               row_time + r0, (int)nchan, (int)wcorr, 4, (int)nbl, (int)ntime, osl);
        else
            hipLaunchKernelGGL(k_unpack_scan<0>, grid, dim3(256), 0, st, flag_windows, row_bl + r0,
                               row_time + r0, (int)nchan, (int)wcorr, (int)out_ncorr, (int)nbl, (int)ntime, osl);
    });
}

extern "C" int tri_pack_scan_rows(const void* data_c64, const void* model_c64, const uint8_t* flag,
                                  const int64_t* src_row, int64_t src_rows, const int32_t* row_bl,
                                  const int32_t* row_time, int64_t n, int64_t nchan, int64_t ncorr, int64_t nbl,
                                  int64_t ntime, int mode, const int32_t* pol_idx, const double* pol_alpha,
                                  int64_t n_pol, void* vis_windows_c64, uint8_t* flag_windows, void* stream) {
    if (!data_c64 || !row_bl || !row_time || !vis_windows_c64 || !flag_windows)
        return set_err(TRI_EINVAL, "NULL pointer argument");
    if (n < 0 || src_rows < 0 || nchan <= 0 || ncorr <= 0 || nbl < 0 || ntime < 0) return set_err(TRI_EINVAL, "bad shape");
    if (!src_row && n > src_rows) return set_err(TRI_EINVAL, "a list without src_row reads rows [0, n): n > src_rows");
    StokesTerms terms;
    if (const int rc = scan_stokes_terms(mode, pol_idx, pol_alpha, n_pol, ncorr, terms)) return rc;
    const bool stokes = mode != 0;
    const bool al = (uintptr_t)data_c64 % 16 == 0 && (uintptr_t)model_c64 % 16 == 0 && (uintptr_t)flag % 4 == 0;
    const bool vec = al && (ncorr == 4 || ncorr == 2 || ncorr == 1);
    hipStream_t st = (hipStream_t)stream;
    const float2* d = (const float2*)data_c64;
    const float2* m = (const float2*)model_c64;
    const uint8_t* fl = flag;
    float2* vw = (float2*)vis_windows_c64;
    return for_row_slabs(n, nchan, ncorr, nbl, ntime, [&](int64_t e0, unsigned nr) {
        const dim3 grid((unsigned)cdiv(nchan, 256), nr, 1);
#define TRI_PACK_SCAN_ROWS_V(NC, S)                                                                                 \
        do {                                                                                                         \
            if (m && fl)  hipLaunchKernelGGL((k_pack_scan_rows_v<NC, S, true, true>), grid, dim3(256), 0, st, d, m,  \
                                             fl, src_row, src_rows, row_bl, row_time, e0, (int)nchan, (int)nbl,      \
                                             (int)ntime, terms, vw, flag_windows);                                   \
            else if (m)   hipLaunchKernelGGL((k_pack_scan_rows_v<NC, S, true, false>), grid, dim3(256), 0, st, d, m, \
                                             fl, src_row, src_rows, row_bl, row_time, e0, (int)nchan, (int)nbl,      \
                                             (int)ntime, terms, vw, flag_windows);                                   \
            else if (fl)  hipLaunchKernelGGL((k_pack_scan_rows_v<NC, S, false, true>), grid, dim3(256), 0, st, d, m, \
                                             fl, src_row, src_rows, row_bl, row_time, e0, (int)nchan, (int)nbl,      \
                                             (int)ntime, terms, vw, flag_windows);                                   \
            else          hipLaunchKernelGGL((k_pack_scan_rows_v<NC, S, false, false>), grid, dim3(256), 0, st, d,   \
                                             m, fl, src_row, src_rows, row_bl, row_time, e0, (int)nchan, (int)nbl,   \
                                             (int)ntime, terms, vw, flag_windows);                                   \
        } while (0)
        if (vec && ncorr == 4 && stokes) TRI_PACK_SCAN_ROWS_V(4, true);
        else if (vec && ncorr == 4) TRI_PACK_SCAN_ROWS_V(4, false);
        else if (vec && ncorr == 2 && stokes) TRI_PACK_SCAN_ROWS_V(2, true);
        else if (vec && ncorr == 2) TRI_PACK_SCAN_ROWS_V(2, false);
        else if (vec && ncorr == 1 && stokes) TRI_PACK_SCAN_ROWS_V(1, true);
        else if (vec && ncorr == 1) TRI_PACK_SCAN_ROWS_V(1, false);
        else
            hipLaunchKernelGGL(k_pack_scan_rows, grid, dim3(256), 0, st, d, m, fl, src_row, src_rows, row_bl, row_time,
                               e0, (int)nchan, (int)ncorr, (int)nbl, (int)ntime, stokes ? 1 : 0, terms, vw,
                               flag_windows);
#undef TRI_PACK_SCAN_ROWS_V
    });
}

extern "C" int tri_unpack_scan_rows(const uint8_t* flag_windows, const int64_t* dst_row, int64_t out_rows,
                                    const int32_t* row_bl, const int32_t* row_time, int64_t n, int64_t nchan,
                                    int64_t wcorr, int64_t out_ncorr, int64_t nbl, int64_t ntime, uint8_t* out_flags,
                                    void* stream) {
    if (!flag_windows || !row_bl || !row_time || !out_flags) return set_err(TRI_EINVAL, "NULL pointer argument");
    if (n < 0 || out_rows < 0 || nchan <= 0 || out_ncorr <= 0 || nbl < 0 || ntime < 0)
        return set_err(TRI_EINVAL, "bad shape");
    if (wcorr != 1 && wcorr != out_ncorr) return set_err(TRI_EINVAL, "wcorr must be 1 or out_ncorr");
    if (!dst_row && n > out_rows) return set_err(TRI_EINVAL, "a list without dst_row writes rows [0, n): n > out_rows");
    hipStream_t st = (hipStream_t)stream;
    return for_row_slabs(n, nchan, out_ncorr, nbl, ntime, [&](int64_t e0, unsigned nr) {
        const dim3 grid((unsigned)cdiv(nchan, 256), nr, 1);
        if (out_ncorr == 4 && (uintptr_t)out_flags % 4 == 0)
            hipLaunchKernelGGL(k_unpack_scan_rows<4>, grid, dim3(256), 0, st, flag_windows, dst_row, out_rows, row_bl,
                               row_time, e0, (int)nchan, (int)wcorr, 4, (int)nbl, (int)ntime, out_flags);
        else
            hipLaunchKernelGGL(k_unpack_scan_rows<0>, grid, dim3(256), 0, st, flag_windows, dst_row, out_rows, row_bl,
                               row_time, e0, (int)nchan, (int)wcorr, (int)out_ncorr, (int)nbl, (int)ntime, out_flags);
    });
}

extern "C" int tri_bench_reject(const float* resid, const uint8_t* flags_in, uint8_t* flags_out, uint8_t* flags_t4, double* med,
                                int64_t n_win, int64_t n_chan, int64_t n_time, const int64_t* chunk_ends, int64_t n_chunk_ends,
                                double reject, int repeats, float* ms_per_step, void* stream) {
    if (!resid || !flags_in || !flags_out || !flags_t4 || !med || !chunk_ends || !ms_per_step) return set_err(TRI_EINVAL, "NULL pointer argument");
    if (n_win <= 0 || n_win > 65535 || n_chan <= 0 || n_time <= 0 || n_time % 4 != 0 || n_chunk_ends < 2 || n_chunk_ends > 256 || repeats <= 0)
        return set_err(TRI_EINVAL, "bad shape");
    if ((uint64_t)n_chan * (uint64_t)n_time * 4u >= (1ull << 31)) return set_err(TRI_EUNSUPPORTED, "a window of 2^31 bytes or more");
    const int G = (int)n_chunk_ends - 1, T = (int)n_time, Fa = (int)n_chan;
    int64_t maxchunk = 0, minchunk = n_chan;
    int ytiles = 0;
    for (int g = 0; g < G; g++) {
        const int64_t c = chunk_ends[g + 1] - chunk_ends[g];
        if (c <= 0 || chunk_ends[g] < 0 || chunk_ends[g + 1] > n_chan) return set_err(TRI_EINVAL, "bad chunk");
        maxchunk = std::max(maxchunk, c); minchunk = std::min(minchunk, c);
        ytiles += (int)cdiv(c, 64);
    }
    if (chunk_ends[0] != 0 || chunk_ends[G] != n_chan) return set_err(TRI_EINVAL, "chunks must cover the channels");
    if (minchunk * (int64_t)T < 65536 || ytiles > 65535) return set_err(TRI_EUNSUPPORTED, "blocks below 65536 samples take the two-kernel route");
    hipStream_t st = (hipStream_t)stream;
    const size_t N = (size_t)Fa * T;
    const size_t nb = (size_t)maxchunk * T, ccap = (nb / 4) & ~(size_t)3, ucap = (nb / 8) & ~(size_t)3;
    const size_t wsS = mrt_scratch_words(G, ccap, ucap);
    DevBuf<unsigned> scb;
    DevBuf<int64_t> endsb;
    HIPCHK(scb.alloc((size_t)n_win * wsS));
    HIPCHK(endsb.alloc((size_t)n_chunk_ends));
    unsigned* sc = scb.get();
    int64_t* d_ends = endsb.get();
    HIPCHK(hipMemcpyAsync(d_ends, chunk_ends, (size_t)n_chunk_ends * sizeof(int64_t), hipMemcpyHostToDevice, st));
    HIPCHK(hipStreamSynchronize(st));
    const double rej = TRI_MAD_NORMAL * reject;
    HipEvent e0, e1;
    HIPCHK(hipEventCreate(e0.out()));
    HIPCHK(hipEventCreate(e1.out()));
    const unsigned W = (unsigned)n_win;
    HIPCHK(hipEventRecord(e0.get(), st));
    for (int i = 0; i < repeats; i++) {
        hipLaunchKernelGGL(k_mr_predict, dim3((unsigned)G, W), dim3(256), 0, st, resid, flags_in, d_ends, rej, T / 4, G, N, N, sc, wsS, ccap, ucap, 0);
        for (unsigned round = 1; round <= 2; round++) {
            hipLaunchKernelGGL(k_mr_pass, dim3((unsigned)cdiv(T / 4, 64), (unsigned)ytiles, W), dim3(256), 0, st, resid, flags_in, flags_out, flags_t4,
                               d_ends, Fa, T / 4, G, N, N, sc, wsS, ccap, ucap, round);
            hipLaunchKernelGGL(k_mr_finish, dim3((unsigned)G, W), dim3(256), 0, st, resid, flags_in, flags_out, flags_t4, med, d_ends, rej, Fa, T / 4, G,
                               N, N, sc, wsS, ccap, ucap, round);
        }
        hipLaunchKernelGGL(k_median_reject, dim3((unsigned)G, W), dim3(256), 0, st, resid, flags_in, flags_out, flags_t4, med, d_ends, rej, Fa, T / 4, G,
                           N, N, sc, wsS, 0u, 0u, 1, (const unsigned*)sc, wsS, (int)MRT_PARW, 11);
    }
    HIPCHK(hipEventRecord(e1.get(), st));
    hipError_t le = hipGetLastError();
    hipError_t se = hipEventSynchronize(e1.get());
    float ms = 0.f;
    if (le == hipSuccess && se == hipSuccess) (void)hipEventElapsedTime(&ms, e0.get(), e1.get());
    if (le != hipSuccess) return set_err(TRI_EHIP, "launch: %s", hipGetErrorString(le));
    if (se != hipSuccess) return set_err(TRI_EHIP, "sync: %s", hipGetErrorString(se));
    *ms_per_step = ms / (float)repeats;
    return TRI_OK;
}

static int st_hook(const float* data, const double* mad, uint8_t* out, int64_t n_win, int64_t n_line, int64_t n_col,
                   const int64_t* windows, int64_t n_windows, double outlier_nsigma, double rho, int variant, int repeats,
                   float* ms_per_launch, void* stream, const int64_t* chunk_ends, int64_t n_chunk_ends, bool flagger_pick) {
    if (!data || !mad || !out || !windows || !ms_per_launch || !chunk_ends) return set_err(TRI_EINVAL, "NULL pointer argument");
    if (n_win <= 0 || n_line <= 0 || n_col <= 0 || repeats <= 0 || n_win > 65535) return set_err(TRI_EINVAL, "bad shape");
    if (n_chunk_ends < 2 || n_chunk_ends > 256) return set_err(TRI_EINVAL, "2 .. 256 chunk ends");
    for (int64_t g = 0; g < n_chunk_ends; g++)
        if (chunk_ends[g] < 0 || chunk_ends[g] > n_line || (g > 0 && chunk_ends[g] < chunk_ends[g - 1]))
            return set_err(TRI_EINVAL, "chunk ends must not decrease and must lie in [0, n_line]");
    const int G = (int)n_chunk_ends - 1;
    const int64_t o0 = chunk_ends[0], o1 = chunk_ends[G];
    hipStream_t st = (hipStream_t)stream;
    StWin sw;
    int rc = make_stwin(windows, n_windows, rho, &sw);
    if (rc) return rc;
    double thr_scale = outlier_nsigma * TRI_MAD_NORMAL;
    size_t nthreads = (size_t)n_win * n_col * G;
    int C = (int)n_col, L = (int)n_line;
    bool can_fuse = sw.nw == 4 && sw.w[0] == 1 && sw.w[1] == 2 && sw.w[2] == 4 && sw.w[3] == 8;
    if ((variant == 2 || variant == 3) && !can_fuse) return set_err(TRI_EUNSUPPORTED, "register cascade needs windows (1,2,4,8)");
    if (variant == 3 && !((uint64_t)L * (uint64_t)C * 4u < (1ull << 31)))
        return set_err(TRI_EUNSUPPORTED, "lane-mask cascade needs a window below 2^31 bytes");
    if (variant == 5 && !(can_fuse && C % 64 == 0 && (uint64_t)L * (uint64_t)C * 4u < (1ull << 31)))
        return set_err(TRI_EUNSUPPORTED, "panel SumThreshold: windows (1,2,4,8), a multiple of 64 columns, a window below 2^31 bytes");
    if (variant == 5 && G > 1) return set_err(TRI_EUNSUPPORTED, "panel SumThreshold: one chunk only (launch_colst never pairs a panel with chunks)");
    if (variant == 0 && can_fuse) variant = st_use_mask(L, C) ? ((G == 1 && C % 64 == 0 && !st_no_panel()) ? 5 : 3) : 2;
    if (variant == 0 && flagger_pick && st_use_pipe(sw)) variant = 4;
    if (variant == 4) {
        if (sw.nw > 8 || stp_lds_bytes(sw) > 160 * 1024) return set_err(TRI_EUNSUPPORTED, "stage pipeline: more than eight windows, or the flag ring does not fit LDS");
        HIPCHK(lds_optin_all(160 * 1024, &k_colst_pipe));
    }
    DevBuf<double> ring;
    DevBuf<uint8_t> acc;
    DevBuf<int64_t> d_ends;
    HIPCHK(ring.alloc(nthreads * sw.ringtot));
    HIPCHK(acc.alloc(nthreads * sw.acccap));
    HIPCHK(d_ends.alloc((size_t)n_chunk_ends));
    HIPCHK(hipMemcpyAsync(d_ends.get(), chunk_ends, (size_t)n_chunk_ends * sizeof(int64_t), hipMemcpyHostToDevice, st));
    HIPCHK(hipStreamSynchronize(st));
    HipEvent e0, e1;
    HIPCHK(hipEventCreate(e0.out()));
    HIPCHK(hipEventCreate(e1.out()));
    size_t ws = (size_t)n_line * n_col;
    DevBuf<float> pdata;
    DevBuf<uint8_t> pout;
    if (variant == 5) {
        HIPCHK(pdata.alloc((size_t)n_win * ws));
        HIPCHK(pout.alloc((size_t)n_win * ws));
        {
            ScopedSet<bool> pause(g_klog_on, false);
            hipLaunchKernelGGL(k_panelize<float>, dim3((unsigned)cdiv((int64_t)ws, 256), (unsigned)n_win), dim3(256), 0, st, data, pdata.get(), L, C, ws);
        }
        LAUNCHCHK();
    }
    const StKernel k = variant == 5 ? StKernel::MaskPanel : variant == 3 ? StKernel::Mask : variant == 2 ? StKernel::Fused :
                       variant == 4 ? StKernel::Pipe : StKernel::Dyn;
    const float* kdata = variant == 5 ? (const float*)pdata.get() : data;
    uint8_t* kout = variant == 5 ? pout.get() : out;
    HIPCHK(hipEventRecord(e0.get(), st));
    for (int i = 0; i < repeats; i++) {
        rc = st_launch(st, k, sw, kdata, mad, kout, d_ends.get(), thr_scale, L, C, G, ws, ws, n_win, ring.get(), acc.get());
        if (rc) return rc;
    }
    HIPCHK(hipEventRecord(e1.get(), st));
    HIPCHK(hipEventSynchronize(e1.get()));
    LAUNCHCHK();
    float ms = 0;
    HIPCHK(hipEventElapsedTime(&ms, e0.get(), e1.get()));
    *ms_per_launch = ms / repeats;
    if (variant == 5) {
        const bool whole = o0 == 0 && o1 == n_line;
        DevBuf<uint8_t> rows;
        if (!whole) HIPCHK(rows.alloc((size_t)n_win * ws));
        uint8_t* dst = whole ? out : rows.get();
        {
            ScopedSet<bool> pause(g_klog_on, false);
            hipLaunchKernelGGL(k_unpanel_w<uint8_t>, dim3((unsigned)cdiv((int64_t)ws, 256), (unsigned)n_win), dim3(256), 0, st, (const uint8_t*)pout.get(), dst, L, C, ws);
        }
        LAUNCHCHK();
        if (!whole && o1 > o0)
            for (int64_t w = 0; w < n_win; w++)
                HIPCHK(hipMemcpyAsync(out + (size_t)w * ws + (size_t)o0 * C, dst + (size_t)w * ws + (size_t)o0 * C, (size_t)(o1 - o0) * C,
                                      hipMemcpyDeviceToDevice, st));
        HIPCHK(hipStreamSynchronize(st));
    }
    return TRI_OK;
}

extern "C" int tri_bench_sumthreshold(const float* data, const double* mad, uint8_t* out,
                                      int64_t n_win, int64_t n_line, int64_t n_col,
                                      const int64_t* windows, int64_t n_windows,
                                      double outlier_nsigma, double rho, int variant, int repeats,
                                      float* ms_per_launch, void* stream) {
    const int64_t ends[2] = {0, n_line};
    return st_hook(data, mad, out, n_win, n_line, n_col, windows, n_windows, outlier_nsigma, rho, variant, repeats, ms_per_launch,
                   stream, ends, 2, false);
}

extern "C" int tri_test_sumthreshold(const float* data, const double* mad, uint8_t* out,
                                     int64_t n_win, int64_t n_line, int64_t n_col,
                                     const int64_t* windows, int64_t n_windows,
                                     double outlier_nsigma, double rho, int variant, int repeats,
                                     float* ms_per_launch, void* stream, const int64_t* chunk_ends, int64_t n_chunk_ends) {
    return st_hook(data, mad, out, n_win, n_line, n_col, windows, n_windows, outlier_nsigma, rho, variant, repeats, ms_per_launch,
                   stream, chunk_ends, n_chunk_ends, true);
}

struct RouteOverrides {
    const int r = g_boxr_override, w = g_boxw_override, p = g_boxp_override, q = g_boxq_override,
              q8 = g_boxq_b8_override, x = g_boxx_override;
    ~RouteOverrides() {
        g_boxr_override = r; g_boxw_override = w; g_boxp_override = p;
        g_boxq_override = q; g_boxq_b8_override = q8; g_boxx_override = x;
    }
};

extern "C" int tri_bench_boxfilter(const float* data, const uint8_t* flags4, float* out_w, float* out_o,
                                   int64_t n_win, int64_t n_line, int64_t n_col, int64_t radius,
                                   int stage, int variant, int repeats, float* ms_per_launch, void* stream) {
    if (!data || !flags4 || !out_w || !out_o || !ms_per_launch) return set_err(TRI_EINVAL, "NULL pointer argument");
    if (n_win <= 0 || n_line <= 0 || n_col <= 0 || repeats <= 0 || n_win > 65535 || radius <= 0 || (stage != 2 && n_line % 4 != 0))
        return set_err(TRI_EINVAL, "bad shape");
    if (stage < 0 || stage > 2) return set_err(TRI_EUNSUPPORTED, "stage must be 0, 1 or 2");
    if (variant < 0 || variant > 5 || (variant == 4 && stage != 1) || (variant == 5 && stage == 2))
        return set_err(TRI_EINVAL, "variant must be 0 .. 3 (4: exact row filter, stage 1 only; 5: stage pipeline with blocks of 16, stages 0 and 1)");
    if (stage == 2 && n_win != 1) return set_err(TRI_EINVAL, "the spectrum stage takes one window");
    Run r;
    r.st = (hipStream_t)stream;
    r.p = nullptr;
    r.dbg = nullptr;
    HipEvent e0, e1;
    HIPCHK(hipEventCreate(e0.out()));
    HIPCHK(hipEventCreate(e1.out()));
    const size_t N = (size_t)n_line * n_col;
    const RouteOverrides saved;
    ScopedSet<bool> unpadded(g_colfilter_unpadded, true);
    g_boxr_override = variant == 0 ? -1 : (variant == 1 ? 0 : 1);
    g_boxw_override = variant == 0 ? -1 : 0;
    if (stage == 2) { g_boxr_override = -1; g_boxp_override = variant == 0 ? -1 : (variant == 1 ? 0 : (variant == 2 ? 16 : 8)); }
    if (stage == 0 || stage == 1) {
        g_boxq_override = variant == 0 ? -1 : (variant == 3 || variant == 5 ? 1 : 0);
        if (variant == 3 || variant == 5) g_boxr_override = -1;
        g_boxq_b8_override = variant == 5 ? 0 : -1;
    }
    int rc = TRI_OK;
    BgStep s = {};
    s.r0 = s.r1 = (int)radius;
    s.time = TimeStage::PackedSweep;
    BgImages im = {};
    im.T = (int)n_line; im.Fa = (int)n_col; im.W = n_win;
    BgState bst = {};
    if (stage == 0) {
        im.dataTF = data; im.flagsTF = flags4;
        im.Aw = out_w; im.Ao = out_o; im.wsA = N;
    } else if (stage == 1) {
        im.Aw = const_cast<float*>(reinterpret_cast<const float*>(flags4));
        im.Ao = im.Aw + N; im.wsA = 2 * N;
        im.Bw = out_w; im.Bo = out_o; im.wsB = N;
        im.dataFT = data;
        s.freq = pick_freq_stage((int)radius, (int)n_col, (int)n_line, N, false);
    }
    DevBuf<float> x_data_tf;
    DevBuf<unsigned long long> x_stats;
    int xl = 0;
    if (stage == 1 && variant == 4) {
        g_boxx_override = 1;
        xl = boxx_pick_l((int)radius, (int)n_col);
        g_boxx_override = -1;
        if (!xl) return set_err(TRI_EUNSUPPORTED, "no exact row filter for radius %d on lines of %d", (int)radius, (int)n_col);
        HIPCHK(x_data_tf.alloc((size_t)n_win * N));
        HIPCHK(x_stats.alloc(2));
        HIPCHK(hipMemsetAsync(x_stats.get(), 0, 2 * sizeof(unsigned long long), r.st));
        rc = launch_transpose<float>(r, data, x_data_tf.get(), (int)n_col, (int)n_line, N, N, n_win);
        if (rc) return rc;
        s.freq = {FreqStage::ExactRows, 0, xl, 0};
        im.dataTF = x_data_tf.get(); im.rows = out_w; im.ws_rows = N; im.xstats = x_stats.get();
    }
    if (stage == 1 && s.freq.route == FreqStage::Transposed)
        return set_err(TRI_EUNSUPPORTED, "no single-sweep frequency stage for radius %d", (int)radius);
    HIPCHK(hipEventRecord(e0.get(), r.st));
    for (int i = 0; i < repeats && rc == TRI_OK; i++) {
        if (stage == 2) {
            if (variant >= 2 && boxp_pick_block((int)radius, (int)n_col) == 0) rc = set_err(TRI_EUNSUPPORTED, "no stage pipeline for this shape");
            else rc = launch_colfilter(r, ColSrc::ByteFlags, out_w, out_o, data, flags4, out_w, out_o, (int)n_line, (int)n_col, (int)radius, 0, 0, 0, 1, COL_WEIGHTS_01);
        } else if (stage == 0) {
            float den_t;
            rc = bg_time_stage(r, s, im, bst, &den_t);
        } else {
            rc = bg_freq_stage(r, s, im, bst, 0.0f);
        }
    }
    if (rc) return rc;
    HIPCHK(hipEventRecord(e1.get(), r.st));
    HIPCHK(hipEventSynchronize(e1.get()));
    LAUNCHCHK();
    float ms = 0;
    HIPCHK(hipEventElapsedTime(&ms, e0.get(), e1.get()));
    *ms_per_launch = ms / repeats;
    if (xl) {
        unsigned long long h[2] = {0, 0};
        HIPCHK(hipMemcpy(h, x_stats.get(), sizeof(h), hipMemcpyDeviceToHost));
        g_boxx_last_stats[0] = h[0];
        g_boxx_last_stats[1] = h[1];
        if (const char* e = getenv("TRI_BOXX_STATS")) if (e[0] == '1')
            fprintf(stderr, "k_boxx r=%d L=%d x %d threads: %llu line passes, %llu redone sequentially\n", (int)radius, xl & 255, xl >> 8, h[0], h[1]);
    }
    return TRI_OK;
}

#include <cxxabi.h>
extern "C" int tri_kernel_log(int op, char* buf, int64_t cap) {
    if (op == 0) {
        if (g_klog) g_klog->clear();
        g_klog_on = true;
        return 0;
    }
    g_klog_on = false;
    if (op != 1) return 0;
    if (!buf || cap <= 0) return set_err(TRI_EINVAL, "kernel log: no buffer");
    buf[0] = 0;
    if (!g_klog) return 0;
    std::vector<std::pair<std::string, long long>> rows;
    for (const auto& kv : *g_klog) {
        const char* m = hipKernelNameRefByPtr(kv.first, nullptr);
        std::string name = m ? m : "?";
        int st = 0;
        char* d = m ? abi::__cxa_demangle(m, nullptr, nullptr, &st) : nullptr;
        if (d && st == 0) { name = d; }
        if (d) free(d);
        const size_t par = name.find('(');
        if (par != std::string::npos) name.erase(par);
        if (name.compare(0, 5, "void ") == 0) name.erase(0, 5);
        rows.emplace_back(name, kv.second);
    }
    std::sort(rows.begin(), rows.end());
    size_t off = 0;
    for (const auto& r : rows) {
        const int n = snprintf(buf + off, (size_t)cap - off, "%s=%lld;", r.first.c_str(), r.second);
        if (n < 0 || off + (size_t)n >= (size_t)cap) break;
        off += (size_t)n;
    }
    return (int)rows.size();
}

extern "C" int tri_medrej_stats(uint64_t* out20, int reset) {
    unsigned long long h[20] = {0};
    HIPCHK(hipDeviceSynchronize());
    if (out20) {
        HIPCHK(hipMemcpyFromSymbol(h, HIP_SYMBOL(g_medrej_stats), sizeof(h)));
        for (int k = 0; k < 20; k++) out20[k] = h[k];
    }
    if (reset) {
        unsigned long long z[20] = {0};
        HIPCHK(hipMemcpyToSymbol(HIP_SYMBOL(g_medrej_stats), z, sizeof(z)));
    }
    return TRI_OK;
}

extern "C" int tri_boxx_last_stats(uint64_t* passes, uint64_t* sequential) {
    if (!passes || !sequential) return set_err(TRI_EINVAL, "NULL pointer argument");
    *passes = g_boxx_last_stats[0];
    *sequential = g_boxx_last_stats[1];
    return TRI_OK;
}

__global__ void k_check_box_divide(BoxDenom dn, unsigned long long* out) {
    unsigned long long bad = 0;
    const unsigned stride = gridDim.x * blockDim.x;
    unsigned i = blockIdx.x * blockDim.x + threadIdx.x;
    for (unsigned long long it = 0; it < (1ull << 32) / stride; it++, i += stride) {
        const float a = __uint_as_float(i);
        const float q = box_divide_checked(a, dn);
        const float e = a / dn.b;
        if (!((__float_as_uint(q) == __float_as_uint(e)) || (isnan(q) && isnan(e)))) bad++;
    }
    if (bad) atomicAdd(out, bad);
}
extern "C" int tri_test_box_divide(int64_t radius, uint64_t* mismatches, void* stream) {
    if (!mismatches || radius < 0 || radius > (1 << 20)) return set_err(TRI_EINVAL, "bad argument");
    hipStream_t st = (hipStream_t)stream;
    DevBuf<unsigned long long> d;
    HIPCHK(d.alloc(1));
    HIPCHK(hipMemsetAsync(d.get(), 0, sizeof(unsigned long long), st));
    hipLaunchKernelGGL(k_check_box_divide, dim3(4096), dim3(256), 0, st, box_reciprocal(box_denominator(radius)), d.get());
    LAUNCHCHK();
    unsigned long long h = 0;
    HIPCHK(hipMemcpyAsync(&h, d.get(), sizeof(h), hipMemcpyDeviceToHost, st));
    HIPCHK(hipStreamSynchronize(st));
    *mismatches = h;
    return TRI_OK;
}
// ... 766 lines not shown
```

Before: 3118 Mvis/s.

## Emit packed TF flags from begin transpose and skip redundant flag copies and stores

The fused begin transpose now also writes the packed time-by-4 TF flag layout directly into bgfTF, so background2d can skip its separate float transpose of flags. The spectral OR kernel keeps that packed copy consistent, and when TF flags equal the iteration flags the copy to flagsTF is dropped and medians read iter directly. The final kernel stores output flags only on the last major iteration. Together these cut several full-slab byte passes per iteration, at the cost of extra scattered writes in the spectral OR path and more coupled state between stages.

Result: no change. 3145 Mvis/s (median of 6 runs) (+0.9%).

```diff
diff --git a/tricolour_amd/csrc/kernels_elementwise.hpp b/tricolour_amd/csrc/kernels_elementwise.hpp
--- a/tricolour_amd/csrc/kernels_elementwise.hpp
+++ b/tricolour_amd/csrc/kernels_elementwise.hpp
@@ -82,7 +82,8 @@
 template <bool COPY, bool ZERO>
 __global__ __launch_bounds__(256) void k_transpose_u8w(const uint8_t* __restrict__ src, uint8_t* __restrict__ dst,
                                                        uint8_t* __restrict__ copy, float* __restrict__ data, int R, int C,
-                                                       size_t src_ws, size_t dst_ws, size_t copy_ws, size_t data_ws) {
+                                                       size_t src_ws, size_t dst_ws, size_t copy_ws, size_t data_ws,
+                                                       unsigned* __restrict__ tf4, size_t tf4_ws) {
     __shared__ unsigned tile[128][17];
     const uint8_t* s = src + (size_t)blockIdx.z * src_ws;
     uint8_t* d = dst + (size_t)blockIdx.z * dst_ws;
@@ -97,7 +98,7 @@
             unsigned v = 0;
             if (r < R && c < C) {
                 v = *reinterpret_cast<const unsigned*>(s + (size_t)r * C + c);
-                if (COPY) *reinterpret_cast<unsigned*>(copy + (size_t)blockIdx.z * copy_ws + (size_t)r * C + c) = v;
+                if (COPY && copy) *reinterpret_cast<unsigned*>(copy + (size_t)blockIdx.z * copy_ws + (size_t)r * C + c) = v;
             }
             tile[rr][tx] = v;
         }
@@ -114,6 +115,8 @@
         const unsigned u0 = __builtin_amdgcn_perm(a3, a2, 0x05010400u), u1 = __builtin_amdgcn_perm(a3, a2, 0x07030602u);
         const unsigned o[4] = {__builtin_amdgcn_perm(u0, t0, 0x05040100u), __builtin_amdgcn_perm(u0, t0, 0x07060302u),
                                __builtin_amdgcn_perm(u1, t1, 0x05040100u), __builtin_amdgcn_perm(u1, t1, 0x07060302u)};
+        if (tf4 && c0 + 4 * q < C)
+            *reinterpret_cast<uint4*>(tf4 + (size_t)blockIdx.z * tf4_ws + (size_t)(r >> 2) * C + c0 + 4 * q) = make_uint4(o[0], o[1], o[2], o[3]);
 #pragma unroll
         for (int b = 0; b < 4; b++) {
             const int c = c0 + 4 * q + b;
@@ -416,7 +419,7 @@
 __global__ void k_final(const uint8_t* __restrict__ dil, const int* __restrict__ rowcnt,
                         const int* __restrict__ colcnt, const void* __restrict__ vis,
                         uint8_t* __restrict__ out, uint8_t* __restrict__ iter, int T, int F,
-                        double row_limit, double col_limit, int update_iter) {
+                        double row_limit, double col_limit, int update_iter, int store_out) {
     size_t i = (size_t)blockIdx.x * blockDim.x + threadIdx.x;
     if (i >= (size_t)T * F) return;
     size_t win = blockIdx.y;
@@ -426,7 +429,7 @@
     v = v || ((double)rowcnt[win * (size_t)T + t] > row_limit);
     v = v || ((double)colcnt[win * (size_t)F + f] > col_limit);
     v = v || load_isnan<VD>(vis, a);
-    out[a] = v ? 1 : 0;
+    if (store_out) out[a] = v ? 1 : 0;
     if (update_iter && v) iter[a] = 1;
 }
 
@@ -551,13 +554,25 @@
     *pf = or4(or4(*pf, sp), reinterpret_cast<const uint4*>(more)[a]);
 }
 
-__global__ void k_or_spec_ft16(uint8_t* __restrict__ flagsFT, const uint8_t* __restrict__ spec_rows, int T16, int Fa) {
+__global__ void k_or_spec_ft16(uint8_t* __restrict__ flagsFT, const uint8_t* __restrict__ spec_rows, int T16, int Fa,
+                               unsigned* __restrict__ tf4) {
     size_t i = (size_t)blockIdx.x * blockDim.x + threadIdx.x;
     if (i >= (size_t)T16 * Fa) return;
     size_t win = blockIdx.y;
     int f = (int)(i / T16);
     if (!spec_rows[win * (size_t)Fa + f]) return;
-    reinterpret_cast<uint4*>(flagsFT + win * (size_t)T16 * 16 * Fa)[i] = make_uint4(0x01010101u, 0x01010101u, 0x01010101u, 0x01010101u);
+    uint4* pf = reinterpret_cast<uint4*>(flagsFT + win * (size_t)T16 * 16 * Fa) + i;
+    if (tf4) {
+        const uint4 cur = *pf;
+        const unsigned cw[4] = {cur.x, cur.y, cur.z, cur.w};
+        const int t16 = (int)(i - (size_t)f * T16);
+        unsigned* p = tf4 + win * (size_t)T16 * 4 * Fa + (size_t)t16 * 4 * Fa + f;
+#pragma unroll
+        for (int k = 0; k < 4; k++)
+            if (cw[k] != 0x01010101u) p[(size_t)k * Fa] = 0x01010101u;
+        if ((cw[0] & cw[1] & cw[2] & cw[3]) == 0x01010101u) return;
+    }
+    *pf = make_uint4(0x01010101u, 0x01010101u, 0x01010101u, 0x01010101u);
 }
 
 __global__ void k_combine16(const uint8_t* __restrict__ spec_rows, const uint8_t* __restrict__ tflags,
@@ -694,7 +709,7 @@
 __global__ void k_final16(const uint8_t* __restrict__ dil, const int* __restrict__ rowcnt,
                           const int* __restrict__ colcnt, const void* __restrict__ vis,
                           uint8_t* __restrict__ out, uint8_t* __restrict__ iter, int T, int F16,
-                          double row_limit, double col_limit, int update_iter) {
+                          double row_limit, double col_limit, int update_iter, int store_out) {
     size_t i = (size_t)blockIdx.x * blockDim.x + threadIdx.x;
     if (i >= (size_t)T * F16) return;
     size_t win = blockIdx.y;
@@ -731,7 +746,7 @@
         o[q] = rowall ? 0x01010101u : (dw[q] | colb | nanb);
     }
     uint4 ov = make_uint4(o[0], o[1], o[2], o[3]);
-    reinterpret_cast<uint4*>(out)[a16] = ov;
+    if (store_out) reinterpret_cast<uint4*>(out)[a16] = ov;
     if (update_iter) {
         uint4* ip = reinterpret_cast<uint4*>(iter) + a16;
         *ip = or4(*ip, ov);
diff --git a/tricolour_amd/csrc/tricolour_amd.hip b/tricolour_amd/csrc/tricolour_amd.hip
--- a/tricolour_amd/csrc/tricolour_amd.hip
+++ b/tricolour_amd/csrc/tricolour_amd.hip
@@ -856,7 +856,7 @@
         ((uintptr_t)src % 4 == 0) && ((uintptr_t)dst % 4 == 0)) {
         dim3 gridw((unsigned)cdiv(C, 64), (unsigned)cdiv(R, 128), (unsigned)W);
         hipLaunchKernelGGL((k_transpose_u8w<false, false>), gridw, dim3(256), 0, r.st, (const uint8_t*)src, (uint8_t*)dst,
-                           (uint8_t*)nullptr, (float*)nullptr, R, C, sws, dws, (size_t)0, (size_t)0);
+                           (uint8_t*)nullptr, (float*)nullptr, R, C, sws, dws, (size_t)0, (size_t)0, (unsigned*)nullptr, (size_t)0);
         LAUNCHCHK();
         return TRI_OK;
     }
@@ -1259,6 +1259,22 @@
             t.ytiles > 0 && t.ytiles <= 65535;
     return t;
 }
+static int launch_reject_tile(hipStream_t st, const float* resid, const uint8_t* flags_in, uint8_t* flags_out, uint8_t* flags_t4, double* med,
+                              const int64_t* d_chunk_ends, double rej, int Fa, int T4, int G, int ytiles, unsigned W, size_t ws_resid,
+                              size_t ws_flags, unsigned* sc, size_t scratch_ws, size_t ccap, size_t ucap, int force_fallback) {
+    hipLaunchKernelGGL(k_mr_predict, dim3((unsigned)G, W), dim3(256), 0, st, resid, flags_in, d_chunk_ends, rej, T4, G, ws_resid, ws_flags, sc,
+                       scratch_ws, ccap, ucap, force_fallback);
+    for (unsigned round = 1; round <= 2; round++) {
+        hipLaunchKernelGGL(k_mr_pass, dim3((unsigned)cdiv(T4, 64), (unsigned)ytiles, W), dim3(256), 0, st, resid, flags_in, flags_out, flags_t4, d_chunk_ends, Fa, T4, G, ws_resid, ws_flags,
+                           sc, scratch_ws, ccap, ucap, round);
+        hipLaunchKernelGGL(k_mr_finish, dim3((unsigned)G, W), dim3(256), 0, st, resid, flags_in, flags_out, flags_t4, med, d_chunk_ends, rej, Fa,
+                           T4, G, ws_resid, ws_flags, sc, scratch_ws, ccap, ucap, round);
+    }
+    hipLaunchKernelGGL(k_median_reject, dim3((unsigned)G, W), dim3(256), 0, st, resid, flags_in, flags_out, flags_t4, med, d_chunk_ends, rej, Fa,
+                       T4, G, ws_resid, ws_flags, sc, scratch_ws, 0u, 0u, 1, (const unsigned*)sc, scratch_ws, (int)MRT_PARW, 11);
+    LAUNCHCHK();
+    return TRI_OK;
+}
 static unsigned medrej_capq(size_t wsA, int G) {
     const size_t per_block = (wsA / (size_t)G) & ~(size_t)7;
     return (unsigned)std::min<size_t>(per_block / 2, 0x3ffffffcu);
@@ -1441,19 +1457,10 @@
             return TRI_OK;
         }
         case Reject::Tile: {
-            unsigned* sc = reinterpret_cast<unsigned*>(ws.Aw);
-            hipLaunchKernelGGL(k_mr_predict, dim3((unsigned)G, (unsigned)W), dim3(256), 0, r.st, (const float*)ws.Bo, (const uint8_t*)st.cur_ft,
-                               ws.d_chunk_ends, rej, T / 4, G, wsB, N, sc, wsA, tile.ccap, tile.ucap, medrej_force_fallback());
-            for (unsigned round = 1; round <= 2; round++) {
-                hipLaunchKernelGGL(k_mr_pass, dim3((unsigned)cdiv(T / 4, 64), (unsigned)tile.ytiles, (unsigned)W), dim3(256), 0, r.st, (const float*)ws.Bo,
-                                   (const uint8_t*)st.cur_ft, st.alt_ft, ws.bgfTF, ws.d_chunk_ends, Fa, T / 4, G, wsB, N, sc, wsA, tile.ccap, tile.ucap, round);
-                hipLaunchKernelGGL(k_mr_finish, dim3((unsigned)G, (unsigned)W), dim3(256), 0, r.st, (const float*)ws.Bo, (const uint8_t*)st.cur_ft, st.alt_ft,
-                                   ws.bgfTF, ws.med, ws.d_chunk_ends, rej, Fa, T / 4, G, wsB, N, sc, wsA, tile.ccap, tile.ucap, round);
-            }
-            hipLaunchKernelGGL(k_median_reject, dim3((unsigned)G, (unsigned)W), dim3(256), 0, r.st, (const float*)ws.Bo, (const uint8_t*)st.cur_ft,
-                               st.alt_ft, ws.bgfTF, ws.med, ws.d_chunk_ends, rej, Fa, T / 4, G, wsB, N, sc, wsA, 0u, 0u, 1,
-                               (const unsigned*)sc, wsA, (int)MRT_PARW, 11);
-            LAUNCHCHK();
+            const int rc = launch_reject_tile(r.st, ws.Bo, st.cur_ft, st.alt_ft, ws.bgfTF, ws.med, ws.d_chunk_ends, rej, Fa, T / 4, G, tile.ytiles,
+                                              (unsigned)W, wsB, N, reinterpret_cast<unsigned*>(ws.Aw), wsA, tile.ccap, tile.ucap,
+                                              medrej_force_fallback());
+            if (rc) return rc;
             std::swap(st.cur_ft, st.alt_ft);
             if (st.alt_ft == ws.flagsFT) st.alt_ft = ws.fflFT;
             return TRI_OK;
@@ -1493,7 +1500,7 @@
     return launch_transpose<uint8_t>(r, st.cur_ft, ws.bgfTF, Fa, T, N, N, W);
 }
 
-int background2d(const Run& r, bool flagsFT_current, float* residP = nullptr, bool* wroteP = nullptr) {
+int background2d(const Run& r, bool flagsFT_current, bool tf4_current, float* residP = nullptr, bool* wroteP = nullptr) {
     const Plan& pl = r.pl;
     const Ws& ws = r.ws;
     const int T = (int)pl.T, Fa = (int)pl.Fa;
@@ -1510,7 +1517,9 @@
         rc = flagsFT_current ? launch_u8<0>(r, ws.flagsFT, ws.bgfFT, N, N, N, W)
                              : launch_transpose<uint8_t>(r, ws.flagsTF, ws.bgfFT, T, Fa, N, N, W);
     if (rc) return rc;
-    if (packed)
+    if (packed && tf4_current)
+        ;
+    else if (packed)
         rc = launch_transpose<float>(r, reinterpret_cast<const float*>(flags_in_place ? ws.flagsFT : ws.bgfFT), reinterpret_cast<float*>(ws.bgfTF), Fa, T / 4, N / 4, N / 4, W);
     else
         rc = launch_u8<0>(r, ws.flagsTF, ws.bgfTF, N, N, N, W);
@@ -1579,6 +1588,8 @@
     bool panel;
     bool fused_resid;
     int lo, hi, flo, fhi;
+    bool tf4_from_begin;
+    bool tf_flags_are_iter;
     bool ft_current() const { return spec_or == SpecOr::FtInPlace || spec_or == SpecOr::FtInPlaceDeferTf; }
 };
 
@@ -1615,6 +1626,8 @@
     s.panel = !st_no_panel() && s.chunk_flags == ChunkFlags::ExtraSources && s.finish == Finish::FusedDilate && Fa % 64 == 0 && Fa == F &&
               median_takes_extra_flags(pl.maxchunk + 3) && st_use_fused(pl.swT) && st_use_mask(T, Fa);
     s.fused_resid = s.panel && !no_fused_resid;
+    s.tf4_from_begin = s.begin == Begin::FusedCached && s.ft_current() && bg_flags_packed(T, N);
+    s.tf_flags_are_iter = s.tf4_from_begin && s.chunk_flags == ChunkFlags::ExtraSources && Fa == F;
     return s;
 }
 
@@ -1631,17 +1644,17 @@
     return TRI_OK;
 }
 template <int VD>
-static int launch_final(const Run& r, const IterStep& s, const void* vis, uint8_t* out_flags, bool update_iter) {
+static int launch_final(const Run& r, const IterStep& s, const void* vis, uint8_t* out_flags, bool update_iter, bool store_out) {
     const Ws& ws = r.ws;
-    const int T = (int)r.pl.T, F = (int)r.pl.F, upd = update_iter ? 1 : 0;
+    const int T = (int)r.pl.T, F = (int)r.pl.F, upd = update_iter ? 1 : 0, sto = store_out ? 1 : 0;
     const size_t NF = (size_t)T * F, W = (size_t)r.Wb;
     const double row_limit = r.p->flag_all_freq_frac * (double)F, col_limit = (double)T * r.p->flag_all_time_frac;
     if (s.final_kernel == FinalKernel::NanMask16)
-        hipLaunchKernelGGL(k_final16<TRI_VIS_NANMASK>, grid1(NF / 16, W), dim3(256), 0, r.st, ws.dil, ws.rowcnt, ws.colcnt, (const void*)ws.nanmask, out_flags, ws.iter, T, F / 16, row_limit, col_limit, upd);
+        hipLaunchKernelGGL(k_final16<TRI_VIS_NANMASK>, grid1(NF / 16, W), dim3(256), 0, r.st, ws.dil, ws.rowcnt, ws.colcnt, (const void*)ws.nanmask, out_flags, ws.iter, T, F / 16, row_limit, col_limit, upd, sto);
     else if (s.final_kernel == FinalKernel::Vis16)
-        hipLaunchKernelGGL(k_final16<VD>, grid1(NF / 16, W), dim3(256), 0, r.st, ws.dil, ws.rowcnt, ws.colcnt, vis, out_flags, ws.iter, T, F / 16, row_limit, col_limit, upd);
+        hipLaunchKernelGGL(k_final16<VD>, grid1(NF / 16, W), dim3(256), 0, r.st, ws.dil, ws.rowcnt, ws.colcnt, vis, out_flags, ws.iter, T, F / 16, row_limit, col_limit, upd, sto);
     else
-        hipLaunchKernelGGL(k_final<VD>, grid1(NF, W), dim3(256), 0, r.st, ws.dil, ws.rowcnt, ws.colcnt, vis, out_flags, ws.iter, T, F, row_limit, col_limit, upd);
+        hipLaunchKernelGGL(k_final<VD>, grid1(NF, W), dim3(256), 0, r.st, ws.dil, ws.rowcnt, ws.colcnt, vis, out_flags, ws.iter, T, F, row_limit, col_limit, upd, sto);
     LAUNCHCHK();
     return TRI_OK;
 }
@@ -1657,7 +1670,8 @@
     switch (s.begin) {
         case Begin::FusedCached:
             hipLaunchKernelGGL((k_transpose_u8w<true, true>), dim3((unsigned)cdiv(Fa, 64), (unsigned)cdiv(T, 128), (unsigned)W), dim3(256), 0, r.st,
-                               ws.iter, ws.flagsFT, ws.flagsTF, ws.dataFT, T, Fa, N, N, N, N);
+                               ws.iter, ws.flagsFT, s.tf_flags_are_iter ? (uint8_t*)nullptr : ws.flagsTF, ws.dataFT, T, Fa, N, N, N, N,
+                               s.tf4_from_begin ? reinterpret_cast<unsigned*>(ws.bgfTF) : (unsigned*)nullptr, N / 4);
             break;
         case Begin::Cached:
             rc = launch_u8<0>(r, ws.iter, ws.flagsTF, N, N, N, W);
@@ -1700,6 +1714,7 @@
     if (!rc) rc = spectrum_medians(r, ws.sres, ws.sflags);
     if (!rc) rc = launch_colst(r, r.pl.swF, ws.sres, ws.smed, ws.sout, ws.d_chunk_ends, Fa, Wn, (int)r.pl.G, 0, 0, 1);
     if (rc) return rc;
+    unsigned* const tf4 = s.tf4_from_begin ? reinterpret_cast<unsigned*>(ws.bgfTF) : nullptr;
     if (s.spec_or != SpecOr::Scalar)
         hipLaunchKernelGGL(k_spec_rows, dim3((unsigned)cdiv(nS, 256)), dim3(256), 0, r.st, ws.sout, ws.srows, Fa, Wn);
     switch (s.spec_or) {
@@ -1711,10 +1726,10 @@
             break;
         case SpecOr::FtInPlace:
             hipLaunchKernelGGL(k_or_spec16, grid1(N / 16, W), dim3(256), 0, r.st, ws.flagsTF, ws.srows, T, Fa / 16);
-            hipLaunchKernelGGL(k_or_spec_ft16, grid1(N / 16, W), dim3(256), 0, r.st, ws.flagsFT, ws.srows, T / 16, Fa);
+            hipLaunchKernelGGL(k_or_spec_ft16, grid1(N / 16, W), dim3(256), 0, r.st, ws.flagsFT, ws.srows, T / 16, Fa, tf4);
             break;
         case SpecOr::FtInPlaceDeferTf:
-            hipLaunchKernelGGL(k_or_spec_ft16, grid1(N / 16, W), dim3(256), 0, r.st, ws.flagsFT, ws.srows, T / 16, Fa);
+            hipLaunchKernelGGL(k_or_spec_ft16, grid1(N / 16, W), dim3(256), 0, r.st, ws.flagsFT, ws.srows, T / 16, Fa, tf4);
             break;
     }
     LAUNCHCHK();
@@ -1725,7 +1740,7 @@
     const Ws& ws = r.ws;
     const int T = (int)r.pl.T, Fa = (int)r.pl.Fa;
     bool wrote_panel = false;
-    const int rc = background2d(r, s.ft_current(), s.fused_resid ? ws.residP : nullptr, &wrote_panel);
+    const int rc = background2d(r, s.ft_current(), s.tf4_from_begin, s.fused_resid ? ws.residP : nullptr, &wrote_panel);
     *residTF = wrote_panel ? ws.residP : ws.Aw;
     if (rc || wrote_panel) return rc;
     return launch_transpose<float>(r, ws.Bw, ws.Aw, Fa, T, (size_t)r.pl.PF * T, (size_t)T * Fa, r.Wb, 0.0f, s.panel);
@@ -1742,7 +1757,7 @@
     if (!rc) rc = launch_colst(r, pl.swT, residTF, ws.med, ws.tflTF, ws.d_tends, T, Fa, 1, N, N, W, s.panel);
     if (rc) return rc;
     MedianJob cj;
-    cj.data = residTF; cj.flags = ws.flagsTF; cj.med = ws.med; cj.WSd = cj.WSf = N; cj.RS = (size_t)Fa;
+    cj.data = residTF; cj.flags = s.tf_flags_are_iter ? ws.iter : ws.flagsTF; cj.med = ws.med; cj.WSd = cj.WSf = N; cj.RS = (size_t)Fa;
     cj.seg_start = ws.segC_start; cj.seg_len = ws.segC_len; cj.R = T; cj.G = G; cj.W = W; cj.max_len = pl.maxchunk;
     cj.rows_aligned = Fa % 4 == 0;
     switch (s.chunk_flags) {
@@ -1783,7 +1798,7 @@
     return TRI_OK;
 }
 
-static int iter_finish(const Run& r, const IterStep& s, const void* vis, int vis_dtype, uint8_t* out_flags, bool update_iter) {
+static int iter_finish(const Run& r, const IterStep& s, const void* vis, int vis_dtype, uint8_t* out_flags, bool update_iter, bool store_out) {
     const Ws& ws = r.ws;
     const int T = (int)r.pl.T, F = (int)r.pl.F, Fa = (int)r.pl.Fa, Wn = (int)r.Wb;
     const size_t N = (size_t)T * Fa;
@@ -1814,18 +1829,18 @@
             break;
     }
     LAUNCHCHK();
-    return BY_VIS_DTYPE(launch_final, r, s, vis, out_flags, update_iter);
+    return BY_VIS_DTYPE(launch_final, r, s, vis, out_flags, update_iter, store_out);
 }
 #undef BY_VIS_DTYPE
 
-int run_iteration(const Run& r, const IterStep& s, const void* vis, int vis_dtype, uint8_t* out_flags, bool update_iter, bool tap) {
+int run_iteration(const Run& r, const IterStep& s, const void* vis, int vis_dtype, uint8_t* out_flags, bool update_iter, bool store_out, bool tap) {
     const float* residTF = nullptr;
     int rc = iter_begin(r, s, vis, vis_dtype);
     if (!rc) rc = iter_spectrum(r, s);
     if (!rc) rc = iter_residual(r, s, &residTF);
     if (!rc) rc = iter_sumthreshold(r, s, residTF);
     if (!rc && tap && r.dbg) rc = iter_taps(r, s, residTF);
-    if (!rc) rc = iter_finish(r, s, vis, vis_dtype, out_flags, update_iter);
+    if (!rc) rc = iter_finish(r, s, vis, vis_dtype, out_flags, update_iter, store_out);
     return rc;
 }
 
@@ -1882,7 +1897,7 @@
         for (int64_t it = 0; it < p->num_major_iterations; it++) {
             bool last = it == p->num_major_iterations - 1;
             bool tap = last && tap_first && w0 == w_begin;
-            rc = run_iteration(r, step, vis_b, vis_dtype, out_b, !last, tap);
+            rc = run_iteration(r, step, vis_b, vis_dtype, out_b, !last, last, tap);
             if (rc) return rc;
         }
     }
@@ -2279,15 +2294,9 @@
     const unsigned W = (unsigned)n_win;
     HIPCHK(hipEventRecord(e0.get(), st));
     for (int i = 0; i < repeats; i++) {
-        hipLaunchKernelGGL(k_mr_predict, dim3((unsigned)G, W), dim3(256), 0, st, resid, flags_in, d_ends, rej, T / 4, G, N, N, sc, wsS, ccap, ucap, 0);
-        for (unsigned round = 1; round <= 2; round++) {
-            hipLaunchKernelGGL(k_mr_pass, dim3((unsigned)cdiv(T / 4, 64), (unsigned)ytiles, W), dim3(256), 0, st, resid, flags_in, flags_out, flags_t4,
-                               d_ends, Fa, T / 4, G, N, N, sc, wsS, ccap, ucap, round);
-            hipLaunchKernelGGL(k_mr_finish, dim3((unsigned)G, W), dim3(256), 0, st, resid, flags_in, flags_out, flags_t4, med, d_ends, rej, Fa, T / 4, G,
-                               N, N, sc, wsS, ccap, ucap, round);
-        }
-        hipLaunchKernelGGL(k_median_reject, dim3((unsigned)G, W), dim3(256), 0, st, resid, flags_in, flags_out, flags_t4, med, d_ends, rej, Fa, T / 4, G,
-                           N, N, sc, wsS, 0u, 0u, 1, (const unsigned*)sc, wsS, (int)MRT_PARW, 11);
+        const int rc = launch_reject_tile(st, resid, flags_in, flags_out, flags_t4, med, d_ends, rej, Fa, T / 4, G, ytiles, W, N, N, sc, wsS, ccap,
+                                          ucap, 0);
+        if (rc) return rc;
     }
     HIPCHK(hipEventRecord(e1.get(), st));
     hipError_t le = hipGetLastError();
```
